# sailordiary/m3f.pytorch

Hardware: AMD Instinct MI355X
Metric: clips/sec (300-frame A+V, fwd+bwd) (higher is better)
Workload: dtype f32 (fp32-accurate products, fp32 accumulate: GEMMs as fp16x3 -- two fp16 terms per scaled operand, three MFMAs, error vs fp64 no larger than an fp32 GEMM's; the forward and backward recurrences at H=512 and H=256 as fp16x3 too (h is bounded; the backward producers split their values under a power-o

## Files before the change

### include/m3t_hip.h

```cpp
#ifndef M3T_HIP_H
#define M3T_HIP_H

#include <stddef.h>
#include <stdint.h>

#ifdef __cplusplus
extern "C" {
#endif

#define M3T_EINVAL 10001
#define M3T_MAX_SCANS 8
#define M3T_ESPIN 10002
#define M3T_SCAN_NO_PERSIST 1
#define M3T_SCAN_WHH 8
#define M3T_SCAN_FP32 4
#define M3T_SCAN_FAULT 16
#define M3T_SCAN_WIDE 32
#define M3T_BF16 2
#define M3T_GEMM_BACKGROUND 1
#define M3T_GEMM_BF16 2
#define M3T_GEMM_HIGH 256
#define M3T_GEMM_F16X3 1024
#define M3T_GEMM_BESIDE_SCAN 512
#define M3T_GEMM_EXCLUSIVE 8
#define M3T_CONV_IMAGES 4096

int m3t_im2col3d(const float* x, int N, int Ci, int T, int H, int W, int kt, int kh, int kw, int st, int sh, int sw,
                 int pt, int ph, int pw, float* out, long long rows_pad, int Kp, unsigned long long* amax_slot, void* stream);

int m3t_conv3d_taps(const float* src, const float* w_taps, float* dst, int N, int C_src, int C_dst, int T, int H, int W,
                    int To, int Ho, int Wo, int kt, int kh, int kw, int base_t, int base_h, int base_w, int sign, int flags,
                    const unsigned long long* amax_src, const unsigned long long* amax_w, float* ws, size_t ws_bytes, float* dst_planes,
                    void* stream);

int m3t_f16x3_split(const float* x, size_t rows, int cols, size_t ld, float* out, size_t ldo, const unsigned long long* slot, void* stream);
int m3t_f16x3_split_perm(const float* w, size_t R, int T, int Cc, size_t sR, size_t sT, size_t sC, float* out, const unsigned long long* slot,
                         void* stream);
int m3t_sgemm_pre(int M, int N, int K, const float* A_img, int lda, const float* B_img, int ldb, float* C, int ldc,
                  const float* bias, int act, int accumulate, const unsigned long long* amax_a, const unsigned long long* amax_b, void* stream);
int m3t_f16x3_image_b(const float* w, int N, int K, size_t ld, float* img, const unsigned long long* slot, void* stream);
int m3t_sgemm_bimg(int M, int N, int K, const float* A, int lda, const float* B_img, float* C, int ldc, const float* bias, int act,
                   int accumulate, float* ws, size_t ws_bytes, const unsigned long long* amax_a, const unsigned long long* amax_b, void* stream);
int m3t_sgemm_ring(int transA, int transB, int M, int N, int K, const float* A, int lda, const float* B, int ldb, float* C, int ldc,
                   const float* bias, int act, int accumulate, int seg_len, int seg_stride, int a_off, int b_off, float* ws, size_t ws_bytes,
                   int splits, const unsigned long long* amax_a, const unsigned long long* amax_b, int variant, void* stream);
int m3t_conv3d_taps_pre(const float* src_img, const float* w_img, float* dst, int N, int C_src, int C_dst, int T, int H, int W,
                        int To, int Ho, int Wo, int kt, int kh, int kw, int base_t, int base_h, int base_w, int sign,
                        const unsigned long long* amax_src, const unsigned long long* amax_w, float* ws, size_t ws_bytes, float* dst_planes,
                    void* stream);

int m3t_planes_to_cl4(const float* x, float* out, int N, int C, long long S, void* stream);
int m3t_conv3d_fwd_taps4(const float* x_img4, const float* w_img, const float* bias, float* y_cl, int N, int Co, int T, int H, int W,
                         int kt, int kh, int kw, int st, int sh, int sw, int pt, int ph, int pw, const unsigned long long* amax_x,
                         const unsigned long long* amax_w, float* ws, size_t ws_bytes, float* y_planes, void* stream);
int m3t_conv3d_fwd_taps(const float* x_img, const float* w_img, const float* bias, float* y_cl, int N, int Ci, int Co, int T, int H, int W,
                        int kt, int kh, int kw, int st, int sh, int sw, int pt, int ph, int pw, const unsigned long long* amax_x,
                        const unsigned long long* amax_w, float* ws, size_t ws_bytes, float* y_planes, void* stream);
int m3t_conv3d_wgrad_taps(const float* x_cl, const float* dy_cl, float* dwt, int N, int Ci, int Co, int T, int H, int W, int kt, int kh, int kw,
                          int st, int sh, int sw, int pt, int ph, int pw, int flags, const unsigned long long* amax_x,
                          const unsigned long long* amax_dy, float* ws, size_t ws_bytes, void* stream);

int m3t_amax_out(unsigned long long* slot);

int m3t_version(void);
int m3t_device_arch(char* arch, int cap);

int m3t_sgemm(int transA, int transB, int M, int N, int K,
              const float* A, int lda, const float* B, int ldb,
              float* C, int ldc, const float* bias, int act, int accumulate,
              int seg_len, int seg_stride, int a_off, int b_off,
              float* ws, size_t ws_bytes, int flags, void* stream);

int m3t_sgemm_scaled(int transA, int transB, int M, int N, int K,
                     const float* A, int lda, const float* B, int ldb,
                     float* C, int ldc, const float* bias, int act, int accumulate,
                     int seg_len, int seg_stride, int a_off, int b_off,
                     float* ws, size_t ws_bytes, int flags,
                     const unsigned long long* amax_a, const unsigned long long* amax_b, void* stream);

int m3t_sgemm_window(int transB, int n_seg, int win_len, int win_stride, int win_off, int N, int K,
                     const float* A, int lda, const float* B, int ldb, float* C, int ldc, const float* bias,
                     int act, int accumulate, int flags, const unsigned long long* amax_a, const unsigned long long* amax_b, void* stream);
#define M3T_WINDOW_BATCH 8
typedef struct {
    const float* A; const float* B; float* C; const float* bias;
    const unsigned long long* amax_a; const unsigned long long* amax_b;
    int accumulate;
} m3t_window_problem;
int m3t_sgemm_window_batch(int n, const m3t_window_problem* problems, int transB, int n_seg, int win_len, int win_stride, int win_off,
                           int N, int K, int lda, int ldb, int ldc, int act, int flags, void* stream);

int m3t_absmax(int n, const float* const* x, const size_t* rows, const int* cols, const size_t* ld,
               unsigned long long* const* slots, void* stream);

int m3t_sgemm_plan(int transA, int M, int N, int K, int seg_len, size_t ws_bytes, int flags, int* kernel, int* splits);

int m3t_colsum(const float* X, int M, int N, int ld, float* out, int accumulate,
               float* ws, size_t ws_bytes, void* stream);

int m3t_transpose(const float* src, int R, int C, int lds, float* dst, int ldd, void* stream);

int m3t_relu_bwd(const float* a, float* dy, size_t n, void* stream);

typedef struct {
    const float* xproj;
    const float* w_hh;
    const float* b_hh;
    float* out;
    float* gates;
    float* h_n;
    int H, reverse, ldx, xoff, ldo, ooff;
} m3t_gru_fwd_desc;

int m3t_gru_scan_fwd(const m3t_gru_fwd_desc* scans, int n_scans, int B, int T,
                     float* ws, size_t ws_bytes, int flags, void* stream);

typedef struct {
    const float* dout;
    const float* out;
    const float* gates;
    const float* w_hh_t;
    const float* dh_n;
    float* dgx;
    float* dgh;
    float* dh;
    float* db_part;
    float* db_ih;
    float* db_hh;
    int H, reverse, ldo, ooff, ldg, goff;
    unsigned long long* amax;
    const float* wfrag;
} m3t_gru_bwd_desc;

size_t m3t_gru_bwd_prepare_floats(int H);
int m3t_gru_bwd_prepare(const float* const* w, int n, int H, int whh_direct, float* const* out, void* stream);

int m3t_gru_scan_workgroups(int n_scans, int H, int B, int T, int flags, int backward);
int m3t_gru_persist_count(void);
int m3t_gru_poll_error(void);
int m3t_gru_error_reset(void);
int m3t_gru_error_defer(int on);
int m3t_gru_inject_error(void* stream);
int m3t_gru_persist_owner(void);
int m3t_gru_scan_arena(void* arena, size_t bytes);
int m3t_gru_scan_arena_reset(void* arena);
int m3t_gru_scan_progress(unsigned* counters, int n_marks, const int* time_bounds, unsigned* need);
int m3t_gru_scan_progress_reset(unsigned* counters);
int m3t_gru_scan_progress_ok(int n_scans, int H, int B, int T, int flags, int backward);
int m3t_stream_wait_progress(const unsigned* counter, unsigned need, void* stream);
int m3t_gru_scan_after(void* event);
int m3t_gru_scan_events(void* start, void* end);
int m3t_gru_persist_profile(unsigned long long* out6);

int m3t_gru_scan_bwd(const m3t_gru_bwd_desc* scans, int n_scans, int B, int T,
                     float* ws, size_t ws_bytes, int flags, void* stream);

int m3t_att_fuse_fwd(const float* s_v, const float* s_a, const float* x_v, const float* x_a,
                     float* f, int rows, int D, void* stream);
int m3t_att_fuse_bwd(const float* df, const float* s_v, const float* s_a,
                     const float* x_v, const float* x_a,
                     float* ds_v, float* ds_a, float* dx_v, float* dx_a,
                     int rows, int D, void* stream);

int m3t_va_loss(const float* y_hat, int rows, int C, int iv, int ia,
                const float* valence, const float* arousal,
                const int64_t* class_expr, const uint8_t* expr_valid, int n_expr,
                float w_v, float w_a, float expr_w, int use_mse,
                float* out_scalars, float* dy, float* ws, size_t ws_bytes, void* stream);
size_t m3t_va_loss_ws_bytes(int rows);

size_t m3t_bn_cl_ws_bytes(size_t M, int C);
int m3t_bn_pool_cl_fwd(const float* x, size_t P, int H, int W, int C, int k, const float* gamma, const float* beta, float* run_mean, float* run_var,
                       float momentum, float eps, int training, float* yp, unsigned char* win, float* save_mean, float* save_invstd, float* ws,
// ... 207 lines not shown
```

### m3f.pytorch_amd/csrc/gemm.hip

```cpp
#include "common.h"
#include <cstdio>
#include <cstdlib>

namespace {

constexpr int BM = 128, BN = 128, BK = 16, LDT = 132;

struct GemmParams {
    const float* A; const float* B; float* C; const float* bias; float* ws;
    int M, N, K, lda, ldb, ldc;
    int act, accumulate, splits, kchunk;
    int seg_len, seg_stride, a_off, b_off;
    int bf16;
    int vecA, vecB;
};

__device__ __forceinline__ int seg_row(int k, int seg_len, int seg_stride, int off) {
    return seg_len > 0 ? (k / seg_len) * seg_stride + (k % seg_len) + off : k;
}

__device__ __forceinline__ void load_kc(const float* __restrict__ src, int ld, int rows, int row0,
                                        int k0, int k_end, int vec, float4 (&r)[2]) {
    const int tid = threadIdx.x;
#pragma unroll
// ... 194 lines not shown
            const float bv = (direct && p.bias) ? p.bias[col] : 0.f;
#pragma unroll
            for (int r = 0; r < 16; ++r) {
                const int row = bm + wm * 64 + i * 32 + (r & 3) + 8 * (r >> 2) + 4 * hi;
                if (!FAST && row >= p.M) continue;
                float v = acc[i][j][r];
                float* q = dst + (size_t)row * ldd + col;
                if (direct) {
                    v += bv;
                    if (p.act == 1) v = m3t_relu(v);
                    if (p.accumulate) v += *q;
                }
                *q = v;
            }
        }
}

__global__ void splitk_reduce_kernel(const float* __restrict__ ws, float* __restrict__ C, const float* __restrict__ bias,
                                     int M, int N, int ldc, int splits, int act, int accumulate) {
    const size_t total = (size_t)M * N;
    for (size_t i = blockIdx.x * (size_t)blockDim.x + threadIdx.x; i < total; i += (size_t)gridDim.x * blockDim.x) {
        const int m = (int)(i / N), n = (int)(i % N);
        float s = 0.f;
        for (int k = 0; k < splits; ++k) s += ws[(size_t)k * total + i];
        if (bias) s += bias[n];
        if (act == 1) s = m3t_relu(s);
        float* q = C + (size_t)m * ldc + n;
        if (accumulate) s += *q;
        *q = s;
    }
}

constexpr int SK_FOLD = 32;
__global__ __launch_bounds__(256) void splitk_fold4_kernel(float* __restrict__ ws, size_t total4, int splits) {
    float4* w4 = reinterpret_cast<float4*>(ws);
    const int k0 = blockIdx.y * SK_FOLD, k1 = min(splits, k0 + SK_FOLD);
    for (size_t i = blockIdx.x * (size_t)blockDim.x + threadIdx.x; i < total4; i += (size_t)gridDim.x * blockDim.x) {
        float4 s = make_float4(0.f, 0.f, 0.f, 0.f);
        int k = k0;
        for (; k + 8 <= k1; k += 8) {
            float4 v[8];
#pragma unroll
            for (int u = 0; u < 8; ++u) v[u] = w4[(size_t)(k + u) * total4 + i];
#pragma unroll
            for (int u = 0; u < 8; ++u) { s.x += v[u].x; s.y += v[u].y; s.z += v[u].z; s.w += v[u].w; }
        }
        for (; k < k1; ++k) {
            const float4 v = w4[(size_t)k * total4 + i];
            s.x += v.x; s.y += v.y; s.z += v.z; s.w += v.w;
        }
        w4[(size_t)k0 * total4 + i] = s;
    }
}

__global__ __launch_bounds__(256) void splitk_reduce4_kernel(const float* __restrict__ ws, float* __restrict__ C,
                                                             const float* __restrict__ bias, int M, int N, int ldc, int splits,
                                                             int act, int accumulate, int kstride) {
    const size_t total4 = (size_t)M * N / 4, slab4 = total4 * (size_t)kstride;
    const float4* w4 = reinterpret_cast<const float4*>(ws);
    const int n4 = N / 4;
    for (size_t i = blockIdx.x * (size_t)blockDim.x + threadIdx.x; i < total4; i += (size_t)gridDim.x * blockDim.x) {
        float4 s = make_float4(0.f, 0.f, 0.f, 0.f);
        int k = 0;
        for (; k + 8 <= splits; k += 8) {
            float4 v[8];
#pragma unroll
            for (int u = 0; u < 8; ++u) v[u] = w4[(size_t)(k + u) * slab4 + i];
#pragma unroll
            for (int u = 0; u < 8; ++u) { s.x += v[u].x; s.y += v[u].y; s.z += v[u].z; s.w += v[u].w; }
        }
        for (; k < splits; ++k) {
            const float4 v = w4[(size_t)k * slab4 + i];
            s.x += v.x; s.y += v.y; s.z += v.z; s.w += v.w;
        }
        const int m = (int)(i / n4), n = (int)(i % n4) * 4;
        if (bias) { s.x += bias[n]; s.y += bias[n + 1]; s.z += bias[n + 2]; s.w += bias[n + 3]; }
        if (act == 1) { s.x = m3t_relu(s.x); s.y = m3t_relu(s.y); s.z = m3t_relu(s.z); s.w = m3t_relu(s.w); }
        float4* q = reinterpret_cast<float4*>(C + (size_t)m * ldc + n);
        if (accumulate) { const float4 c = *q; s.x += c.x; s.y += c.y; s.z += c.z; s.w += c.w; }
        *q = s;
    }
}


constexpr int ABSMAX_REGIONS = 16;
struct AbsmaxArgs { M3TRegion r[ABSMAX_REGIONS]; };
__global__ __launch_bounds__(256) void f16x3_absmax_kernel(AbsmaxArgs a, unsigned epoch) {
    const M3TRegion r = a.r[blockIdx.y];
    const unsigned long long total = r.rows * (unsigned long long)r.c4;
    if ((unsigned long long)blockIdx.x * 256 >= total && blockIdx.x > 0) return;
    unsigned m = 0u;
    const bool dense = (unsigned long long)r.c4 * 4ull == r.ld;
    auto at = [&](unsigned long long i) -> const uint4* {
        if (dense) return reinterpret_cast<const uint4*>(r.p + (size_t)i * 4);
        const unsigned long long row = i / (unsigned)r.c4;
        return reinterpret_cast<const uint4*>(r.p + (size_t)(row * r.ld + (i - row * (unsigned)r.c4) * 4ull));
    };
    auto fin = [](unsigned b) { b &= 0x7fffffffu; return b < 0x7f800000u ? b : 0u; };
    auto fold = [&](const uint4& v) { m = max(max(m, fin(v.x)), max(fin(v.y), max(fin(v.z), fin(v.w)))); };
    const unsigned long long stride = (unsigned long long)gridDim.x * 256;
    unsigned long long i = (unsigned long long)blockIdx.x * 256 + threadIdx.x;
    for (; i + 3 * stride < total; i += 4 * stride) {
        const uint4 v0 = *at(i), v1 = *at(i + stride), v2 = *at(i + 2 * stride), v3 = *at(i + 3 * stride);
        fold(v0); fold(v1); fold(v2); fold(v3);
    }
    for (; i < total; i += stride) fold(*at(i));
#pragma unroll
    for (int o = 32; o > 0; o >>= 1) m = max(m, (unsigned)__shfl_xor((int)m, o, 64));
    __shared__ unsigned red[4];
    if ((threadIdx.x & 63) == 0) red[threadIdx.x >> 6] = m;
    __syncthreads();
    if (threadIdx.x == 0) {
        m = max(max(red[0], red[1]), max(red[2], red[3]));
        const unsigned long long val = ((unsigned long long)epoch << 32) | m;
        if (__hip_atomic_load(r.slot, __ATOMIC_RELAXED, __HIP_MEMORY_SCOPE_AGENT) < val) atomicMax(r.slot, val);
    }
}

static int launch_absmax(const M3TRegion* regs, int n, unsigned epoch, hipStream_t s) {
    AbsmaxArgs a;
    unsigned long long tm = 0;
    for (int i = 0; i < n; ++i) {
        a.r[i] = regs[i];
        const unsigned long long t = regs[i].rows * (unsigned long long)regs[i].c4;
        if (t > tm) tm = t;
    }
    for (int i = n; i < ABSMAX_REGIONS; ++i) a.r[i] = regs[0];
    unsigned long long blocks = (tm + 256ull * 8 - 1) / (256ull * 8);
    static int total = 0;
    if (!total) { const char* e = getenv("M3T_ABSMAX_TOTAL"); total = (e && atoi(e) > 0) ? atoi(e) : 384; }
    const unsigned long long cap = (unsigned long long)max(16, total / max(1, n));
    if (blocks > cap) blocks = cap;
    if (blocks < 1) blocks = 1;
    if (blocks > 1024) blocks = 1024;
    f16x3_absmax_kernel<<<dim3((unsigned)blocks, n), 256, 0, s>>>(a, epoch);
    return (int)hipGetLastError();
}

static void launch_splitk_reduce(const float* ws, float* C, const float* bias, int M, int N, int ldc, int splits, int act,
                                 int accumulate, hipStream_t s) {
    const size_t total = (size_t)M * N;
    if (N % 4 == 0 && ldc % 4 == 0 && ((uintptr_t)C % 16) == 0 && ((uintptr_t)ws % 16) == 0) {
        int blocks = (int)((total / 4 + 255) / 256);
        if (blocks > 4096) blocks = 4096;
        if (splits >= 4 * SK_FOLD && blocks <= 64) {
            const int groups = (splits + SK_FOLD - 1) / SK_FOLD;
            splitk_fold4_kernel<<<dim3(blocks, groups), 256, 0, s>>>(const_cast<float*>(ws), total / 4, splits);
            splitk_reduce4_kernel<<<blocks, 256, 0, s>>>(ws, C, bias, M, N, ldc, groups, act, accumulate, SK_FOLD);
            return;
        }
        splitk_reduce4_kernel<<<blocks, 256, 0, s>>>(ws, C, bias, M, N, ldc, splits, act, accumulate, 1);
        return;
    }
    int blocks = (int)((total + 255) / 256);
    if (blocks > 2048) blocks = 2048;
    splitk_reduce_kernel<<<blocks, 256, 0, s>>>(ws, C, bias, M, N, ldc, splits, act, accumulate);
}

__global__ void colsum_kernel(const float* __restrict__ X, int M, int N, int ld, float* __restrict__ out, int accumulate) {
    __shared__ float red[8][33];
    const int c = blockIdx.x * 32 + (threadIdx.x & 31);
    const int rl = threadIdx.x >> 5;
    float s = 0.f;
    if (c < N)
        for (int m = rl; m < M; m += 8) s += X[(size_t)m * ld + c];
    red[rl][threadIdx.x & 31] = s;
// ... 182 lines not shown
    }
    return on == 1;
}

bool m3t_gemm_tr_enabled() {
    static int on = -1;
    if (on < 0) {
        const char* e = getenv("M3T_GEMM_TR");
        on = (e && e[0] == '0') ? 0 : 1;
    }
    return on == 1;
}

static bool f16x3_on_x6d() { return true; }

static bool x6_enabled() {
    static int on = -1;
    if (on < 0) {
        const char* e = getenv("M3T_GEMM_X6");
        on = (e && e[0] == '0') ? 0 : 1;
    }
    return on == 1;
}

constexpr int GEMM_NO_WIDE = 1 << 20;
struct GemmPlan { int kernel, splits, kchunk, narrow, wide; };

static int narrow_mode() { return 1; }

static bool x6w_enabled() {
    static int on = -1;
    if (on < 0) { const char* e = getenv("M3T_GEMM_X6W"); on = (e && e[0] == '0') ? 0 : 1; }
    return on == 1;
}

static bool tr_wide_wins(int flags) { return (flags & M3T_GEMM_BESIDE_SCAN) != 0; }

static GemmPlan plan_gemm(int transA, int M, int N, int K, int seg_len, bool vec, size_t ws_bytes, int flags) {
    GemmPlan g;
    g.narrow = 0;
    const int bf16 = (flags & M3T_GEMM_BF16) ? 1 : 0;
    const int high = (!bf16 && (flags & M3T_GEMM_HIGH)) ? 1 : 0;
    const int f16x3 = (!bf16 && !high && (flags & M3T_GEMM_F16X3) && m3t_f16x3_enabled()) ? 1 : 0;
    const int tiles = cdiv(M, BM) * cdiv(N, BN);
    const bool n64 = (N % 128 != 0) && (N % 64 == 0) && narrow_mode();
    const bool x6 = x6_enabled() && (M % 128 == 0) && (N % 128 == 0 || n64) && (K % 32 == 0 || seg_len >= 32) && K > 0 && vec &&
                    (seg_len == 0 || seg_len >= 32);
    const double ns_per_k = x6 ? (bf16 ? 14.0 : (high ? 27.0 : (f16x3 ? 22.0 : 36.0))) : 84.0;
    const int kq = x6 ? 32 : BK;
    int splits = 1;
    const size_t cap = ws_bytes / ((size_t)M * N * sizeof(float));
    double best = 1e30;
    auto model = [&](int ntiles, double nsk, int sp) {
        const int rounds = cdiv(ntiles * sp, 256);
        double t = (double)rounds * ((double)K / sp) * nsk * (rounds == 1 ? 1.3 : 1.0);
        if (sp > 1) t += (double)(sp + 2) * M * N * 4.0 / 3000.0 + 3000.0;
        return t;
    };
    if (ws_bytes && K >= 512) {
        for (int sp = 1; sp <= 96 && sp <= K / 96 && (sp == 1 || (size_t)sp <= cap); ++sp) {
            const double t = model(tiles, ns_per_k, sp);
            if (t < best) { best = t; splits = sp; }
        }
    } else best = model(tiles, ns_per_k, 1);
    g.wide = 0;
    if (x6 && !bf16 && !high && N % 256 == 0 && x6w_enabled() && !(flags & (M3T_GEMM_BACKGROUND | GEMM_NO_WIDE))) {
        const int tiles_w = cdiv(M, BM) * (N / 256);
        double best_w = 1e30; int splits_w = 1;
        if (ws_bytes && K >= 512) {
            for (int sp = 1; sp <= 96 && sp <= K / 96 && (sp == 1 || (size_t)sp <= cap); ++sp) {
                const double t = model(tiles_w, 2.0 * 0.8 * ns_per_k, sp);
                if (t < best_w) { best_w = t; splits_w = sp; }
            }
        } else best_w = model(tiles_w, 2.0 * 0.8 * ns_per_k, 1);
        if (best_w < best) { g.wide = 1; splits = splits_w; }
    }
    int kchunk = cdiv(cdiv(K, splits), kq) * kq;
    if (kchunk < kq) kchunk = kq;
    g.kernel = x6 ? 1 : 0; g.kchunk = kchunk; g.splits = K > 0 ? cdiv(K, kchunk) : 1;
    g.narrow = (!g.wide && x6 && narrow_mode() && (n64 || narrow_mode() == 2 || (g.splits == 1 && tiles <= 384))) ? 1 : 0;
    return g;
}

extern "C" int m3t_sgemm_plan(int transA, int M, int N, int K, int seg_len, size_t ws_bytes, int flags, int* kernel, int* splits) {
    if (M <= 0 || N <= 0 || K < 0 || !kernel || !splits) return M3T_EINVAL;
    const GemmPlan g = plan_gemm(transA, M, N, K, seg_len, true, ws_bytes, flags | (transA ? GEMM_NO_WIDE : 0));
    *kernel = g.kernel; *splits = g.splits;
    return 0;
}

extern "C" int m3t_sgemm(int transA, int transB, int M, int N, int K, const float* A, int lda, const float* B, int ldb,
                         float* C, int ldc, const float* bias, int act, int accumulate, int seg_len, int seg_stride,
                         int a_off, int b_off, float* ws, size_t ws_bytes, int flags, void* stream) {
    return m3t_sgemm_scaled(transA, transB, M, N, K, A, lda, B, ldb, C, ldc, bias, act, accumulate, seg_len, seg_stride, a_off, b_off,
                            ws, ws_bytes, flags, nullptr, nullptr, stream);
}

extern "C" int m3t_sgemm_scaled(int transA, int transB, int M, int N, int K, const float* A, int lda, const float* B, int ldb,
                                float* C, int ldc, const float* bias, int act, int accumulate, int seg_len, int seg_stride,
                                int a_off, int b_off, float* ws, size_t ws_bytes, int flags, const unsigned long long* amax_a,
                                const unsigned long long* amax_b, void* stream) {
    if (M <= 0 || N <= 0) return 0;
    if (K < 0 || !A || !B || !C) return M3T_EINVAL;
    if (seg_len > 0 && !(transA == 1 && transB == 0)) return M3T_EINVAL;
    GemmParams p;
    p.A = A; p.B = B; p.C = C; p.bias = bias; p.ws = ws;
    p.M = M; p.N = N; p.K = K; p.lda = lda; p.ldb = ldb; p.ldc = ldc;
    p.act = act; p.accumulate = accumulate;
    p.seg_len = seg_len; p.seg_stride = seg_stride; p.a_off = a_off; p.b_off = b_off;
    p.bf16 = (flags & M3T_GEMM_BF16) ? 1 : 0;
    p.vecA = (lda % 4 == 0) && ((uintptr_t)A % 16 == 0);
    p.vecB = (ldb % 4 == 0) && ((uintptr_t)B % 16 == 0);
    const int tm = cdiv(M, BM), tn = cdiv(N, BN);
    const GemmPlan g = plan_gemm(transA, M, N, K, seg_len, p.vecA && p.vecB, ws ? ws_bytes : 0,
                                 flags | ((transA == 0 && transB == 1) ? 0 : GEMM_NO_WIDE));
    int splits = g.splits, kchunk = g.kchunk;
    {
        static int beside_wgs = -1;
        if (beside_wgs < 0) { const char* e = getenv("M3T_GEMM_BESIDE_WGS"); beside_wgs = e ? atoi(e) : 384; }
        if (beside_wgs > 0 && (flags & M3T_GEMM_BESIDE_SCAN) && g.kernel != 0 && !g.wide && g.splits > 1) {
            const int tiles = cdiv(M, BM) * cdiv(N, g.narrow ? 64 : BN);
            int sp = (beside_wgs + tiles / 2) / tiles;
            if (sp < 1) sp = 1;
            if (sp < g.splits) {
                kchunk = cdiv(cdiv(K, sp), 32) * 32;
                splits = cdiv(K, kchunk);
            }
        }
    }
    p.splits = splits; p.kchunk = kchunk;
    hipStream_t s = (hipStream_t)stream;
    if (g.kernel != 0) {
        int rc;
        const int f16x3 = (!p.bf16 && !(flags & M3T_GEMM_HIGH) && (flags & M3T_GEMM_F16X3) && m3t_f16x3_enabled()) ? 1 : 0;
        const bool wide_tr = f16x3 && !g.wide && !g.narrow && !(transA == 0 && transB == 1) && !(flags & M3T_GEMM_BACKGROUND) && N % 256 == 0 &&
                             K % 32 == 0 && x6w_enabled() && m3t_gemm_tr_enabled() && tr_wide_wins(flags);
        const unsigned long long* use_a = nullptr; const unsigned long long* use_b = nullptr;
        if (f16x3) {
            const size_t kr = seg_len > 0 ? (size_t)(K / seg_len - 1) * seg_stride + seg_len : (size_t)K;
            const float* A0 = seg_len > 0 ? A + (size_t)a_off * lda : A;
            const float* B0 = seg_len > 0 ? B + (size_t)b_off * ldb : B;
            const M3TRegion ra{A0, (unsigned long long)(transA ? kr : (size_t)M), (unsigned long long)lda, (transA ? M : K) / 4, nullptr};
            const M3TRegion rb{B0, (unsigned long long)(transB ? (size_t)N : kr), (unsigned long long)ldb, (transB ? K : N) / 4, nullptr};
            const int rm = m3t_f16x3_measure(ra, amax_a, rb, amax_b, &use_a, &use_b, s);
            if (rm) return rm;
        }
        if (g.wide || wide_tr)
            rc = m3t_sgemm_x6w_launch(transA, transB, M, N, K, A, lda, B, ldb, C, ldc, bias, act, accumulate, seg_len, seg_stride,
                                      a_off, b_off, ws, splits, kchunk, f16x3 ? 3 : 0, use_a, use_b, s);
        else if (!g.narrow && K % 32 == 0 && (!f16x3 || f16x3_on_x6d()) && !(flags & (M3T_GEMM_BACKGROUND | M3T_GEMM_HIGH)) && (x6d_mode() == 1 || (x6d_mode() == 2 && !(flags & M3T_GEMM_BESIDE_SCAN))))
            rc = m3t_sgemm_x6d_launch(transA, transB, M, N, K, A, lda, B, ldb, C, ldc, bias, act, accumulate, seg_len, seg_stride,
                                      a_off, b_off, ws, splits, kchunk, p.bf16 ? 1 : ((flags & M3T_GEMM_HIGH) ? 2 : (f16x3 ? 3 : 0)), use_a, use_b, s);
        else
            rc = m3t_sgemm_x6_launch(transA, transB, M, N, K, A, lda, B, ldb, C, ldc, bias, act, accumulate, seg_len, seg_stride,
                                     a_off, b_off, ws, splits, kchunk, (flags & M3T_GEMM_BACKGROUND) ? (size_t)40 * 1024 : 0,
                                     p.bf16 ? 1 : ((flags & M3T_GEMM_HIGH) ? 2 : (f16x3 ? 3 : 0)), g.narrow, use_a, use_b, s);
        if (rc) return rc;
        if (splits > 1) {
            launch_splitk_reduce(ws, C, bias, M, N, ldc, splits, act, accumulate, s);
            M3T_LAUNCH_CHECK();
        }
        return 0;
    }
    dim3 grid(tn, tm, splits), block(256);
    const bool fast = (M % BM == 0) && (N % BN == 0) && (K % BK == 0) && K > 0 && p.vecA && p.vecB;
    const size_t dyn = (flags & M3T_GEMM_BACKGROUND) ? (size_t)56 * 1024 + 0 : 0;
#define M3T_GEMM_LAUNCH(TA_, TB_)                                                 \
    do {                                                                          \
        if (fast && seg_len >= BK) sgemm_kernel<TA_, TB_, true, true><<<grid, block, dyn, s>>>(p); \
        else if (seg_len > 0) sgemm_kernel<TA_, TB_, false><<<grid, block, dyn, s>>>(p);           \
        else if (fast) sgemm_kernel<TA_, TB_, true><<<grid, block, dyn, s>>>(p);    \
        else sgemm_kernel<TA_, TB_, false><<<grid, block, dyn, s>>>(p);             \
    } while (0)
    if (transA == 0 && transB == 1) M3T_GEMM_LAUNCH(0, 1);
    else if (transA == 0 && transB == 0) M3T_GEMM_LAUNCH(0, 0);
    else if (transA == 1 && transB == 0) M3T_GEMM_LAUNCH(1, 0);
    else M3T_GEMM_LAUNCH(1, 1);
#undef M3T_GEMM_LAUNCH
    M3T_LAUNCH_CHECK();
    if (splits > 1) {
        launch_splitk_reduce(ws, C, bias, M, N, ldc, splits, act, accumulate, s);
        M3T_LAUNCH_CHECK();
    }
    return 0;
}

int m3t_sgemm_x6_window_launch(int n, const m3t_window_problem* pr, int transB, int M, int N, int K, int lda, int ldb, int ldc,
                               int act, int mw_len, int mw_stride, int mw_off, int f16x3, int narrow, hipStream_t s);

extern "C" int m3t_sgemm_window_batch(int n, const m3t_window_problem* pr, int transB, int n_seg, int win_len, int win_stride, int win_off,
                                      int N, int K, int lda, int ldb, int ldc, int act, int flags, void* stream) {
    if (n <= 0 || n_seg <= 0 || win_len <= 0 || N <= 0) return 0;
    if (n > M3T_WINDOW_BATCH || !pr || K <= 0 || win_stride < win_len || win_off < 0 || win_off + win_len > win_stride) return M3T_EINVAL;
    const long long Ml = (long long)n_seg * win_len;
    if (Ml > 0x7fffffffll || (long long)n_seg * win_stride > 0x7fffffffll) return M3T_EINVAL;
    const int M = (int)Ml;
    if (!x6_enabled() || M % 128 != 0 || N % 64 != 0 || K % 32 != 0 || lda % 4 != 0 || ldb % 4 != 0 || (flags & (M3T_GEMM_BF16 | M3T_GEMM_HIGH)))
        return M3T_EINVAL;
    const int f16x3 = ((flags & M3T_GEMM_F16X3) && m3t_f16x3_enabled()) ? 1 : 0;
    hipStream_t s = (hipStream_t)stream;
    m3t_window_problem use[M3T_WINDOW_BATCH];
    for (int i = 0; i < n; ++i) {
        use[i] = pr[i];
        if (!use[i].A || !use[i].B || !use[i].C || (uintptr_t)use[i].A % 16 != 0 || (uintptr_t)use[i].B % 16 != 0) return M3T_EINVAL;
        if (f16x3 && (!use[i].amax_a || !use[i].amax_b)) {
            if (n > 1) return M3T_EINVAL;
            const size_t span = (size_t)(n_seg - 1) * win_stride + win_len;
            const M3TRegion ra{use[i].A + (size_t)win_off * lda, (unsigned long long)span, (unsigned long long)lda, K / 4, nullptr};
            const M3TRegion rb{use[i].B, (unsigned long long)(transB ? (size_t)N : (size_t)K), (unsigned long long)ldb, (transB ? K : N) / 4, nullptr};
            const int rm = m3t_f16x3_measure(ra, use[i].amax_a, rb, use[i].amax_b, &use[i].amax_a, &use[i].amax_b, s);
            if (rm) return rm;
        }
    }
    const int narrow = (N % 128 != 0 || (long long)(M / 128) * (N / 128) * n <= 384) ? 1 : 0;
    return m3t_sgemm_x6_window_launch(n, use, transB ? 1 : 0, M, N, K, lda, ldb, ldc, act, win_len, win_stride, win_off, f16x3, narrow, s);
}

extern "C" int m3t_sgemm_window(int transB, int n_seg, int win_len, int win_stride, int win_off, int N, int K,
                                const float* A, int lda, const float* B, int ldb, float* C, int ldc, const float* bias,
                                int act, int accumulate, int flags, const unsigned long long* amax_a, const unsigned long long* amax_b,
                                void* stream) {
    const m3t_window_problem pr{A, B, C, bias, amax_a, amax_b, accumulate};
    return m3t_sgemm_window_batch(1, &pr, transB, n_seg, win_len, win_stride, win_off, N, K, lda, ldb, ldc, act, flags, stream);
}

int m3t_conv3d_taps_launch(const float* src, const float* w_taps, float* dst, int N, int Cs, int Cd, int T, int H, int W, int To, int Ho, int Wo,
                           int kt, int kh, int kw, int bt_, int bh, int bw, int sg, int f16x3, int pre, const unsigned long long* amax_a,
                           const unsigned long long* amax_b, float* ws, int splits, int kchunk, hipStream_t s, const int* stride3 = nullptr,
                           const float* bias = nullptr, int planes = 0);
extern "C" int m3t_btc_to_bct(const float* src, float* dst, int B, int T, int C, void* stream);
int m3t_conv3d_wgrad_launch(const float* x_cl, const float* dy_cl, float* dwt, int N, int Ci, int Co, int T, int H, int W, int To, int Ho, int Wo,
                            int kt, int kh, int kw, const int* stride3, int pt, int ph, int pw, int f16x3, const unsigned long long* amax_x,
                            const unsigned long long* amax_dy, float* ws, int splits, int kchunk, hipStream_t s, int pre);

int m3t_conv3d_taps4_launch(const float* x_img4, const float* w_img, const float* bias, float* y_cl, int N, int Co, int T, int H, int W, int To,
                            int Ho, int Wo, int kt, int kh, int kw, const int* stride3, int pt, int ph, int pw, const unsigned long long* amax_x,
                            const unsigned long long* amax_w, float* ws, int splits, int kchunk, hipStream_t s, int planes);

static void taps_split(long long rows, int Cd, int K, float* ws, size_t ws_bytes, int& splits, int& kchunk) {
    splits = 1; kchunk = K;
    const long long tiles = ((rows + 127) / 128) * ((Cd + 127) / 128);
    if (!ws || tiles >= 512) return;
    int sp = (int)((640 + tiles - 1) / tiles);
    const size_t cap = ws_bytes / ((size_t)rows * Cd * sizeof(float));
    if ((size_t)sp > cap) sp = (int)cap;
    if (sp > K / 256) sp = K / 256;
    if (sp < 2) return;
    kchunk = cdiv(cdiv(K, sp), 32) * 32;
    splits = cdiv(K, kchunk);
}

namespace {
typedef _Float16 sp_f16x2 __attribute__((ext_vector_type(2)));
typedef float sp_f32x2 __attribute__((ext_vector_type(2)));
__global__ __launch_bounds__(256) void f16x3_split_kernel(const float* __restrict__ x, float* __restrict__ out, size_t rows, int c4, size_t ld,
                                                          size_t ldo, const unsigned long long* __restrict__ slot) {
    float sc, inv;
    m3t_f16_scale((unsigned)*slot, sc, inv);
    const size_t total = rows * (size_t)c4;
    for (size_t i = blockIdx.x * (size_t)blockDim.x + threadIdx.x; i < total; i += (size_t)gridDim.x * blockDim.x) {
        const size_t r = i / c4; const int c = (int)(i - r * c4);
        const float4 v = *reinterpret_cast<const float4*>(x + r * ld + 4 * (size_t)c);
        const sp_f32x2 a = (sp_f32x2){v.x, v.y} * sc, b = (sp_f32x2){v.z, v.w} * sc;
        const sp_f16x2 ha = __builtin_convertvector(a, sp_f16x2), hb = __builtin_convertvector(b, sp_f16x2);
        const sp_f16x2 la = __builtin_convertvector(a - __builtin_convertvector(ha, sp_f32x2), sp_f16x2);
// ... 417 lines not shown
```

### m3f.pytorch_amd/csrc/gemm_x6.hip

```cpp
#include "common.h"
#include <cstdlib>

namespace {

typedef __bf16 bf16x8 __attribute__((ext_vector_type(8)));
typedef __bf16 bf16x4 __attribute__((ext_vector_type(4)));

constexpr int XM = 128, XN = 128, XK = 32;
constexpr int PLANE = XM * 16 + 64;
constexpr int SPLIT_BYTES = 4 * PLANE;
constexpr int OPER_BYTES = 3 * SPLIT_BYTES;
constexpr int TRROW = XM * 2 + 64;
constexpr int TRTERM = XK * TRROW;
static_assert(2 * TRTERM <= OPER_BYTES, "the transposed-read image must fit the operand's LDS");
typedef short s16x4 __attribute__((ext_vector_type(4)));

struct X6Params {
    const float* A; const float* B; float* C; const float* bias; float* ws;
    int M, N, K, lda, ldb, ldc;
    int act, accumulate, splits, kchunk;
    int seg_len, seg_stride, a_off, b_off;
    int cv_T, cv_C, cv_K, cv_dil, cv_lead, cv_anti;
    size_t cv_btap;
    const float* cv_mask; const float* cv_res; float* cv_pre;
// ... 62 lines not shown
__device__ __forceinline__ void kc_store(unsigned char* __restrict__ S, const float4 (&r)[4], float scale = 1.f) {
    const int tid = threadIdx.x & 255;
    const int c = tid & 7, r0 = tid >> 3;
#pragma unroll
    for (int i = 0; i < NR; ++i) {
        unsigned lo[3], hi2[3];
        if (PRE) {
            lo[0] = __float_as_uint(r[i].x); hi2[0] = __float_as_uint(r[i].y); lo[1] = __float_as_uint(r[i].z); hi2[1] = __float_as_uint(r[i].w);
        } else {
            split3_pair<NS>((f32x2){r[i].x, r[i].y}, lo, scale);
            split3_pair<NS>((f32x2){r[i].z, r[i].w}, hi2, scale);
        }
#pragma unroll
        for (int s = 0; s < planes_of(NS); ++s)
            *reinterpret_cast<u32x2*>(S + s * SPLIT_BYTES + (c >> 1) * PLANE + (r0 + 32 * i) * 16 + (c & 1) * 8) = (u32x2){lo[s], hi2[s]};
    }
}
template <int NS, bool PRE = false>
__device__ __forceinline__ void mc_store(unsigned char* __restrict__ S, const float4 (&r)[4], float scale = 1.f) {
    const int tid = threadIdx.x & 255;
    const int wave = tid >> 6, h = (tid >> 5) & 1, row0 = (tid & 31) * 4;
    typedef unsigned u32x4 __attribute__((ext_vector_type(4)));
    unsigned lo[4][3], hi2[4][3];
    if (PRE && NS == 4) {
#pragma unroll
        for (int i = 0; i < 4; ++i) {
            const unsigned sel = (i & 1) ? 0x07060302u : 0x05040100u;
#pragma unroll
            for (int s = 0; s < 2; ++s) {
                const unsigned c0 = __float_as_uint(s == 0 ? (i < 2 ? r[0].x : r[0].y) : (i < 2 ? r[0].z : r[0].w));
                const unsigned c1 = __float_as_uint(s == 0 ? (i < 2 ? r[1].x : r[1].y) : (i < 2 ? r[1].z : r[1].w));
                const unsigned c2 = __float_as_uint(s == 0 ? (i < 2 ? r[2].x : r[2].y) : (i < 2 ? r[2].z : r[2].w));
                const unsigned c3 = __float_as_uint(s == 0 ? (i < 2 ? r[3].x : r[3].y) : (i < 2 ? r[3].z : r[3].w));
                lo[i][s] = __builtin_amdgcn_perm(c1, c0, sel);
                hi2[i][s] = __builtin_amdgcn_perm(c3, c2, sel);
            }
        }
    } else
#pragma unroll
    for (int i = 0; i < 4; ++i) {
        const float v0 = i == 0 ? r[0].x : i == 1 ? r[0].y : i == 2 ? r[0].z : r[0].w;
        const float v1 = i == 0 ? r[1].x : i == 1 ? r[1].y : i == 2 ? r[1].z : r[1].w;
        const float v2 = i == 0 ? r[2].x : i == 1 ? r[2].y : i == 2 ? r[2].z : r[2].w;
        const float v3 = i == 0 ? r[3].x : i == 1 ? r[3].y : i == 2 ? r[3].z : r[3].w;
        split3_pair<NS>((f32x2){v0, v1}, lo[i], scale);
        split3_pair<NS>((f32x2){v2, v3}, hi2[i], scale);
    }
    unsigned char* q = S + wave * PLANE + (row0 + 2 * h) * 16;
#pragma unroll
    for (int s = 0; s < planes_of(NS); ++s) {
        const u32x2 e0 = __builtin_amdgcn_permlane32_swap(lo[0][s], lo[2][s], false, false);
        const u32x2 e1 = __builtin_amdgcn_permlane32_swap(hi2[0][s], hi2[2][s], false, false);
        const u32x2 f0 = __builtin_amdgcn_permlane32_swap(lo[1][s], lo[3][s], false, false);
        const u32x2 f1 = __builtin_amdgcn_permlane32_swap(hi2[1][s], hi2[3][s], false, false);
        *reinterpret_cast<u32x4*>(q + s * SPLIT_BYTES) = (u32x4){e0.x, e1.x, e0.y, e1.y};
        *reinterpret_cast<u32x4*>(q + s * SPLIT_BYTES + 16) = (u32x4){f0.x, f1.x, f0.y, f1.y};
    }
}

template <int NS, bool PRE = false>
__device__ __forceinline__ void mc_store_tr(unsigned char* __restrict__ S, const float4 (&r)[4], float scale = 1.f) {
    const int tid = threadIdx.x & 255;
    unsigned char* q = S + 4 * (tid >> 5) * TRROW + (tid & 31) * 8;
#pragma unroll
    for (int e = 0; e < 4; ++e) {
        unsigned a[3], b[3];
        if (PRE) {
            a[0] = __float_as_uint(r[e].x); b[0] = __float_as_uint(r[e].y); a[1] = __float_as_uint(r[e].z); b[1] = __float_as_uint(r[e].w);
        } else {
            split3_pair<NS>((f32x2){r[e].x, r[e].y}, a, scale);
            split3_pair<NS>((f32x2){r[e].z, r[e].w}, b, scale);
        }
#pragma unroll
        for (int s = 0; s < planes_of(NS); ++s) *reinterpret_cast<u32x2*>(q + s * TRTERM + e * TRROW) = (u32x2){a[s], b[s]};
    }
}
__device__ __forceinline__ bf16x8 tr_frag(const unsigned char* at) {
    typedef __attribute__((address_space(3))) s16x4 lds_s16x4;
    const s16x4 lo = __builtin_amdgcn_ds_read_tr16_b64_v4i16((lds_s16x4*)(at));
    const s16x4 hi = __builtin_amdgcn_ds_read_tr16_b64_v4i16((lds_s16x4*)(at + 4 * TRROW));
    return __builtin_bit_cast(bf16x8, __builtin_shufflevector(lo, hi, 0, 1, 2, 3, 4, 5, 6, 7));
}

template <int TA, int TB, bool SEG, int NS, bool CONV = false, int XNT = 128, bool MW = false, int C3 = 0, int PRE = 0, bool TR = false>
__global__ __launch_bounds__(256, 3) void sgemm_x6_kernel(X6Params p, X6Batch bt) {
    static_assert(!TR || NS == 4, "the transposed-read image is sized for two terms");
    constexpr bool TRA = TR && TA == 1, TRB = TR && TB == 0;
    if (MW) {
        const int z = blockIdx.z;
        p.A = bt.A[z]; p.B = bt.B[z]; p.C = bt.C[z]; p.bias = bt.bias[z];
        p.amax_a = bt.amax_a[z]; p.amax_b = bt.amax_b[z]; p.accumulate = bt.accumulate[z];
    }
    constexpr int NJ = XNT / 64;
    constexpr int BR = XNT / 32;
    __shared__ __attribute__((aligned(16))) unsigned char lds[2 * OPER_BYTES];
    unsigned char* As = lds;
    unsigned char* Bs = lds + OPER_BYTES;
    const int tid = threadIdx.x, lane = tid & 63, wave = tid >> 6;
    const int wm = wave >> 1, wn = wave & 1;
    const int l31 = lane & 31, hi = lane >> 5;

    const int tn_ = gridDim.x, nt_ = gridDim.x * gridDim.y;
    const int lin = blockIdx.y * tn_ + blockIdx.x;
    const int xq = nt_ >> 3, xr = nt_ & 7, xcd = lin & 7, slot = lin >> 3;
    const int til = xcd * xq + min(xcd, xr) + slot;
    const int bm = (til / tn_) * XM, bn = (til % tn_) * XNT;
    const bool bcol = XNT == 128 || (tid & 31) < 16;
    const int k_begin = MW ? 0 : blockIdx.z * p.kchunk;
    const int k_end = min(p.K, k_begin + p.kchunk);
    const int ntiles = (C3 == 2 || SEG) ? (k_end - k_begin + XK - 1) / XK : (k_end - k_begin) / XK;
    __shared__ int rowmap[MW ? XM : 1];
    if (MW) {
        if (tid < XM) {
            const int m = bm + tid, q = m / p.mw_len;
            rowmap[tid] = q * p.mw_stride + (m - q * p.mw_len) + p.mw_off;
        }
        __syncthreads();
    }

    f32x16 acc[2][NJ];
#pragma unroll
    for (int i = 0; i < 2; ++i)
#pragma unroll
        for (int j = 0; j < NJ; ++j)
#pragma unroll
            for (int r = 0; r < 16; ++r) acc[i][j][r] = 0.f;

    float sc_a = 1.f, sc_b = 1.f, sc_ia = 1.f, sc_ib = 1.f;
    if (NS == 4) {
        m3t_f16_scale((unsigned)*p.amax_a, sc_a, sc_ia);
        m3t_f16_scale((unsigned)*p.amax_b, sc_b, sc_ib);
    }

    const float* pa; const float* pb;
    size_t a_step, b_step, a_krow = 0, b_krow = 0;
    const float* paw[MW ? 4 : 1];
    if (TA == 0) { pa = p.A + (size_t)(bm + (tid >> 3)) * p.lda + k_begin + (tid & 7) * 4; a_step = XK; }
    else { pa = p.A + (size_t)(k_begin + (tid >> 5) * 4) * p.lda + bm + (tid & 31) * 4; a_step = (size_t)XK * p.lda; a_krow = p.lda; }
    if (MW) {
#pragma unroll
        for (int i = 0; i < 4; ++i) paw[i] = p.A + (size_t)rowmap[(tid >> 3) + 32 * i] * p.lda + k_begin + (tid & 7) * 4;
    }
    if (TB == 1) { pb = p.B + (size_t)(bn + (tid >> 3)) * p.ldb + k_begin + (tid & 7) * 4; b_step = XK; }
    else { pb = p.B + (size_t)(k_begin + (tid >> 5) * 4) * p.ldb + bn + (tid & 31) * 4; b_step = (size_t)XK * p.ldb; b_krow = p.ldb; }
    int sq = 0, sr = 0;
    if (SEG) {
        const int k = k_begin + (tid >> 5) * 4;
        sq = k / p.seg_len; sr = k % p.seg_len;
    }

    constexpr bool C3ROWS = C3 == 1 || C3 == 3;
    int c3_tt[C3ROWS ? 4 : 1], c3_hh[C3ROWS ? 4 : 1], c3_ww[C3ROWS ? 4 : 1], c3_nb[C3ROWS ? 4 : 1];
    if (C3ROWS) {
#pragma unroll
        for (int i = 0; i < 4; ++i) {
            int m = bm + (tid >> 3) + 32 * i;
            const bool past = m >= p.M;
            const int w_ = m % p.c3_W; m /= p.c3_W;
            const int h_ = m % p.c3_H; m /= p.c3_H;
            const int t_ = m % p.c3_T; m /= p.c3_T;
            c3_tt[i] = past ? -(1 << 28) : t_ * p.c3_st + p.c3_bt; c3_hh[i] = h_ * p.c3_sh + p.c3_bh; c3_ww[i] = w_ * p.c3_sw + p.c3_bw; c3_nb[i] = past ? 0 : m * p.c3_To;
        }
    }
    int g_w = 0, g_h = 0, g_t = 0, g_n = 0, adv_w = 0, adv_h = 0, adv_t = 0, adv_n = 0, g_dt = 0, g_dh = 0, g_dw = 0, g_c = 0;
    int g_k = 0;
    bool g_ok = false;
    if (SEG) g_k = k_begin + (tid >> 5) * 4;
    if (C3 == 2) {
        g_k = k_begin + (tid >> 5) * 4;
        const int m0 = bm + (tid & 31) * 4;
        const int j = m0 / p.c3_C;
        g_c = m0 - j * p.c3_C;
        g_ok = j < p.c3_kt * p.c3_kh * p.c3_kw;
        const int khw = p.c3_kh * p.c3_kw;
        const int jt = j / khw, jr = j - jt * khw, jh = jr / p.c3_kw, jw = jr - jh * p.c3_kw;
        g_dt = p.c3_bt + jt; g_dh = p.c3_bh + jh; g_dw = p.c3_bw + jw;
        int k = k_begin + (tid >> 5) * 4;
        g_w = k % p.c3_W; k /= p.c3_W; g_h = k % p.c3_H; k /= p.c3_H; g_t = k % p.c3_T; g_n = k / p.c3_T;
        int a = XK;
        adv_w = a % p.c3_W; a /= p.c3_W; adv_h = a % p.c3_H; a /= p.c3_H; adv_t = a % p.c3_T; adv_n = a / p.c3_T;
    }
    int cv_t[4] = {0, 0, 0, 0}, cv_k = k_begin;
    if (CONV) {
#pragma unroll
        for (int i = 0; i < 4; ++i) cv_t[i] = (bm + (tid >> 3) + 32 * i) % p.cv_T;
    }
    float4 ra[4], rb[4];
    auto gload = [&]() {
        if (C3 == 2) {
            int w_ = g_w, h_ = g_h, t_ = g_t, n_ = g_n;
#pragma unroll
// ... 81 lines not shown
#pragma unroll
                for (int i = 0; i < 4; ++i) { ra[i] = *reinterpret_cast<const float4*>(paw[i]); paw[i] += XK; }
            } else if (TA == 0) kc_load(pa, p.lda, ra);
            else {
#pragma unroll
                for (int e = 0; e < 4; ++e) ra[e] = *reinterpret_cast<const float4*>(pa + e * a_krow);
            }
            if (TB == 1) kc_load<BR>(pb, p.ldb, rb);
            else {
#pragma unroll
                for (int e = 0; e < 4; ++e) rb[e] = bcol ? *reinterpret_cast<const float4*>(pb + e * b_krow) : make_float4(0.f, 0.f, 0.f, 0.f);
            }
            pa += a_step; pb += b_step;
        }
    };
    auto sstore = [&]() {
        if (TA == 0) kc_store<NS, 4, (PRE & 1) != 0>(As, ra, sc_a);
        else if (TRA) mc_store_tr<NS, (PRE & 1) != 0>(As, ra, sc_a);
        else mc_store<NS, (PRE & 1) != 0>(As, ra, sc_a);
        if (TB == 1) kc_store<NS, BR, (PRE & 2) != 0>(Bs, rb, sc_b);
        else if (TRB) mc_store_tr<NS, (PRE & 2) != 0>(Bs, rb, sc_b);
        else mc_store<NS, (PRE & 2) != 0>(Bs, rb, sc_b);
    };

    const int tro = (8 * hi + ((lane >> 2) & 3)) * TRROW + (16 * ((lane >> 4) & 1) + 4 * (lane & 3)) * 2;
    if (ntiles > 0) { gload(); sstore(); }
    __syncthreads();
    for (int t = 0; t < ntiles; ++t) {
        if (t + 1 < ntiles) gload();
        __builtin_amdgcn_sched_barrier(0);
#pragma unroll
        for (int kh = 0; kh < 2; ++kh) {
            constexpr int NP = planes_of(NS);
            bf16x8 fa[NP][2], fb[NP][NJ];
#pragma unroll
            for (int s = 0; s < NP; ++s)
#pragma unroll
                for (int i = 0; i < 2; ++i) {
                    if (TRA) fa[s][i] = tr_frag(As + tro + s * TRTERM + kh * 16 * TRROW + (wm * 64 + i * 32) * 2);
                    else fa[s][i] = *reinterpret_cast<const bf16x8*>(As + s * SPLIT_BYTES + (kh * 2 + hi) * PLANE + (wm * 64 + i * 32 + l31) * 16);
                    if (i < NJ) {
                        if (TRB) fb[s][i] = tr_frag(Bs + tro + s * TRTERM + kh * 16 * TRROW + (wn * 32 * NJ + i * 32) * 2);
                        else fb[s][i] = *reinterpret_cast<const bf16x8*>(Bs + s * SPLIT_BYTES + (kh * 2 + hi) * PLANE + (wn * 32 * NJ + i * 32 + l31) * 16);
                    }
                }
            __builtin_amdgcn_sched_barrier(0);
#pragma unroll
            for (int i = 0; i < 2; ++i)
#pragma unroll
                for (int j = 0; j < NJ; ++j) {
                    f32x16 c = acc[i][j];
                    if (NS == 4) {
                        c = __builtin_amdgcn_mfma_f32_32x32x16_f16(__builtin_bit_cast(f16x8, fa[1][i]), __builtin_bit_cast(f16x8, fb[0][j]), c, 0, 0, 0);
                        c = __builtin_amdgcn_mfma_f32_32x32x16_f16(__builtin_bit_cast(f16x8, fa[0][i]), __builtin_bit_cast(f16x8, fb[1][j]), c, 0, 0, 0);
                        c = __builtin_amdgcn_mfma_f32_32x32x16_f16(__builtin_bit_cast(f16x8, fa[0][i]), __builtin_bit_cast(f16x8, fb[0][j]), c, 0, 0, 0);
                        acc[i][j] = c;
                        continue;
                    }
                    if (NS == 2) {
                        c = __builtin_amdgcn_mfma_f32_32x32x16_bf16(fa[1][i], fb[1][j], c, 0, 0, 0);
                        c = __builtin_amdgcn_mfma_f32_32x32x16_bf16(fa[1][i], fb[0][j], c, 0, 0, 0);
                        c = __builtin_amdgcn_mfma_f32_32x32x16_bf16(fa[0][i], fb[1][j], c, 0, 0, 0);
                    }
                    if (NS == 3) {
                        c = __builtin_amdgcn_mfma_f32_32x32x16_bf16(fa[NS - 1][i], fb[0][j], c, 0, 0, 0);
                        c = __builtin_amdgcn_mfma_f32_32x32x16_bf16(fa[NS / 2][i], fb[NS / 2][j], c, 0, 0, 0);
                        c = __builtin_amdgcn_mfma_f32_32x32x16_bf16(fa[0][i], fb[NS - 1][j], c, 0, 0, 0);
                        c = __builtin_amdgcn_mfma_f32_32x32x16_bf16(fa[NS / 2][i], fb[0][j], c, 0, 0, 0);
                        c = __builtin_amdgcn_mfma_f32_32x32x16_bf16(fa[0][i], fb[NS / 2][j], c, 0, 0, 0);
                    }
                    c = __builtin_amdgcn_mfma_f32_32x32x16_bf16(fa[0][i], fb[0][j], c, 0, 0, 0);
                    acc[i][j] = c;
                }
        }
        __builtin_amdgcn_sched_barrier(0);
        __syncthreads();
        if (t + 1 < ntiles) {
            sstore();
            __syncthreads();
        }
    }

    const bool direct = p.splits == 1;
    float* dst = direct ? p.C : p.ws + (size_t)blockIdx.z * p.M * p.N;
    const int ldd = direct ? p.ldc : p.N;
    if constexpr (C3 == 1 || C3 == 3) {
        if (direct && p.tr_S > 0) {
            const int S = p.tr_S;
#pragma unroll
            for (int i = 0; i < 2; ++i)
#pragma unroll
                for (int j = 0; j < NJ; ++j) {
                    const int col = bn + wn * 32 * NJ + j * 32 + l31;
                    const float bv = p.bias ? p.bias[col] : 0.f;
#pragma unroll
                    for (int q4 = 0; q4 < 4; ++q4) {
                        const int m0 = bm + wm * 64 + i * 32 + 8 * q4 + 4 * hi;
                        if (m0 >= p.M) continue;
                        int n = m0 / S, sp = m0 - n * S;
                        float4 v;
                        v.x = acc[i][j][4 * q4 + 0] * sc_ia * sc_ib + bv; v.y = acc[i][j][4 * q4 + 1] * sc_ia * sc_ib + bv;
                        v.z = acc[i][j][4 * q4 + 2] * sc_ia * sc_ib + bv; v.w = acc[i][j][4 * q4 + 3] * sc_ia * sc_ib + bv;
                        if ((S & 3) == 0) *reinterpret_cast<float4*>(p.C + ((size_t)n * p.N + col) * S + sp) = v;
                        else {
                            const float ve[4] = {v.x, v.y, v.z, v.w};
#pragma unroll
                            for (int e = 0; e < 4; ++e) {
                                if (m0 + e >= p.M) break;
                                p.C[((size_t)n * p.N + col) * S + sp] = ve[e];
                                if (++sp == S) { sp = 0; ++n; }
                            }
                        }
                    }
                }
            return;
        }
    }
    float vmax = 0.f;
#pragma unroll
    for (int i = 0; i < 2; ++i)
#pragma unroll
        for (int j = 0; j < NJ; ++j) {
            const int col = bn + wn * 32 * NJ + j * 32 + l31;
            const float bv = (direct && p.bias) ? p.bias[col] : 0.f;
            float dm[4] = {1.f, 1.f, 1.f, 1.f};
#pragma unroll
            for (int r = 0; r < 16; ++r) {
                const int row = bm + wm * 64 + i * 32 + (r & 3) + 8 * (r >> 2) + 4 * hi;
                if (C3ROWS && row >= p.M) continue;
                if (CONV && p.cv_drop.on && (r & 3) == 0) m3t_drop_mask4(p.cv_drop, (uint32_t)row >> 2, (uint32_t)col, dm);
                float v = acc[i][j][r];
                if (NS == 4) v = v * sc_ia * sc_ib;
                float* q = dst + (size_t)(MW ? rowmap[row - bm] : row) * ldd + col;
                if (CONV) {
                    const size_t o = (size_t)row * ldd + col;
                    v += bv;
                    if (p.cv_pre) p.cv_pre[o] = v;
                    const float mk = p.cv_drop.on ? dm[r & 3] : (p.cv_mask ? p.cv_mask[o] : 1.f);
                    if (p.act == 1) v = m3t_relu(v) * mk;
                    else if (p.act == 2) v = m3t_relu(m3t_relu(v) * mk + p.cv_res[o]);
                    else if (p.cv_res) v += p.cv_res[o];
                    vmax = fmaxf(vmax, m3t_fin_abs(v));
                } else if (direct) {
                    v += bv;
                    if (p.act == 1) v = m3t_relu(v);
                    if (p.accumulate) v += *q;
                }
                *q = v;
            }
        }
    if (CONV && p.cv_amax) {
        __shared__ float red4[4];
        m3t_block_raise_slot(p.cv_amax, vmax, red4);
    }
}

const X6Batch g_no_batch = {};

}

int m3t_sgemm_x6_launch(int transA, int transB, int M, int N, int K, const float* A, int lda, const float* B, int ldb,
                        float* C, int ldc, const float* bias, int act, int accumulate, int seg_len, int seg_stride,
                        int a_off, int b_off, float* ws, int splits, int kchunk, size_t dyn_lds, int bf16_operands, int narrow,
                        const unsigned long long* amax_a, const unsigned long long* amax_b, hipStream_t s) {
    X6Params p;
    p.amax_a = amax_a; p.amax_b = amax_b;
    p.A = A; p.B = B; p.C = C; p.bias = bias; p.ws = ws;
    p.M = M; p.N = N; p.K = K; p.lda = lda; p.ldb = ldb; p.ldc = ldc;
    p.act = act; p.accumulate = accumulate; p.splits = splits; p.kchunk = kchunk;
    p.seg_len = seg_len; p.seg_stride = seg_stride; p.a_off = a_off; p.b_off = b_off;
    p.cv_T = p.cv_C = p.cv_K = p.cv_dil = p.cv_lead = p.cv_anti = 0; p.cv_btap = 0; p.cv_mask = p.cv_res = nullptr; p.cv_pre = nullptr;
    p.cv_drop = m3t_make_drop(0.f, 0ull);
    p.cv_amax = nullptr;
    p.mw_len = p.mw_stride = p.mw_off = 0;
    p.c3_T = p.c3_H = p.c3_W = p.c3_To = p.c3_Ho = p.c3_Wo = p.c3_kt = p.c3_kh = p.c3_kw = p.c3_bt = p.c3_bh = p.c3_bw = p.c3_sg = p.c3_C = 0; p.c3_st = p.c3_sh = p.c3_sw = 1; p.tr_S = 0;
    dim3 grid(N / (narrow ? 64 : XN), M / XM, splits), block(256);
#define M3T_X6_DISPATCH(NS_, XNT_, TR_)                                                                                                                 \
    do {                                                                                                                                               \
        if (seg_len > 0) sgemm_x6_kernel<1, 0, true, NS_, false, XNT_, false, 0, 0, TR_><<<grid, block, dyn_lds, s>>>(p, g_no_batch);                  \
        else if (transA == 0 && transB == 1) sgemm_x6_kernel<0, 1, false, NS_, false, XNT_><<<grid, block, dyn_lds, s>>>(p, g_no_batch);               \
        else if (transA == 0 && transB == 0) sgemm_x6_kernel<0, 0, false, NS_, false, XNT_, false, 0, 0, TR_><<<grid, block, dyn_lds, s>>>(p, g_no_batch); \
        else if (transA == 1 && transB == 0) sgemm_x6_kernel<1, 0, false, NS_, false, XNT_, false, 0, 0, TR_><<<grid, block, dyn_lds, s>>>(p, g_no_batch); \
        else sgemm_x6_kernel<1, 1, false, NS_, false, XNT_, false, 0, 0, TR_><<<grid, block, dyn_lds, s>>>(p, g_no_batch);                             \
    } while (0)
    if (bf16_operands == 3 && (!amax_a || !amax_b)) return M3T_EINVAL;
    const bool tr = m3t_gemm_tr_enabled();
    if (bf16_operands == 1) { if (narrow) M3T_X6_DISPATCH(1, 64, false); else M3T_X6_DISPATCH(1, 128, false); }
    else if (bf16_operands == 2) { if (narrow) M3T_X6_DISPATCH(2, 64, false); else M3T_X6_DISPATCH(2, 128, false); }
    else if (bf16_operands == 3 && tr) { if (narrow) M3T_X6_DISPATCH(4, 64, true); else M3T_X6_DISPATCH(4, 128, true); }
    else if (bf16_operands == 3) { if (narrow) M3T_X6_DISPATCH(4, 64, false); else M3T_X6_DISPATCH(4, 128, false); }
    else { if (narrow) M3T_X6_DISPATCH(3, 64, false); else M3T_X6_DISPATCH(3, 128, false); }
#undef M3T_X6_DISPATCH
    hipError_t e = hipGetLastError();
    return (int)e;
}

int m3t_sgemm_x6_window_launch(int n, const m3t_window_problem* pr, int transB, int M, int N, int K, int lda, int ldb, int ldc,
                               int act, int mw_len, int mw_stride, int mw_off, int f16x3, int narrow, hipStream_t s) {
    X6Params p;
    X6Batch bt = {};
    for (int i = 0; i < n; ++i) {
        if (f16x3 && (!pr[i].amax_a || !pr[i].amax_b)) return M3T_EINVAL;
        bt.A[i] = pr[i].A; bt.B[i] = pr[i].B; bt.C[i] = pr[i].C; bt.bias[i] = pr[i].bias;
        bt.amax_a[i] = pr[i].amax_a; bt.amax_b[i] = pr[i].amax_b; bt.accumulate[i] = pr[i].accumulate;
    }
    p.amax_a = p.amax_b = nullptr;
    p.A = p.B = nullptr; p.C = nullptr; p.bias = nullptr; p.ws = nullptr;
    p.M = M; p.N = N; p.K = K; p.lda = lda; p.ldb = ldb; p.ldc = ldc;
    p.act = act; p.accumulate = 0; p.splits = 1; p.kchunk = K;
    p.seg_len = p.seg_stride = p.a_off = p.b_off = 0;
    p.cv_T = p.cv_C = p.cv_K = p.cv_dil = p.cv_lead = p.cv_anti = 0; p.cv_btap = 0; p.cv_mask = p.cv_res = nullptr; p.cv_pre = nullptr;
    p.cv_drop = m3t_make_drop(0.f, 0ull);
    p.cv_amax = nullptr;
    p.mw_len = mw_len; p.mw_stride = mw_stride; p.mw_off = mw_off;
    dim3 grid(N / (narrow ? 64 : XN), M / XM, n), block(256);
#define M3T_X6W_GO(NS_, XNT_, TR_)                                                                                  \
    do {                                                                                                            \
        if (transB) sgemm_x6_kernel<0, 1, false, NS_, false, XNT_, true><<<grid, block, 0, s>>>(p, bt);             \
        else sgemm_x6_kernel<0, 0, false, NS_, false, XNT_, true, 0, 0, TR_><<<grid, block, 0, s>>>(p, bt);         \
    } while (0)
    if (f16x3 && m3t_gemm_tr_enabled()) { if (narrow) M3T_X6W_GO(4, 64, true); else M3T_X6W_GO(4, 128, true); }
    else if (f16x3) { if (narrow) M3T_X6W_GO(4, 64, false); else M3T_X6W_GO(4, 128, false); }
    else { if (narrow) M3T_X6W_GO(3, 64, false); else M3T_X6W_GO(3, 128, false); }
#undef M3T_X6W_GO
    return (int)hipGetLastError();
}


int m3t_sgemm_x6_pre_launch(int M, int N, int K, const float* A, int lda, const float* B, int ldb, float* C, int ldc, const float* bias,
                            int act, int accumulate, int narrow, const unsigned long long* amax_a, const unsigned long long* amax_b, hipStream_t s) {
    if (!amax_a || !amax_b) return M3T_EINVAL;
    X6Params p;
    p.amax_a = amax_a; p.amax_b = amax_b; p.cv_amax = nullptr;
    p.A = A; p.B = B; p.C = C; p.bias = bias; p.ws = nullptr;
    p.M = M; p.N = N; p.K = K; p.lda = lda; p.ldb = ldb; p.ldc = ldc;
    p.act = act; p.accumulate = accumulate; p.splits = 1; p.kchunk = K;
    p.seg_len = p.seg_stride = p.a_off = p.b_off = 0;
    p.cv_T = p.cv_C = p.cv_K = p.cv_dil = p.cv_lead = p.cv_anti = 0; p.cv_btap = 0; p.cv_mask = p.cv_res = nullptr; p.cv_pre = nullptr;
    p.cv_drop = m3t_make_drop(0.f, 0ull);
    p.mw_len = p.mw_stride = p.mw_off = 0;
    p.c3_T = p.c3_H = p.c3_W = p.c3_To = p.c3_Ho = p.c3_Wo = p.c3_kt = p.c3_kh = p.c3_kw = p.c3_bt = p.c3_bh = p.c3_bw = p.c3_sg = p.c3_C = 0; p.c3_st = p.c3_sh = p.c3_sw = 1; p.tr_S = 0;
    dim3 grid(N / (narrow ? 64 : XN), M / XM, 1), block(256);
    if (narrow) sgemm_x6_kernel<0, 1, false, 4, false, 64, false, false, 3><<<grid, block, 0, s>>>(p, g_no_batch);
    else sgemm_x6_kernel<0, 1, false, 4, false, 128, false, false, 3><<<grid, block, 0, s>>>(p, g_no_batch);
    return (int)hipGetLastError();
}

int m3t_conv3d_taps_launch(const float* src, const float* w_taps, float* dst, int N, int Cs, int Cd, int T, int H, int W, int To, int Ho, int Wo,
                           int kt, int kh, int kw, int bt_, int bh, int bw, int sg, int f16x3, int pre, const unsigned long long* amax_a,
                           const unsigned long long* amax_b, float* ws, int splits, int kchunk, hipStream_t s, const int* stride3,
                           const float* bias, int planes) {
    X6Params p;
    if (pre && !f16x3) return M3T_EINVAL;
    if (f16x3 && (!amax_a || !amax_b)) return M3T_EINVAL;
    p.amax_a = amax_a; p.amax_b = amax_b; p.cv_amax = nullptr;
    p.A = src; p.B = w_taps; p.C = dst; p.bias = bias; p.ws = ws;
    p.M = N * T * H * W; p.N = Cd; p.K = kt * kh * kw * Cs; p.lda = Cs; p.ldb = pre ? kt * kh * kw * Cs : Cd; p.ldc = Cd;
    p.act = 0; p.accumulate = 0; p.splits = splits; p.kchunk = kchunk;
    p.seg_len = p.seg_stride = p.a_off = p.b_off = 0;
    p.cv_T = p.cv_C = p.cv_K = p.cv_dil = p.cv_lead = p.cv_anti = 0; p.cv_btap = 0; p.cv_mask = p.cv_res = nullptr; p.cv_pre = nullptr;
    p.cv_drop = m3t_make_drop(0.f, 0ull);
    p.mw_len = p.mw_stride = p.mw_off = 0;
    p.c3_T = T; p.c3_H = H; p.c3_W = W; p.c3_To = To; p.c3_Ho = Ho; p.c3_Wo = Wo; p.c3_kt = kt; p.c3_kh = kh; p.c3_kw = kw;
    p.c3_bt = bt_; p.c3_bh = bh; p.c3_bw = bw; p.c3_sg = sg; p.c3_C = Cs;
    p.c3_st = stride3 ? stride3[0] : 1; p.c3_sh = stride3 ? stride3[1] : 1; p.c3_sw = stride3 ? stride3[2] : 1;
    p.tr_S = (planes && splits == 1) ? T * H * W : 0;
    const int tm = (p.M + XM - 1) / XM;
    const bool narrow = (Cd % 128 != 0) || (Cd / XN) * tm * splits <= 384;
    dim3 grid(Cd / (narrow ? 64 : XN), tm, splits), block(256);
#define M3T_C3_GO(NS_, TR_)                                                                                                  \
    do {                                                                                                                     \
        if (narrow) sgemm_x6_kernel<0, 0, false, NS_, false, 64, false, 1, 0, TR_><<<grid, block, 0, s>>>(p, g_no_batch);    \
        else sgemm_x6_kernel<0, 0, false, NS_, false, 128, false, 1, 0, TR_><<<grid, block, 0, s>>>(p, g_no_batch);          \
    } while (0)
    if (pre) {
        if (narrow) sgemm_x6_kernel<0, 1, false, 4, false, 64, false, 1, 3><<<grid, block, 0, s>>>(p, g_no_batch);
        else sgemm_x6_kernel<0, 1, false, 4, false, 128, false, 1, 3><<<grid, block, 0, s>>>(p, g_no_batch);
// ... 106 lines not shown
```

### m3f.pytorch_amd/csrc/gemm_x6d.hip

```cpp
#include "common.h"
#include <cstdlib>
#include <type_traits>

namespace {

typedef __bf16 bf16x8 __attribute__((ext_vector_type(8)));
typedef __bf16 bf16x4 __attribute__((ext_vector_type(4)));
typedef __bf16 bf16x2 __attribute__((ext_vector_type(2)));
typedef float f32x2 __attribute__((ext_vector_type(2)));
typedef unsigned u32x2 __attribute__((ext_vector_type(2)));
typedef unsigned u32x4 __attribute__((ext_vector_type(4)));
typedef float f32x4 __attribute__((ext_vector_type(4)));

constexpr int BM = 128, BN = 128, BKS = 16, NTH = 256;
constexpr int PLANEB = BM * 16 + 128;
constexpr int SPLITB = 2 * PLANEB;
constexpr int OPERB = 3 * SPLITB;
constexpr int STAGEB = 2 * OPERB;
constexpr int TRROW = BM * 2 + 64;
constexpr int TRTERM = BKS * TRROW;
static_assert(2 * TRTERM <= OPERB, "the transposed-read image must fit the operand's LDS");
typedef short s16x4 __attribute__((ext_vector_type(4)));
typedef short s16x8 __attribute__((ext_vector_type(8)));

// ... 13 lines not shown
typedef _Float16 f16x2 __attribute__((ext_vector_type(2)));
typedef _Float16 f16x8 __attribute__((ext_vector_type(8)));
constexpr int planes_of(int NS) { return NS == 4 ? 2 : NS; }
template <int NS>
__device__ __forceinline__ void split3_pair(f32x2 v, unsigned (&o)[3], float scale = 1.f) {
    if (NS == 4) {
        const f32x2 vs = v * scale;
        const f16x2 h = __builtin_convertvector(vs, f16x2);
        o[0] = __builtin_bit_cast(unsigned, h);
        const f32x2 r1 = vs - __builtin_convertvector(h, f32x2);
        const f16x2 l = __builtin_convertvector(r1, f16x2);
        o[1] = __builtin_bit_cast(unsigned, l);
        return;
    }
    const bf16x2 h = __builtin_convertvector(v, bf16x2);
    o[0] = __builtin_bit_cast(unsigned, h);
    if (NS == 1) return;
    f32x2 hf;
    hf.x = __uint_as_float(o[0] << 16); hf.y = __uint_as_float(o[0] & 0xffff0000u);
    const f32x2 r1 = v - hf;
    const bf16x2 m = __builtin_convertvector(r1, bf16x2);
    o[1] = __builtin_bit_cast(unsigned, m);
    if (NS == 2) return;
    f32x2 mf;
    mf.x = __uint_as_float(o[1] << 16); mf.y = __uint_as_float(o[1] & 0xffff0000u);
    const f32x2 r2 = r1 - mf;
    const bf16x2 l = __builtin_convertvector(r2, bf16x2);
    o[2] = __builtin_bit_cast(unsigned, l);
}

template <int NS>
__device__ __forceinline__ void kc_store_c(unsigned char* __restrict__ S, const f32x4 (&r)[2], float scale) {
    const int tid = threadIdx.x;
    unsigned char* q = S + ((tid >> 1) & 1) * PLANEB + (tid >> 2) * 16 + (tid & 1) * 8;
#pragma unroll
    for (int i = 0; i < 2; ++i) {
        unsigned lo[3], hi2[3];
        split3_pair<NS>((f32x2){r[i].x, r[i].y}, lo, scale);
        split3_pair<NS>((f32x2){r[i].z, r[i].w}, hi2, scale);
#pragma unroll
        for (int s = 0; s < planes_of(NS); ++s) *reinterpret_cast<u32x2*>(q + s * SPLITB + i * 1024) = (u32x2){lo[s], hi2[s]};
    }
}
template <int NS>
__device__ __forceinline__ void mc_store_c(unsigned char* __restrict__ S, const f32x4 (&r)[2], float scale) {
    const int tid = threadIdx.x, lane = tid & 63, w = tid >> 6;
    unsigned o[4][3];
    split3_pair<NS>((f32x2){r[0].x, r[1].x}, o[0], scale);
    split3_pair<NS>((f32x2){r[0].y, r[1].y}, o[1], scale);
    split3_pair<NS>((f32x2){r[0].z, r[1].z}, o[2], scale);
    split3_pair<NS>((f32x2){r[0].w, r[1].w}, o[3], scale);
    unsigned char* q = S + (w >> 1) * PLANEB + ((w & 1) * 64 + (lane & 15) * 4 + (lane >> 4)) * 16;
#pragma unroll
    for (int s = 0; s < planes_of(NS); ++s) {
        const u32x2 p01 = __builtin_amdgcn_permlane16_swap(o[0][s], o[1][s], false, false);
        const u32x2 p23 = __builtin_amdgcn_permlane16_swap(o[2][s], o[3][s], false, false);
        const u32x2 c02 = __builtin_amdgcn_permlane32_swap(p01.x, p23.x, false, false);
        const u32x2 c13 = __builtin_amdgcn_permlane32_swap(p01.y, p23.y, false, false);
        *reinterpret_cast<u32x4*>(q + s * SPLITB) = (u32x4){c02.x, c13.x, c02.y, c13.y};
    }
}

template <int NS>
__device__ __forceinline__ void mc_store_tr(unsigned char* __restrict__ S, const f32x4 (&r)[2], float scale) {
    const int tid = threadIdx.x, lane = tid & 63, w = tid >> 6;
    unsigned char* q = S + (8 * (w >> 1) + 2 * (lane >> 4)) * TRROW + ((w & 1) * 64 + (lane & 15) * 4) * 2;
#pragma unroll
    for (int e = 0; e < 2; ++e) {
        unsigned a[3], b[3];
        split3_pair<NS>((f32x2){r[e].x, r[e].y}, a, scale);
        split3_pair<NS>((f32x2){r[e].z, r[e].w}, b, scale);
#pragma unroll
        for (int s = 0; s < planes_of(NS); ++s) *reinterpret_cast<u32x2*>(q + s * TRTERM + e * TRROW) = (u32x2){a[s], b[s]};
    }
}
__device__ __forceinline__ bf16x8 tr_frag(const unsigned char* at) {
    typedef __attribute__((address_space(3))) s16x4 lds_s16x4;
    const s16x4 lo = __builtin_amdgcn_ds_read_tr16_b64_v4i16((lds_s16x4*)(at));
    const s16x4 hi = __builtin_amdgcn_ds_read_tr16_b64_v4i16((lds_s16x4*)(at + 4 * TRROW));
    return __builtin_bit_cast(bf16x8, __builtin_shufflevector(lo, hi, 0, 1, 2, 3, 4, 5, 6, 7));
}

template <int TA, int TB, bool SEG, int NS, bool CONV = false, bool TR = false>
__global__ __launch_bounds__(NTH, 3) void sgemm_x6d_kernel(X6DParams p) {
    static_assert(!TR || NS == 4, "the transposed-read image is sized for two terms");
    constexpr bool TRA = TR && TA == 1, TRB = TR && TB == 0;
    extern __shared__ __attribute__((aligned(16))) unsigned char ldsb[];
    const int tid = threadIdx.x, lane = tid & 63, wave = tid >> 6;
    const int wm = wave >> 1, wn = wave & 1;
    const int l31 = lane & 31, hi = lane >> 5;

    const int tn_ = gridDim.x, nt_ = gridDim.x * gridDim.y;
    const int lin = blockIdx.y * tn_ + blockIdx.x;
    const int xq = nt_ >> 3, xr = nt_ & 7, xcd = lin & 7, slot = lin >> 3;
    const int til = xcd * xq + min(xcd, xr) + slot;
    const int bm = (til / tn_) * BM, bn = (til % tn_) * BN;
    const int k_begin = blockIdx.z * p.kchunk;
    const int k_end = min(p.K, k_begin + p.kchunk);
    const int nst = (k_end - k_begin) / BKS;

    f32x16 acc[2][2];
#pragma unroll
    for (int i = 0; i < 2; ++i)
#pragma unroll
        for (int j = 0; j < 2; ++j)
#pragma unroll
            for (int r = 0; r < 16; ++r) acc[i][j][r] = 0.f;
    float sc_a = 1.f, sc_b = 1.f, sc_ia = 1.f, sc_ib = 1.f;
    if (NS == 4) {
        m3t_f16_scale((unsigned)*p.amax_a, sc_a, sc_ia);
        m3t_f16_scale((unsigned)*p.amax_b, sc_b, sc_ib);
    }

    const float* pa[2]; const float* pb[2];
    size_t a_step, b_step;
    const int mck = 8 * (wave >> 1) + 2 * (lane >> 4);
    const int mcr = (wave & 1) * 64 + (lane & 15) * 4;
    if (TA == 0) {
#pragma unroll
        for (int i = 0; i < 2; ++i) pa[i] = p.A + (size_t)min(bm + (tid >> 2) + 64 * i, p.M - 1) * p.lda + k_begin + (tid & 3) * 4;
        a_step = BKS;
    } else {
        const int c0 = min(bm + mcr, p.M - 4);
#pragma unroll
        for (int e = 0; e < 2; ++e) pa[e] = p.A + (size_t)(k_begin + mck + e) * p.lda + c0;
        a_step = (size_t)BKS * p.lda;
    }
    if (TB == 1) {
#pragma unroll
        for (int i = 0; i < 2; ++i) pb[i] = p.B + (size_t)min(bn + (tid >> 2) + 64 * i, p.N - 1) * p.ldb + k_begin + (tid & 3) * 4;
        b_step = BKS;
    } else {
        const int c0 = min(bn + mcr, p.N - 4);
#pragma unroll
        for (int e = 0; e < 2; ++e) pb[e] = p.B + (size_t)(k_begin + mck + e) * p.ldb + c0;
        b_step = (size_t)BKS * p.ldb;
    }
    int sq[2] = {0, 0}, sr[2] = {0, 0};
    if (SEG) {
#pragma unroll
        for (int e = 0; e < 2; ++e) {
            const int k = k_begin + mck + e;
            sq[e] = k / p.seg_len; sr[e] = k % p.seg_len;
        }
        const int ca = min(bm + mcr, p.M - 4), cb = min(bn + mcr, p.N - 4);
        pa[0] = p.A + (size_t)p.a_off * p.lda + ca;
        pb[0] = p.B + (size_t)p.b_off * p.ldb + cb;
    }

    int cv_t[2] = {0, 0};
    if (CONV) {
#pragma unroll
        for (int i = 0; i < 2; ++i) cv_t[i] = (bm + (tid >> 2) + 64 * i) % p.cv_T;
    }
    f32x4 ra0[2], rb0[2], ra1[2], rb1[2];
    int loaded = 0;
    auto gload = [&](f32x4 (&ra)[2], f32x4 (&rb)[2]) {
        const bool adv = loaded + 1 < nst;
        if (CONV) {
            const int k0 = k_begin + BKS * min(loaded, nst - 1);
            const int j = k0 / p.cv_C, kc = k0 - j * p.cv_C;
            const int sft = (p.cv_K - 1 - j) * p.cv_dil;
            const int off = p.cv_anti ? sft - p.cv_lead : p.cv_lead - sft;
            const float* qa = p.A + ((ptrdiff_t)(bm + (tid >> 2)) + off) * (ptrdiff_t)p.lda + kc + (tid & 3) * 4;
#pragma unroll
            for (int i = 0; i < 2; ++i) {
                const bool ok = (unsigned)(cv_t[i] + off) < (unsigned)p.cv_T;
                ra[i] = ok ? *reinterpret_cast<const f32x4*>(qa + (ptrdiff_t)i * 64 * p.lda) : (f32x4){0.f, 0.f, 0.f, 0.f};
            }
            if (TB == 1) {
                const float* qb = p.B + (size_t)j * p.cv_btap + (size_t)(bn + (tid >> 2)) * p.ldb + kc + (tid & 3) * 4;
#pragma unroll
                for (int i = 0; i < 2; ++i) rb[i] = *reinterpret_cast<const f32x4*>(qb + (size_t)i * 64 * p.ldb);
            } else {
#pragma unroll
                for (int e = 0; e < 2; ++e) {
                    rb[e] = *reinterpret_cast<const f32x4*>(pb[e]);
                    pb[e] += adv ? b_step : 0;
                }
            }
        } else if (SEG) {
#pragma unroll
            for (int e = 0; e < 2; ++e) {
                const size_t row = (size_t)sq[e] * p.seg_stride + sr[e];
                ra[e] = *reinterpret_cast<const f32x4*>(pa[0] + row * p.lda);
                rb[e] = *reinterpret_cast<const f32x4*>(pb[0] + row * p.ldb);
                int r = sr[e] + (adv ? BKS : 0), q = sq[e];
                if (r >= p.seg_len) { r -= p.seg_len; ++q; }
                sr[e] = r; sq[e] = q;
            }
        } else {
#pragma unroll
            for (int e = 0; e < 2; ++e) {
                ra[e] = *reinterpret_cast<const f32x4*>(pa[e]);
                rb[e] = *reinterpret_cast<const f32x4*>(pb[e]);
                pa[e] += adv ? a_step : 0;
                pb[e] += adv ? b_step : 0;
            }
        }
        ++loaded;
    };
    auto sstore = [&](unsigned char* st, const f32x4 (&ra)[2], const f32x4 (&rb)[2]) {
        if (TA == 0) kc_store_c<NS>(st, ra, sc_a); else if (TRA) mc_store_tr<NS>(st, ra, sc_a); else mc_store_c<NS>(st, ra, sc_a);
        if (TB == 1) kc_store_c<NS>(st + OPERB, rb, sc_b); else if (TRB) mc_store_tr<NS>(st + OPERB, rb, sc_b); else mc_store_c<NS>(st + OPERB, rb, sc_b);
    };

    constexpr int NSB = NS == 4 ? 2 : NS;
    constexpr int PA[6] = {NSB - 1, NSB / 2, NSB == 2 ? 1 : 0, NSB == 2 ? 1 : NSB / 2, 0, 0};
    constexpr int PB[6] = {0, NSB / 2, NSB == 2 ? 1 : NSB - 1, 0, NSB == 2 ? 1 : NSB / 2, 0};
    const int tro = (8 * hi + ((lane >> 2) & 3)) * TRROW + (16 * ((lane >> 4) & 1) + 4 * (lane & 3)) * 2;
    const int fro_a = TRA ? tro + wm * 128 : hi * PLANEB + (wm * 64 + l31) * 16;
    const int fro_b = OPERB + (TRB ? tro + wn * 128 : hi * PLANEB + (wn * 64 + l31) * 16);
    auto stage = [&](const unsigned char* cur, unsigned char* nxt, const f32x4 (&ua)[2], const f32x4 (&ub)[2]) {
        constexpr int NP = planes_of(NS);
        bf16x8 fa[NP][2], fb[NP][2];
#pragma unroll
        for (int s = 0; s < NP; ++s)
#pragma unroll
            for (int i = 0; i < 2; ++i) {
                if (TRA) fa[s][i] = tr_frag(cur + fro_a + s * TRTERM + i * 64);
                else fa[s][i] = *reinterpret_cast<const bf16x8*>(cur + fro_a + s * SPLITB + i * 512);
                if (TRB) fb[s][i] = tr_frag(cur + fro_b + s * TRTERM + i * 64);
                else fb[s][i] = *reinterpret_cast<const bf16x8*>(cur + fro_b + s * SPLITB + i * 512);
            }
        sstore(nxt, ua, ub);
#pragma unroll
        for (int i = 0; i < 2; ++i)
#pragma unroll
            for (int j = 0; j < 2; ++j) {
                f32x16 c = acc[i][j];
                if (NS == 4) {
                    c = __builtin_amdgcn_mfma_f32_32x32x16_f16(__builtin_bit_cast(f16x8, fa[1][i]), __builtin_bit_cast(f16x8, fb[0][j]), c, 0, 0, 0);
                    c = __builtin_amdgcn_mfma_f32_32x32x16_f16(__builtin_bit_cast(f16x8, fa[0][i]), __builtin_bit_cast(f16x8, fb[1][j]), c, 0, 0, 0);
                    c = __builtin_amdgcn_mfma_f32_32x32x16_f16(__builtin_bit_cast(f16x8, fa[0][i]), __builtin_bit_cast(f16x8, fb[0][j]), c, 0, 0, 0);
                } else {
#pragma unroll
                    for (int q = (NS == 3 ? 0 : (NS == 2 ? 2 : 5)); q < 6; ++q)
                        c = __builtin_amdgcn_mfma_f32_32x32x16_bf16(fa[PA[q]][i], fb[PB[q]][j], c, 0, 0, 0);
                }
                acc[i][j] = c;
            }
    };

    unsigned char* buf0 = ldsb;
    unsigned char* buf1 = ldsb + STAGEB;
    if (nst > 0) {
        gload(ra0, rb0);
        sstore(buf0, ra0, rb0);
        gload(ra1, rb1);
    }
    asm volatile("s_waitcnt lgkmcnt(0)\n\ts_barrier" ::: "memory");
    for (int t = 0; t < nst; t += 2) {
        gload(ra0, rb0);
        stage(buf0, buf1, ra1, rb1);
        asm volatile("s_waitcnt lgkmcnt(0)\n\ts_barrier" ::: "memory");
        gload(ra1, rb1);
        stage(buf1, buf0, ra0, rb0);
        asm volatile("s_waitcnt lgkmcnt(0)\n\ts_barrier" ::: "memory");
    }

    const bool direct = p.splits == 1;
    float* dst = direct ? p.C : p.ws + (size_t)blockIdx.z * p.M * p.N;
    const int ldd = direct ? p.ldc : p.N;
#pragma unroll
    for (int i = 0; i < 2; ++i)
#pragma unroll
        for (int j = 0; j < 2; ++j) {
            const int col = bn + wn * 64 + j * 32 + l31;
            const float bv = (direct && p.bias) ? p.bias[col] : 0.f;
            float dm[4] = {1.f, 1.f, 1.f, 1.f};
#pragma unroll
            for (int r = 0; r < 16; ++r) {
                const int row = bm + wm * 64 + i * 32 + (r & 3) + 8 * (r >> 2) + 4 * hi;
                if (CONV && p.cv_drop.on && (r & 3) == 0) m3t_drop_mask4(p.cv_drop, (uint32_t)row >> 2, (uint32_t)col, dm);
                float v = acc[i][j][r];
                if (NS == 4) v = v * sc_ia * sc_ib;
                float* q = dst + (size_t)row * ldd + col;
                if (CONV) {
                    const size_t o = (size_t)row * ldd + col;
                    v += bv;
                    if (p.cv_pre) p.cv_pre[o] = v;
                    const float mk = p.cv_drop.on ? dm[r & 3] : (p.cv_mask ? p.cv_mask[o] : 1.f);
                    if (p.act == 1) v = m3t_relu(v) * mk;
                    else if (p.act == 2) v = m3t_relu(m3t_relu(v) * mk + p.cv_res[o]);
                    else if (p.cv_res) v += p.cv_res[o];
                } else if (direct) {
                    v += bv;
                    if (p.act == 1) v = m3t_relu(v);
                    if (p.accumulate) v += *q;
                }
                *q = v;
            }
        }
}

}

int m3t_sgemm_x6d_launch(int transA, int transB, int M, int N, int K, const float* A, int lda, const float* B, int ldb,
                         float* C, int ldc, const float* bias, int act, int accumulate, int seg_len, int seg_stride,
                         int a_off, int b_off, float* ws, int splits, int kchunk, int bf16_operands,
                         const unsigned long long* amax_a, const unsigned long long* amax_b, hipStream_t s) {
    X6DParams p;
    p.amax_a = amax_a; p.amax_b = amax_b;
    if (bf16_operands == 3 && (!amax_a || !amax_b)) return M3T_EINVAL;
    p.A = A; p.B = B; p.C = C; p.bias = bias; p.ws = ws;
    p.M = M; p.N = N; p.K = K; p.lda = lda; p.ldb = ldb; p.ldc = ldc;
    p.act = act; p.accumulate = accumulate; p.splits = splits; p.kchunk = kchunk;
    p.seg_len = seg_len; p.seg_stride = seg_stride; p.a_off = a_off; p.b_off = b_off;
    p.cv_T = p.cv_C = p.cv_K = p.cv_dil = p.cv_lead = p.cv_anti = 0; p.cv_btap = 0; p.cv_mask = p.cv_res = nullptr; p.cv_pre = nullptr;
    p.cv_drop = m3t_make_drop(0.f, 0ull);
    dim3 grid(N / BN, M / BM, splits), block(NTH);
    const size_t lds = 2 * (size_t)STAGEB;
    const bool tr = m3t_gemm_tr_enabled();
#define M3T_X6D_GO(TA_, TB_, SEG_, NS_, TR_)                                                                          \
    do {                                                                                                               \
        static bool attr_set = false;                                                                                  \
        if (!attr_set) {                                                                                               \
            hipError_t ea = hipFuncSetAttribute((const void*)sgemm_x6d_kernel<TA_, TB_, SEG_, NS_, false, TR_>,        \
                                                hipFuncAttributeMaxDynamicSharedMemorySize, (int)lds);                \
            if (ea != hipSuccess) return (int)ea;                                                                      \
            attr_set = true;                                                                                           \
        }                                                                                                              \
        sgemm_x6d_kernel<TA_, TB_, SEG_, NS_, false, TR_><<<grid, block, lds, s>>>(p);                                 \
    } while (0)
#define M3T_X6D_DISPATCH(NS_, TR_)                                                                                   \
    do {                                                                                                               \
        if (seg_len > 0) M3T_X6D_GO(1, 0, true, NS_, TR_);                                                             \
        else if (transA == 0 && transB == 1) M3T_X6D_GO(0, 1, false, NS_, false);                                      \
        else if (transA == 0 && transB == 0) M3T_X6D_GO(0, 0, false, NS_, TR_);                                        \
        else if (transA == 1 && transB == 0) M3T_X6D_GO(1, 0, false, NS_, TR_);                                        \
        else M3T_X6D_GO(1, 1, false, NS_, TR_);                                                                        \
    } while (0)
    if (bf16_operands == 1) M3T_X6D_DISPATCH(1, false);
    else if (bf16_operands == 2) M3T_X6D_DISPATCH(2, false);
    else if (bf16_operands == 3) { if (tr) M3T_X6D_DISPATCH(4, true); else M3T_X6D_DISPATCH(4, false); }
    else M3T_X6D_DISPATCH(3, false);
#undef M3T_X6D_DISPATCH
#undef M3T_X6D_GO
    return (int)hipGetLastError();
}


int m3t_conv_x6d_launch(const float* x, const float* w_t, const float* bias, const float* res, const float* mask, float* y,
                        float* pre, int B, int T, int Ci, int Co, int K, int dil, int lead, int act, int anti, int bf16_operands,
                        M3TDrop drop, hipStream_t s) {
    X6DParams p;
    p.amax_a = p.amax_b = nullptr;
    p.A = x; p.B = w_t; p.C = y; p.bias = bias; p.ws = nullptr;
    p.M = B * T; p.N = Co; p.K = K * Ci; p.lda = Ci; p.ldb = anti ? Co : Ci; p.ldc = Co;
    p.act = act; p.accumulate = 0; p.splits = 1; p.kchunk = K * Ci;
    p.seg_len = p.seg_stride = p.a_off = p.b_off = 0;
    p.cv_T = T; p.cv_C = Ci; p.cv_K = K; p.cv_dil = dil; p.cv_lead = lead; p.cv_anti = anti;
    p.cv_btap = (size_t)Co * Ci; p.cv_mask = mask; p.cv_res = res; p.cv_pre = pre; p.cv_drop = drop;
    dim3 grid(Co / BN, p.M / BM, 1), block(NTH);
    const size_t lds = 2 * (size_t)STAGEB;
#define M3T_CONVD_GO(TB_, NS_)                                                                                            \
    do {                                                                                                                   \
        static bool attr_set = false;                                                                                      \
        if (!attr_set) {                                                                                                   \
            hipError_t ea = hipFuncSetAttribute((const void*)sgemm_x6d_kernel<0, TB_, false, NS_, true>,                   \
                                                hipFuncAttributeMaxDynamicSharedMemorySize, (int)lds);                    \
            if (ea != hipSuccess) return (int)ea;                                                                          \
            attr_set = true;                                                                                               \
        }                                                                                                                  \
        sgemm_x6d_kernel<0, TB_, false, NS_, true><<<grid, block, lds, s>>>(p);                                            \
    } while (0)
    if (anti) {
        if (bf16_operands == 1) M3T_CONVD_GO(0, 1); else if (bf16_operands == 2) M3T_CONVD_GO(0, 2); else M3T_CONVD_GO(0, 3);
    } else {
        if (bf16_operands == 1) M3T_CONVD_GO(1, 1); else if (bf16_operands == 2) M3T_CONVD_GO(1, 2); else M3T_CONVD_GO(1, 3);
    }
#undef M3T_CONVD_GO
    return (int)hipGetLastError();
}
```

### m3f.pytorch_amd/csrc/gemm_x6w.hip

```cpp
#include "common.h"
#include <atomic>
#include <cstdlib>

namespace {

typedef __bf16 bf16x8 __attribute__((ext_vector_type(8)));
typedef __bf16 bf16x2 __attribute__((ext_vector_type(2)));
typedef float f32x2 __attribute__((ext_vector_type(2)));
typedef unsigned u32x2 __attribute__((ext_vector_type(2)));
typedef unsigned u32x4 __attribute__((ext_vector_type(4)));
typedef float f32x4 __attribute__((ext_vector_type(4)));
typedef _Float16 f16x2 __attribute__((ext_vector_type(2)));
typedef _Float16 f16x8 __attribute__((ext_vector_type(8)));

constexpr int WM = 128, WN = 256, WKS = 16, WTH = 256;
constexpr int PLA = WM * 16 + 128;
constexpr int PLB = WN * 16 + 128;
constexpr int planes_of(int NS) { return NS == 4 ? 2 : NS; }
constexpr int opera(int NS) { return planes_of(NS) * 2 * PLA; }
constexpr int operb(int NS) { return planes_of(NS) * 2 * PLB; }
constexpr int stageb(int NS) { return opera(NS) + operb(NS); }
constexpr int TRROWA = WM * 2 + 64, TRROWB = WN * 2 + 64;
constexpr int opera_of(int NS, bool tr) { return tr ? 2 * WKS * TRROWA : opera(NS); }
constexpr int operb_of(int NS, bool tr) { return tr ? 2 * WKS * TRROWB : operb(NS); }
// ... 9 lines not shown
    const unsigned long long* amax_b;
};

template <int NS>
__device__ __forceinline__ void split3_pair(f32x2 v, unsigned (&o)[3], float scale = 1.f) {
    if (NS == 4) {
        const f32x2 vs = v * scale;
        const f16x2 h = __builtin_convertvector(vs, f16x2);
        o[0] = __builtin_bit_cast(unsigned, h);
        const f32x2 r1 = vs - __builtin_convertvector(h, f32x2);
        const f16x2 l = __builtin_convertvector(r1, f16x2);
        o[1] = __builtin_bit_cast(unsigned, l);
        return;
    }
    const bf16x2 h = __builtin_convertvector(v, bf16x2);
    o[0] = __builtin_bit_cast(unsigned, h);
    f32x2 hf;
    hf.x = __uint_as_float(o[0] << 16); hf.y = __uint_as_float(o[0] & 0xffff0000u);
    const f32x2 r1 = v - hf;
    const bf16x2 m = __builtin_convertvector(r1, bf16x2);
    o[1] = __builtin_bit_cast(unsigned, m);
    f32x2 mf;
    mf.x = __uint_as_float(o[1] << 16); mf.y = __uint_as_float(o[1] & 0xffff0000u);
    const f32x2 r2 = r1 - mf;
    const bf16x2 l = __builtin_convertvector(r2, bf16x2);
    o[2] = __builtin_bit_cast(unsigned, l);
}

template <int NS, int NR, int PL>
__device__ __forceinline__ void kc_store_w(unsigned char* __restrict__ S, const f32x4 (&r)[NR], float scale) {
    const int tid = threadIdx.x;
    unsigned char* q = S + ((tid >> 1) & 1) * PL + (tid >> 2) * 16 + (tid & 1) * 8;
#pragma unroll
    for (int i = 0; i < NR; ++i) {
        unsigned lo[3], hi2[3];
        split3_pair<NS>((f32x2){r[i].x, r[i].y}, lo, scale);
        split3_pair<NS>((f32x2){r[i].z, r[i].w}, hi2, scale);
#pragma unroll
        for (int s = 0; s < planes_of(NS); ++s) *reinterpret_cast<u32x2*>(q + s * 2 * PL + i * 1024) = (u32x2){lo[s], hi2[s]};
    }
}
template <int NS, int PL>
__device__ __forceinline__ void mc_store_w(unsigned char* __restrict__ S, const f32x4& r0, const f32x4& r1, float scale, int half) {
    const int tid = threadIdx.x, lane = tid & 63, w = tid >> 6;
    unsigned o[4][3];
    split3_pair<NS>((f32x2){r0.x, r1.x}, o[0], scale);
    split3_pair<NS>((f32x2){r0.y, r1.y}, o[1], scale);
    split3_pair<NS>((f32x2){r0.z, r1.z}, o[2], scale);
    split3_pair<NS>((f32x2){r0.w, r1.w}, o[3], scale);
    unsigned char* q = S + (w >> 1) * PL + (half * 128 + (w & 1) * 64 + (lane & 15) * 4 + (lane >> 4)) * 16;
#pragma unroll
    for (int s = 0; s < planes_of(NS); ++s) {
        const u32x2 p01 = __builtin_amdgcn_permlane16_swap(o[0][s], o[1][s], false, false);
        const u32x2 p23 = __builtin_amdgcn_permlane16_swap(o[2][s], o[3][s], false, false);
        const u32x2 c02 = __builtin_amdgcn_permlane32_swap(p01.x, p23.x, false, false);
        const u32x2 c13 = __builtin_amdgcn_permlane32_swap(p01.y, p23.y, false, false);
        *reinterpret_cast<u32x4*>(q + s * 2 * PL) = (u32x4){c02.x, c13.x, c02.y, c13.y};
    }
}

template <int NS, int ROW>
__device__ __forceinline__ void mc_store_wtr(unsigned char* __restrict__ S, const f32x4& r0, const f32x4& r1, float scale, int half) {
    const int tid = threadIdx.x, lane = tid & 63, w = tid >> 6;
    unsigned char* q = S + (8 * (w >> 1) + 2 * (lane >> 4)) * ROW + (half * 128 + (w & 1) * 64 + (lane & 15) * 4) * 2;
#pragma unroll
    for (int e = 0; e < 2; ++e) {
        const f32x4& r = e ? r1 : r0;
        unsigned a[3], b[3];
        split3_pair<NS>((f32x2){r.x, r.y}, a, scale);
        split3_pair<NS>((f32x2){r.z, r.w}, b, scale);
#pragma unroll
        for (int s = 0; s < planes_of(NS); ++s) *reinterpret_cast<u32x2*>(q + s * WKS * ROW + e * ROW) = (u32x2){a[s], b[s]};
    }
}
template <int ROW>
__device__ __forceinline__ bf16x8 tr_frag(const unsigned char* at) {
    typedef __attribute__((address_space(3))) s16x4 lds_s16x4;
    const s16x4 lo = __builtin_amdgcn_ds_read_tr16_b64_v4i16((lds_s16x4*)(at));
    const s16x4 hi = __builtin_amdgcn_ds_read_tr16_b64_v4i16((lds_s16x4*)(at + 4 * ROW));
    return __builtin_bit_cast(bf16x8, __builtin_shufflevector(lo, hi, 0, 1, 2, 3, 4, 5, 6, 7));
}

template <int TA, int TB, bool SEG, int NS, int BD = 0, bool TR = false>
__global__ __launch_bounds__(WTH, 2) void sgemm_x6w_kernel(X6WParams p) {
    static_assert(!TR || (NS == 4 && !BD), "the transposed-read image is sized for two terms");
    constexpr bool TRA = TR && TA == 1, TRB = TR && TB == 0;
    extern __shared__ __attribute__((aligned(16))) unsigned char ldsb[];
    constexpr int NP = planes_of(NS);
    constexpr int OPA = opera_of(NS, TRA), STG = stageb_of(NS, TA, TB, TR);
    const int tid = threadIdx.x, lane = tid & 63, wave = tid >> 6;
    const int wm = wave >> 1, wn = wave & 1;
    const int l31 = lane & 31, hi = lane >> 5;

    const int tn_ = gridDim.x, nt_ = gridDim.x * gridDim.y;
    const int lin = blockIdx.y * tn_ + blockIdx.x;
    const int xq = nt_ >> 3, xr = nt_ & 7, xcd = lin & 7, slot = lin >> 3;
    const int til = xcd * xq + min(xcd, xr) + slot;
    const int bm = (til / tn_) * WM, bn = (til % tn_) * WN;
    const int k_begin = blockIdx.z * p.kchunk;
    const int k_end = min(p.K, k_begin + p.kchunk);
    const int nst = (k_end - k_begin) / WKS;

    f32x16 acc[2][4];
#pragma unroll
    for (int i = 0; i < 2; ++i)
#pragma unroll
        for (int j = 0; j < 4; ++j)
#pragma unroll
            for (int r = 0; r < 16; ++r) acc[i][j][r] = 0.f;
    float sc_a = 1.f, sc_b = 1.f, sc_ia = 1.f, sc_ib = 1.f;
    if (NS == 4) {
        m3t_f16_scale((unsigned)*p.amax_a, sc_a, sc_ia);
        m3t_f16_scale((unsigned)*p.amax_b, sc_b, sc_ib);
    }

    const float* pa[2]; const float* pb[4];
    size_t a_step, b_step;
    const int mck = 8 * (wave >> 1) + 2 * (lane >> 4);
    const int mcr = (wave & 1) * 64 + (lane & 15) * 4;
    if (TA == 0) {
#pragma unroll
        for (int i = 0; i < 2; ++i) pa[i] = p.A + (size_t)(bm + (tid >> 2) + 64 * i) * p.lda + k_begin + (tid & 3) * 4;
        a_step = WKS;
    } else {
#pragma unroll
        for (int e = 0; e < 2; ++e) pa[e] = p.A + (size_t)(k_begin + mck + e) * p.lda + bm + mcr;
        a_step = (size_t)WKS * p.lda;
    }
    const int wv = __builtin_amdgcn_readfirstlane(wave);
    const unsigned char* bd_src = nullptr;
    if (BD) {
        bd_src = reinterpret_cast<const unsigned char*>(p.B) + ((size_t)(bn / 64 + wv) * (p.K / 8) + k_begin / 8) * 2048 + lane * 16;
        b_step = 0;
    } else if (TB == 1) {
#pragma unroll
        for (int i = 0; i < 4; ++i) pb[i] = p.B + (size_t)(bn + (tid >> 2) + 64 * i) * p.ldb + k_begin + (tid & 3) * 4;
        b_step = WKS;
    } else {
#pragma unroll
        for (int h = 0; h < 2; ++h)
#pragma unroll
            for (int e = 0; e < 2; ++e) pb[2 * h + e] = p.B + (size_t)(k_begin + mck + e) * p.ldb + bn + 128 * h + mcr;
        b_step = (size_t)WKS * p.ldb;
    }
    int srow = 0, sr = 0;
    if (SEG) {
        const int k = k_begin + mck;
        srow = (k / p.seg_len) * p.seg_stride + k % p.seg_len; sr = k % p.seg_len;
        pa[0] = p.A + (size_t)p.a_off * p.lda + bm + mcr;
        pb[0] = p.B + (size_t)p.b_off * p.ldb + bn + mcr;
    }
    f32x4 ra0[2], rb0[4], ra1[2], rb1[4];
    int loaded = 0;
    auto gload = [&](f32x4 (&ra)[2], f32x4 (&rb)[4]) {
        const bool adv = loaded + 1 < nst;
        if (SEG) {
#pragma unroll
            for (int e = 0; e < 2; ++e) {
                const size_t row = (size_t)(srow + e + ((e && sr + 1 >= p.seg_len) ? p.seg_stride - p.seg_len : 0));
                ra[e] = *reinterpret_cast<const f32x4*>(pa[0] + row * p.lda);
                rb[e] = *reinterpret_cast<const f32x4*>(pb[0] + row * p.ldb);
                rb[2 + e] = *reinterpret_cast<const f32x4*>(pb[0] + row * p.ldb + 128);
            }
            if (adv) {
                sr += WKS; srow += WKS;
                if (sr >= p.seg_len) { sr -= p.seg_len; srow += p.seg_stride - p.seg_len; }
            }
        } else {
#pragma unroll
            for (int e = 0; e < 2; ++e) {
                ra[e] = *reinterpret_cast<const f32x4*>(pa[e]);
                pa[e] += adv ? a_step : 0;
            }
            if (!BD) {
#pragma unroll
                for (int e = 0; e < 4; ++e) {
                    rb[e] = *reinterpret_cast<const f32x4*>(pb[e]);
                    pb[e] += adv ? b_step : 0;
                }
            }
        }
        ++loaded;
// ... 26 lines not shown
    const int trk = 8 * hi + ((lane >> 2) & 3), trc = (16 * ((lane >> 4) & 1) + 4 * (lane & 3)) * 2;
    const int fro_a = TRA ? trk * TRROWA + trc + wm * 128 : hi * PLA + (wm * 64 + l31) * 16;
    const int fro_b = OPA + (TRB ? trk * TRROWB + trc + wn * 256 : hi * PLB + (wn * 128 + l31) * 16);
    auto stage = [&](const unsigned char* cur, unsigned char* nxt, const f32x4 (&ua)[2], const f32x4 (&ub)[4]) {
        bf16x8 fa[NP][2], fb[NP][4];
#pragma unroll
        for (int s = 0; s < NP; ++s) {
#pragma unroll
            for (int i = 0; i < 2; ++i) {
                if (TRA) fa[s][i] = tr_frag<TRROWA>(cur + fro_a + s * WKS * TRROWA + i * 64);
                else fa[s][i] = *reinterpret_cast<const bf16x8*>(cur + fro_a + s * 2 * PLA + i * 512);
            }
#pragma unroll
            for (int j = 0; j < 4; ++j) {
                if (TRB) fb[s][j] = tr_frag<TRROWB>(cur + fro_b + s * WKS * TRROWB + j * 64);
                else fb[s][j] = *reinterpret_cast<const bf16x8*>(cur + fro_b + s * 2 * PLB + j * 512);
            }
        }
        sstore(nxt, ua, ub);
#pragma unroll
        for (int i = 0; i < 2; ++i)
#pragma unroll
            for (int j = 0; j < 4; ++j) {
                f32x16 c = acc[i][j];
                if (NS == 4) {
                    c = __builtin_amdgcn_mfma_f32_32x32x16_f16(__builtin_bit_cast(f16x8, fa[1][i]), __builtin_bit_cast(f16x8, fb[0][j]), c, 0, 0, 0);
                    c = __builtin_amdgcn_mfma_f32_32x32x16_f16(__builtin_bit_cast(f16x8, fa[0][i]), __builtin_bit_cast(f16x8, fb[1][j]), c, 0, 0, 0);
                    c = __builtin_amdgcn_mfma_f32_32x32x16_f16(__builtin_bit_cast(f16x8, fa[0][i]), __builtin_bit_cast(f16x8, fb[0][j]), c, 0, 0, 0);
                } else {
#pragma unroll
                    for (int q = 0; q < 6; ++q)
                        c = __builtin_amdgcn_mfma_f32_32x32x16_bf16(fa[PA[q] < NP ? PA[q] : 0][i], fb[PB[q] < NP ? PB[q] : 0][j], c, 0, 0, 0);
                }
                acc[i][j] = c;
            }
    };

    unsigned char* buf0 = ldsb;
    unsigned char* buf1 = ldsb + STG;
    if (BD) {
        if (nst > 0) {
            bdma(buf0);
            gload(ra0, rb0);
            sstore(buf0, ra0, rb0);
            __builtin_amdgcn_sched_barrier(0);
            bdma(buf1);
            __builtin_amdgcn_sched_barrier(0);
            gload(ra1, rb1);
        }
        asm volatile("s_waitcnt vmcnt(2) lgkmcnt(0)\n\ts_barrier" ::: "memory");
        for (int t = 0; t < nst; t += 2) {
            __builtin_amdgcn_sched_barrier(0);
            gload(ra0, rb0);
            stage(buf0, buf1, ra1, rb1);
            asm volatile("s_waitcnt vmcnt(2) lgkmcnt(0)\n\ts_barrier" ::: "memory");
            __builtin_amdgcn_sched_barrier(0);
            bdma(buf0);
            __builtin_amdgcn_sched_barrier(0);
            gload(ra1, rb1);
            stage(buf1, buf0, ra0, rb0);
            asm volatile("s_waitcnt vmcnt(2) lgkmcnt(0)\n\ts_barrier" ::: "memory");
            __builtin_amdgcn_sched_barrier(0);
            bdma(buf1);
            __builtin_amdgcn_sched_barrier(0);
        }
    } else {
    if (nst > 0) {
        gload(ra0, rb0);
        sstore(buf0, ra0, rb0);
        gload(ra1, rb1);
    }
    asm volatile("s_waitcnt lgkmcnt(0)\n\ts_barrier" ::: "memory");
    for (int t = 0; t < nst; t += 2) {
        gload(ra0, rb0);
        stage(buf0, buf1, ra1, rb1);
        asm volatile("s_waitcnt lgkmcnt(0)\n\ts_barrier" ::: "memory");
        gload(ra1, rb1);
        stage(buf1, buf0, ra0, rb0);
        asm volatile("s_waitcnt lgkmcnt(0)\n\ts_barrier" ::: "memory");
    }
    }

    const bool direct = p.splits == 1;
    float* dst = direct ? p.C : p.ws + (size_t)blockIdx.z * p.M * p.N;
    const int ldd = direct ? p.ldc : p.N;
#pragma unroll
    for (int i = 0; i < 2; ++i)
#pragma unroll
        for (int j = 0; j < 4; ++j) {
            const int col = bn + wn * 128 + j * 32 + l31;
            const float bv = (direct && p.bias) ? p.bias[col] : 0.f;
#pragma unroll
            for (int r = 0; r < 16; ++r) {
                const int row = bm + wm * 64 + i * 32 + (r & 3) + 8 * (r >> 2) + 4 * hi;
                float v = acc[i][j][r];
                if (NS == 4) v = v * sc_ia * sc_ib;
                float* q = dst + (size_t)row * ldd + col;
                if (direct) {
                    v += bv;
                    if (p.act == 1) v = m3t_relu(v);
                    if (p.accumulate) v += *q;
                }
                *q = v;
            }
        }
}

}

int m3t_sgemm_x6w_launch(int transA, int transB, int M, int N, int K, const float* A, int lda, const float* B, int ldb,
                         float* C, int ldc, const float* bias, int act, int accumulate, int seg_len, int seg_stride,
                         int a_off, int b_off, float* ws, int splits, int kchunk, int bf16_operands,
                         const unsigned long long* amax_a, const unsigned long long* amax_b, hipStream_t s) {
    if (bf16_operands != 0 && bf16_operands != 3) return M3T_EINVAL;
    if (bf16_operands == 3 && (!amax_a || !amax_b)) return M3T_EINVAL;
    X6WParams p;
    p.amax_a = amax_a; p.amax_b = amax_b;
    p.A = A; p.B = B; p.C = C; p.bias = bias; p.ws = ws;
    p.M = M; p.N = N; p.K = K; p.lda = lda; p.ldb = ldb; p.ldc = ldc;
    p.act = act; p.accumulate = accumulate; p.splits = splits; p.kchunk = kchunk;
    p.seg_len = seg_len; p.seg_stride = seg_stride; p.a_off = a_off; p.b_off = b_off;
    dim3 grid(N / WN, M / WM, splits), block(WTH);
    int dev = 0;
    if (hipGetDevice(&dev) != hipSuccess || dev < 0 || dev >= 32) return M3T_EINVAL;
#define M3T_X6W_GO(TA_, TB_, SEG_, NS_, TR_)                                                                          \
    do {                                                                                                               \
        const size_t lds = 2 * (size_t)stageb_of(NS_, TA_, TB_, TR_);                                                  \
        static std::atomic<unsigned> attr_set{0};                      \
        if (!(attr_set.load(std::memory_order_relaxed) & (1u << dev))) {                                               \
            hipError_t ea = hipFuncSetAttribute((const void*)sgemm_x6w_kernel<TA_, TB_, SEG_, NS_, 0, TR_>,            \
                                                hipFuncAttributeMaxDynamicSharedMemorySize, (int)lds);                \
            if (ea != hipSuccess) return (int)ea;                                                                      \
            attr_set.fetch_or(1u << dev, std::memory_order_relaxed);                                                   \
        }                                                                                                              \
        sgemm_x6w_kernel<TA_, TB_, SEG_, NS_, 0, TR_><<<grid, block, lds, s>>>(p);                                     \
    } while (0)
#define M3T_X6W_DISPATCH(NS_, TR_)                                                                                   \
    do {                                                                                                               \
        if (seg_len > 0) M3T_X6W_GO(1, 0, true, NS_, TR_);                                                             \
        else if (transA == 0 && transB == 1) M3T_X6W_GO(0, 1, false, NS_, false);                                      \
        else if (transA == 0 && transB == 0) M3T_X6W_GO(0, 0, false, NS_, TR_);                                        \
        else if (transA == 1 && transB == 0) M3T_X6W_GO(1, 0, false, NS_, TR_);                                        \
        else M3T_X6W_GO(1, 1, false, NS_, TR_);                                                                        \
    } while (0)
    if (bf16_operands == 3 && m3t_gemm_tr_enabled()) M3T_X6W_DISPATCH(4, true);
    else if (bf16_operands == 3) M3T_X6W_DISPATCH(4, false);
    else M3T_X6W_DISPATCH(3, false);
#undef M3T_X6W_DISPATCH
#undef M3T_X6W_GO
    return (int)hipGetLastError();
}

int m3t_sgemm_x6w_bimg_launch(int M, int N, int K, const float* A, int lda, const float* B_img, float* C, int ldc, const float* bias, int act,
                              int accumulate, float* ws, int splits, int kchunk, const unsigned long long* amax_a,
                              const unsigned long long* amax_b, hipStream_t s) {
    if (!amax_a || !amax_b) return M3T_EINVAL;
    X6WParams p;
    p.amax_a = amax_a; p.amax_b = amax_b;
    p.A = A; p.B = B_img; p.C = C; p.bias = bias; p.ws = ws;
    p.M = M; p.N = N; p.K = K; p.lda = lda; p.ldb = 0; p.ldc = ldc;
    p.act = act; p.accumulate = accumulate; p.splits = splits; p.kchunk = kchunk;
    p.seg_len = p.seg_stride = p.a_off = p.b_off = 0;
    dim3 grid(N / WN, M / WM, splits), block(WTH);
    const size_t lds = 2 * (size_t)stageb(4);
    int dev = 0;
    if (hipGetDevice(&dev) != hipSuccess || dev < 0 || dev >= 32) return M3T_EINVAL;
    static std::atomic<unsigned> attr_set{0};
    if (!(attr_set.load(std::memory_order_relaxed) & (1u << dev))) {
        hipError_t ea = hipFuncSetAttribute((const void*)sgemm_x6w_kernel<0, 1, false, 4, 1>, hipFuncAttributeMaxDynamicSharedMemorySize, (int)lds);
        if (ea != hipSuccess) return (int)ea;
        attr_set.fetch_or(1u << dev, std::memory_order_relaxed);
    }
    sgemm_x6w_kernel<0, 1, false, 4, 1><<<grid, block, lds, s>>>(p);
    return (int)hipGetLastError();
}
```

### m3f.pytorch_amd/m3t/_lib.py

```python
import ctypes as C
import os

_HERE = os.path.dirname(os.path.abspath(__file__))
LIB_PATH = os.environ.get("M3T_LIB_PATH") or os.path.join(os.path.dirname(_HERE), "lib", "libm3t_hip.so")
CSRC_DIR = os.path.join(os.path.dirname(_HERE), "csrc")

M3T_EINVAL = 10001
M3T_ESPIN = 10002
M3T_SCAN_NO_PERSIST = 1
M3T_BF16 = 2
M3T_GEMM_BESIDE_SCAN = 512
M3T_GEMM_F16X3 = 1024
M3T_GEMM_HIGH = 256
M3T_GEMM_EXCLUSIVE = 8
M3T_CONV_IMAGES = 4096
M3T_SCAN_FP32 = 4
M3T_SCAN_WHH = 8
M3T_SCAN_FAULT = 16
M3T_SCAN_WIDE = 32
M3T_MAX_SCANS = 8

_f = C.c_void_p
_i = C.c_int
_z = C.c_size_t
_s = C.c_void_p


class GruFwdDesc(C.Structure):
    _fields_ = [("xproj", _f), ("w_hh", _f), ("b_hh", _f), ("out", _f), ("gates", _f), ("h_n", _f),
                ("H", _i), ("reverse", _i), ("ldx", _i), ("xoff", _i), ("ldo", _i), ("ooff", _i)]


class GruBwdDesc(C.Structure):
    _fields_ = [("dout", _f), ("out", _f), ("gates", _f), ("w_hh_t", _f), ("dh_n", _f),
                ("dgx", _f), ("dgh", _f), ("dh", _f), ("db_part", _f), ("db_ih", _f), ("db_hh", _f),
                ("H", _i), ("reverse", _i), ("ldo", _i), ("ooff", _i), ("ldg", _i), ("goff", _i), ("amax", _f), ("wfrag", _f)]


class WindowProblem(C.Structure):
    _fields_ = [("A", _f), ("B", _f), ("C", _f), ("bias", _f), ("amax_a", _f), ("amax_b", _f), ("accumulate", _i)]


class AttDecArgs(C.Structure):
    _fields_ = [(n, _f) for n in ("enc", "P", "h0", "w_a", "v", "w_ih", "w_hh", "b_ih", "b_hh", "w_o", "b_o", "y0", "trg", "tf",
                                  "out", "h_last", "G", "alpha", "a_save", "x", "gates", "hs", "dout", "dh_last", "dgi", "dgh",
                                  "dc", "da", "dy", "dP", "dv_acc", "dh", "dy0", "w_iht", "wt", "dyin", "dhz")] + \
        [(n, _i) for n in ("B", "T", "L", "H", "save")]


M3T_WINDOW_BATCH = 8

SIGNATURES = {
    "m3t_version": [],
    "m3t_device_arch": [C.c_char_p, _i],
    "m3t_sgemm": [_i, _i, _i, _i, _i, _f, _i, _f, _i, _f, _i, _f, _i, _i, _i, _i, _i, _i, _f, _z, _i, _s],
    "m3t_sgemm_scaled": [_i, _i, _i, _i, _i, _f, _i, _f, _i, _f, _i, _f, _i, _i, _i, _i, _i, _i, _f, _z, _i, _f, _f, _s],
    "m3t_sgemm_window": [_i, _i, _i, _i, _i, _i, _i, _f, _i, _f, _i, _f, _i, _f, _i, _i, _i, _f, _f, _s],
    "m3t_sgemm_window_batch": [_i, C.POINTER(WindowProblem), _i, _i, _i, _i, _i, _i, _i, _i, _i, _i, _i, _i, _s],
    "m3t_absmax": [_i, C.POINTER(C.c_void_p), C.POINTER(C.c_size_t), C.POINTER(C.c_int), C.POINTER(C.c_size_t), C.POINTER(C.c_void_p), _s],
    "m3t_sgemm_plan": [_i, _i, _i, _i, _i, _z, _i, C.POINTER(C.c_int), C.POINTER(C.c_int)],
    "m3t_im2col3d": [_f] + [_i] * 14 + [_f, C.c_longlong, _i, C.c_void_p, _s],
    "m3t_conv3d_taps": [_f, _f, _f] + [_i] * 17 + [_f, _f, _f, _z, _f, _s],
    "m3t_sgemm_pre": [_i, _i, _i, _f, _i, _f, _i, _f, _i, _f, _i, _i, _f, _f, _s],
    "m3t_f16x3_split": [_f, _z, _i, _z, _f, _z, _f, _s],
    "m3t_f16x3_split_perm": [_f, _z, _i, _i, _z, _z, _z, _f, _f, _s],
    "m3t_f16x3_image_b": [_f, _i, _i, _z, _f, _f, _s],
    "m3t_sgemm_bimg": [_i, _i, _i, _f, _i, _f, _f, _i, _f, _i, _i, _f, _z, _f, _f, _s],
    "m3t_sgemm_ring": [_i, _i, _i, _i, _i, _f, _i, _f, _i, _f, _i, _f, _i, _i, _i, _i, _i, _i, _f, _z, _i, _f, _f, _i, _s],
    "m3t_conv3d_taps_pre": [_f, _f, _f] + [_i] * 16 + [_f, _f, _f, _z, _f, _s],
    "m3t_conv3d_fwd_taps": [_f, _f, _f, _f] + [_i] * 15 + [_f, _f, _f, _z, _f, _s],
    "m3t_conv3d_fwd_taps4": [_f, _f, _f, _f] + [_i] * 14 + [_f, _f, _f, _z, _f, _s],
    "m3t_planes_to_cl4": [_f, _f, _i, _i, C.c_longlong, _s],
    "m3t_conv3d_wgrad_taps": [_f, _f, _f] + [_i] * 16 + [_f, _f, _f, _z, _s],
    "m3t_amax_out": [C.c_void_p],
    "m3t_colsum": [_f, _i, _i, _i, _f, _i, _f, _z, _s],
    "m3t_transpose": [_f, _i, _i, _i, _f, _i, _s],
    "m3t_relu_bwd": [_f, _f, _z, _s],
    "m3t_gru_scan_fwd": [C.POINTER(GruFwdDesc), _i, _i, _i, _f, _z, _i, _s],
    "m3t_gru_scan_bwd": [C.POINTER(GruBwdDesc), _i, _i, _i, _f, _z, _i, _s],
    "m3t_gru_bwd_prepare_floats": [_i],
    "m3t_gru_bwd_prepare": [C.POINTER(C.c_void_p), _i, _i, _i, C.POINTER(C.c_void_p), _s],
    "m3t_gru_persist_count": [],
    "m3t_gru_scan_workgroups": [_i, _i, _i, _i, _i, _i],
    "m3t_gru_poll_error": [],
    "m3t_gru_error_reset": [],
    "m3t_gru_error_defer": [_i],
    "m3t_gru_inject_error": [_s],
    "m3t_gru_persist_owner": [],
    "m3t_gru_scan_arena": [C.c_void_p, _z],
    "m3t_gru_scan_arena_reset": [C.c_void_p],
    "m3t_gru_scan_after": [C.c_void_p],
    "m3t_gru_scan_progress": [C.c_void_p, _i, C.POINTER(C.c_int), C.POINTER(C.c_uint)],
    "m3t_gru_scan_progress_reset": [C.c_void_p],
    "m3t_gru_scan_progress_ok": [_i, _i, _i, _i, _i, _i],
    "m3t_stream_wait_progress": [C.c_void_p, C.c_uint, _s],
    "m3t_gru_scan_events": [C.c_void_p, C.c_void_p],
    "m3t_gru_persist_profile": [C.c_void_p],
    "m3t_att_fuse_fwd": [_f, _f, _f, _f, _f, _i, _i, _s],
    "m3t_att_fuse_bwd": [_f, _f, _f, _f, _f, _f, _f, _f, _f, _i, _i, _s],
    "m3t_bn_cl_ws_bytes": [_z, _i],
    "m3t_bn_cl_fwd": [_f, _z, _i, _f, _f, _f, _f, C.c_float, C.c_float, _i, _i, _f, _f, _f, _f, _z, _s],
    "m3t_bn_cl_bwd": [_f, _f, _f, _f, _f, _f, _z, _i, _i, _i, _f, _f, _f, _f, _f, _z, _s],
    "m3t_bn_pool_cl_fwd": [_f, _z, _i, _i, _i, _i, _f, _f, _f, _f, C.c_float, C.c_float, _i, _f, C.c_void_p, _f, _f, _f, _z, _s],
    "m3t_bn_pool_cl_bwd": [_f, _f, _f, C.c_void_p, _f, _f, _f, _z, _i, _i, _i, _i, _i, _f, _f, _f, _f, _f, _z, _s],
    "m3t_pool_cl_fwd": [_f, _z, _i, _i, _i, _i, _i, _i, _i, _i, _i, _f, C.c_void_p, _s],
    "m3t_pool_cl_bwd": [_f, C.c_void_p, _z, _i, _i, _i, _i, _i, _i, _i, _i, _i, _f, _s],
    "m3t_va_loss": [_f, _i, _i, _i, _i, _f, _f, _f, _f, _i, C.c_float, C.c_float, C.c_float, _i, _f, _f, _f, _z, _s],
    "m3t_va_loss_ws_bytes": [_i],
    "m3t_weight_norm_fwd": [_f, _f, _f, _f, _i, _i, _i, _s],
    "m3t_weight_norm_bwd": [_f, _f, _f, _f, _f, _f, _i, _i, _i, _s],
    "m3t_causal_conv_fwd": [_f, _f, _f, _f, _f, _f, _f, _i, _i, _i, _i, _i, _i, _i, _i, _s],
    "m3t_causal_conv_wgrad": [_f, _f, _f, _i, _i, _i, _i, _i, _i, _f, _z, _s],
    "m3t_conv1d_fwd": [_f, _f, _f, _f, _f, _f, _f, _i, _i, _i, _i, _i, _i, _i, _i, _i, C.c_float, C.c_ulonglong, _i, _s],
    "m3t_conv1d_fwd_scaled": [_f, _f, _f, _f, _f, _f, _f, _i, _i, _i, _i, _i, _i, _i, _i, _i, C.c_float, C.c_ulonglong, _i, _f, _f, _s],
    "m3t_conv1d_wgrad": [_f, _f, _f, _i, _i, _i, _i, _i, _i, _i, _f, _z, _i, _s],
    "m3t_conv1d_wgrad_scaled": [_f, _f, _f, _i, _i, _i, _i, _i, _i, _i, _f, _z, _i, _f, _f, _s],
    "m3t_pool_planes_fwd": [_f, C.c_longlong, _i, _i, _i, _i, _i, _i, _i, _i, _f, C.c_void_p, _s],
    "m3t_pool_planes_bwd": [_f, C.c_void_p, C.c_longlong, _i, _i, _i, _i, _i, _i, _i, _i, _f, _s],
    "m3t_bn_planes_ws_bytes": [_i, _i, _i],
    "m3t_bn_planes_fwd": [_f, _i, _i, _i, _f, _f, _f, _f, C.c_float, C.c_float, _i, _i, _f, _f, _f, _f, _z, _s],
    "m3t_bn_planes_bwd": [_f, _f, _f, _f, _f, _f, _i, _i, _i, _i, _i, _f, _f, _f, _f, _z, _s],
    "m3t_bn_rows_ws_bytes": [_i, _i],
    "m3t_bn_rows_fwd": [_f, _i, _i, _f, _f, _f, _f, C.c_float, C.c_float, _i, _i, _f, _f, _f, _f, _z, _s],
    "m3t_bn_rows_bwd": [_f, _f, _f, _f, _f, _f, _i, _i, _i, _i, _f, _f, _f, _f, _z, _s],
    "m3t_bct_to_btc": [_f, _f, _i, _i, _i, _s],
    "m3t_bct_to_btc_sums": [_f, _f, _i, _i, _i, _f, _s],
    "m3t_bct_to_btc_img": [_f, _f, _i, _i, _i, C.c_void_p, _f, _s],
    "m3t_btc_to_bct": [_f, _f, _i, _i, _i, _s],
    "m3t_mask_pos": [_f, _f, _f, _f, _z, _s],
    "m3t_add_relu": [_f, _f, _f, _z, _s],
    "m3t_mask_pos_drop": [_f, _f, _f, _i, _i, C.c_float, C.c_ulonglong, _s],
    "m3t_cbam_channel_fwd": [_f, _f, _f, _f, _f, _f, _f, _f, _f, _f, _i, _i, _i, _i, _s],
    "m3t_cbam_channel_bwd": [_f, _f, _f, _f, _f, _f, _f, _f, _f, _f, _f, _f, _f, _i, _i, _i, _i, _f, _z, _s],
    "m3t_cbam_spatial_fwd": [_f, _f, _f, _f, _f, _f, _f, _f, _f, _f, _i, _i, _i, _i, _i, C.c_float, C.c_float, _f, _z, _s],
    "m3t_cbam_spatial_bwd": [_f, _f, _f, _f, _f, _f, _f, _f, _f, _f, _f, _f, _i, _i, _i, _i, _i, _f, _z, _s],
    "m3t_cbam_fused_ok": [_i, _i, _i, _i],
    "m3t_cbam_fused_ws_bytes": [_i, _i, _i, _i, _i],
    "m3t_cbam_fwd": [_f] * 20 + [_i] * 6 + [C.c_float, C.c_float, _f, _z, _s],
    "m3t_cbam_bwd": [_f] * 23 + [_i] * 6 + [_f, _z, _s],
    "m3t_smooth_tracks": [_f, _f, _i, _i, _i, _f, _s],
    "m3t_ccc_masked": [_f, _f, _f, C.c_longlong, _i, _f, _s],
# ... 92 lines not shown
```

### m3f.pytorch_amd/m3t/ops.py

```python
import ctypes as C
import os
import sys

import torch

from . import _lib
from ._lib import GruFwdDesc, GruBwdDesc, M3T_MAX_SCANS, M3THipError

_WS = {}
_WS_MIN = 64 << 20

PROFILE = []

import weakref

_GRAD_SINKS = {}


def register_grad_sink(param, view, owner=None):
    _GRAD_SINKS[id(param)] = [weakref.ref(param), view, False, id(owner) if owner is not None else None]


def clear_grad_sinks(owner=None):
    if owner is None:
# ... 182 lines not shown

def wgrad_joined(device):
    _WGRAD_PENDING[(device.type, device.index)] = False


def wgrad_stream(device, i=0):
    key = (device.type, device.index)
    sts = _WGRAD.get(key)
    if sts is None:
        sts = [torch.cuda.Stream(device=device) for _ in range(_N_WGRAD)]
        _WGRAD[key] = sts
        for i_, st_ in enumerate(sts):
            _ROLE_OF_HANDLE[(st_.device.index, st_.cuda_stream)] = "wgrad%d" % i_
            _wait_slot_fill(st_, key)
    return sts[i % min(2, len(sts))]


def wgrad_streams(device):
    wgrad_stream(device)
    return _WGRAD[(device.type, device.index)]


def live_streams(device):
    key = (device.type, device.index)
    return ([_SIDE[key]] if key in _SIDE else []) + list(_WGRAD.get(key) or [])


_ROLE_OF_HANDLE = {}


def _ws_tag(device):
    if _RAW_STREAM is not None and device.index is not None:
        return _ROLE_OF_HANDLE.get((device.index, _RAW_STREAM(device.index)), "main")
    cur = cur_stream(device)
    st = _SIDE.get((device.type, device.index))
    if st is not None and cur == st:
        return "side"
    for i, st in enumerate(_WGRAD.get((device.type, device.index)) or []):
        if cur == st:
            return "wgrad%d" % i
    return "main"


def workspace(device, nbytes=_WS_MIN, tag=None):
    key = (device.type, device.index, tag or _ws_tag(device))
    ws = _WS.get(key)
    if ws is None or ws.numel() * 4 < nbytes:
        ws = torch.empty(max(nbytes, _WS_MIN) // 4, dtype=torch.float32, device=device)
        _WS[key] = ws
    return ws


_PREC = [_lib.M3T_GEMM_F16X3]


class precision:

    def __init__(self, mode):
        if mode not in ("fp32", "x6", "high", "bf16"):
            raise ValueError("precision mode must be 'fp32', 'x6', 'high' or 'bf16'")
        self.flag = {"fp32": _lib.M3T_GEMM_F16X3, "x6": 0, "high": _lib.M3T_GEMM_HIGH, "bf16": _lib.M3T_BF16}[mode]

    def __enter__(self):
        self.prev = _PREC[0]
        _PREC[0] = self.flag
        return self

    def __exit__(self, *exc):
        _PREC[0] = self.prev
        return False


def sgemm(transA, transB, M, N, K, A, a_off, lda, B, b_off, ldb, Cm, c_off, ldc, bias=None, act=0,
          accumulate=False, seg=(0, 0, 0, 0), use_ws=True, prec=None, exclusive=False, amax=(None, None)):
    ws = workspace(Cm.device) if use_ws else None
    flags = (_PREC[0] if prec is None else prec) | (_lib.M3T_GEMM_EXCLUSIVE if exclusive else 0)
    if _FENCED[0]:
        flags |= _lib.M3T_GEMM_BESIDE_SCAN
    with _Timed("sgemm_kernel", 1, 2.0 * M * N * K) if PROFILE_GEMM[0] else _NULL:
        rc = lib().m3t_sgemm_scaled(transA, transB, M, N, K, _p(A, a_off), lda, _p(B, b_off), ldb, _p(Cm, c_off), ldc,
                                    _p(bias), act, int(accumulate), seg[0], seg[1], seg[2], seg[3],
                                    _p(ws), (ws.numel() * 4) if ws is not None else 0, flags, amax[0], amax[1], _stream())
    _lib.check(rc, "m3t_sgemm")


_AMAX_ONE = {}


def amax_one(device):
    key = (device.type, device.index)
    t = _AMAX_ONE.get(key)
    if t is None:
        t = _AMAX_ONE[key] = torch.full((1,), 0x3F800000, dtype=torch.int64, device=device)
    return t.data_ptr()


_SLOT_POOL = {}
_SLOT_CHUNK = 8192


def amax_slots(n, device):
    key = (device.type, device.index)
    st = _SLOT_POOL.get(key)
    if st is None or st[1] + n > st[0].numel():
        st = _SLOT_POOL[key] = [torch.zeros(max(_SLOT_CHUNK, n), dtype=torch.int64, device=device), 0]
        if device.type == "cuda":
            ev = torch.cuda.Event()
            ev.record(cur_stream(device))
            others = ([_SIDE.get(key)] if _SIDE.get(key) is not None else []) + list(_WGRAD.get(key) or [])
            for other in others:
                other.wait_event(ev)
            st.append(ev)
            st.append({cur_stream(device).cuda_stream} | {o.cuda_stream for o in others})
    if len(st) > 3 and device.type == "cuda":
        h = _RAW_STREAM(device.index if device.index is not None else _CUR_DEV()) if _RAW_STREAM is not None else None
        if h is not None and h not in st[3]:
            cur_stream(device).wait_event(st[2])
            st[3].add(h)
    v = st[0][st[1]:st[1] + n]
    st[1] += n
    return v


_W_AMAX = {}
_W_AMAX_ON = os.environ.get("M3T_WEIGHT_AMAX", "1") != "0"
_W_GEN = [0]


def weights_changed():
    _W_GEN[0] += 1


invalidate_weight_amax = weights_changed


def measure_weight_amax(params, owner=None):
    if not _W_AMAX_ON:
        return
    ws = [p for p in params if p.dim() >= 2 and p.is_cuda and p.dtype == torch.float32 and p.is_contiguous()
          and (p.numel() // p.shape[0]) % 4 == 0 and p.data_ptr() % 16 == 0]
    if not ws:
        return
    slots = amax_slots(len(ws), ws[0].device)
    if measure_amax([(p.detach().view(p.shape[0], -1), slots.data_ptr() + 8 * i) for i, p in enumerate(ws)]):
        for i, p in enumerate(ws):
            _W_AMAX[id(p)] = (weakref.ref(p), slots.data_ptr() + 8 * i, id(owner), slots, p._version, p.data_ptr(), _W_GEN[0])


def drop_weight_amax(owner=None):
    for k in [k for k, e in _W_AMAX.items() if owner is None or e[2] == id(owner)]:
        del _W_AMAX[k]


def weight_amax(w, keep=None):
    e = _W_AMAX.get(id(w))
    if e is None or e[0]() is not w:
        return _frozen_weight_amax(w, keep)
    if e[4] != w._version or e[5] != w.data_ptr() or e[6] != _W_GEN[0]:
        del _W_AMAX[id(w)]
        return None
    if keep is not None and not any(k is e[3] for k in keep):
        keep.append(e[3])
    return e[1]


_W_AMAX_FROZEN = {}
# ... 535 lines not shown


_CONCURRENT_ENABLED = os.environ.get("M3T_SCAN_CONCURRENT", "1") != "0"
_CUS = {}


def _pair_fits(dev, n_heavy, H_heavy, n_light, H_light, B, T, prec):
    if not _CONCURRENT_ENABLED:
        return False
    key = (dev.type, dev.index)
    cus = _CUS.get(key)
    if cus is None:
        cus = _CUS[key] = torch.cuda.get_device_properties(dev).multi_processor_count
    base = _scan_flags(dev) | prec
    if base & _lib.M3T_SCAN_NO_PERSIST:
        return False
    for bwd in (0, 1):
        a = lib().m3t_gru_scan_workgroups(n_heavy, H_heavy, B, T, base | _lib.M3T_SCAN_WIDE, bwd)
        b = lib().m3t_gru_scan_workgroups(n_light, H_light, B, T, base | _lib.M3T_SCAN_WIDE, bwd)
        if a <= 0 or b <= 0 or a + b > cus or (a + 7) // 8 + (b + 7) // 8 > cus // 8:
            return False
    return True


class _MultiBiGRU(torch.autograd.Function):

    @staticmethod
    def forward(ctx, n_stacks, L, cat_lo, cat_hi, unit_mask, *tensors):
        per = 1 + 8 * L
        assert len(tensors) == n_stacks * per
        xs, params = [], []
        for s in range(n_stacks):
            xs.append(_req(tensors[s * per].contiguous(), "x"))
            params.append([_req(t, "gru parameter") for t in tensors[s * per + 1:(s + 1) * per]])
        B, T = xs[0].shape[0], xs[0].shape[1]
        dev = xs[0].device
        for x in xs:
            if x.shape[0] != B or x.shape[1] != T:
                raise M3THipError("grouped GRU stacks must share batch and length")
        Hs = [params[s][1].shape[1] for s in range(n_stacks)]
        new = lambda *shape: torch.empty(*shape, dtype=torch.float32, device=dev)
        h_ns = [new(2 * L, B, Hs[s]) for s in range(n_stacks)]
        outs = [[new(B, T, 2 * Hs[s]) for s in range(n_stacks)] for _ in range(L)]
        cat_buf = None
        if cat_hi - cat_lo >= 2:
            cat_buf = new(B, T, sum(2 * Hs[s] for s in range(cat_lo, cat_hi)))
            off = 0
            for s in range(cat_lo, cat_hi):
                outs[L - 1][s] = cat_buf[..., off:off + 2 * Hs[s]]
                off += 2 * Hs[s]
        gates = [[new(2, B, T, 4 * Hs[s]) for s in range(n_stacks)] for _ in range(L)]
        xprojs = [[new(B, T, 6 * Hs[s]) for s in range(n_stacks)] for _ in range(L)]
        main = cur_stream()
        prec = _PREC[0]
        groups = _stream_groups(Hs, B)
        fslots = None
        if (prec & _lib.M3T_GEMM_F16X3) and all(h % 4 == 0 for h in Hs):
            fslots = amax_slots(n_stacks * (1 + 2 * L), dev)
            items = [(xs[s], fslots.data_ptr() + 8 * s) for s in range(n_stacks) if not (unit_mask >> s) & 1]
            wslot = {}
            ctx.w_keep = []
            for l in range(L):
                for s in range(n_stacks):
                    for d in (0, 1):
                        a = weight_amax(params[s][(2 * l + d) * 4], ctx.w_keep)
                        if a is None:
                            a = fslots.data_ptr() + 8 * (n_stacks + (l * n_stacks + s) * 2 + d)
                            items.append((params[s][(2 * l + d) * 4], a))
                        wslot[(l, s, d)] = a
            if not measure_amax(items):
                fslots = None
        one = amax_one(dev)

        def fslot_x(l, s):
            return None if fslots is None else (fslots.data_ptr() + 8 * s if (l == 0 and not (unit_mask >> s) & 1) else one)

        def fslot_w(l, s, d):
            return None if fslots is None else wslot[(l, s, d)]

        alone = not _interleaved(groups) and all(kind == "main" for kind, _ in groups)

        def level_fwd(l, idxs, scan, after=None, wide=False, progress=None):
            descs = []
            for s in idxs:
                H = Hs[s]
                inp = xs[s] if l == 0 else outs[l - 1][s]
                I = inp.shape[-1]
                for d in (0, 1):
                    w_ih, w_hh, b_ih, b_hh = params[s][(2 * l + d) * 4:(2 * l + d) * 4 + 4]
                    if not scan:
                        sgemm(0, 1, B * T, 3 * H, I, inp, 0, I, w_ih, 0, I, xprojs[l][s], d * 3 * H, 6 * H, bias=b_ih, prec=prec,
                              exclusive=alone, amax=(fslot_x(l, s), fslot_w(l, s, d)))
                    else:
                        descs.append(GruFwdDesc(_vp(xprojs[l][s]), _vp(w_hh), _vp(b_hh), _vp(outs[l][s]),
                                                _vp(gates[l][s], d * B * T * 4 * H), _vp(h_ns[s], (2 * l + d) * B * H),
                                                H, d, 6 * H, d * 3 * H, outs[l][s].stride(1), d * H))
            if scan:
                return _scan_fwd(descs, B, T, prec | (_lib.M3T_SCAN_WIDE if (wide or FORCE_WIDE_FWD[0]) else 0), after,
                                 None if progress is None else (_progress_counters(dev), progress))

        def chunk_plan(idxs, wide):
            if L < 2 or fslots is None or len({Hs[i] for i in idxs}) != 1 or 2 * len(idxs) > M3T_MAX_SCANS:
                return None
            H = Hs[idxs[0]]
            if H % 64 != 0:
                return None
            fl = _scan_flags(dev) | prec | (_lib.M3T_SCAN_WIDE if (wide or FORCE_WIDE_FWD[0]) else 0)
            if not lib().m3t_gru_scan_progress_ok(2 * len(idxs), H, B, T, fl, 0):
                return None
            return _chunk_bounds(B, T)

        def proj_pieces(l, idxs, tb, need, scan_stream):
            wg = wgrad_stream(dev, 0)
            ctr = _progress_counters(dev)
            ev_end = torch.cuda.Event()
            ev_end.record(scan_stream)
            lo, hi = [0] + tb, tb + [T]
            with on_stream(wg):
                ended = False
                for dirn, k, w, second in _arrivals(tb, T):
                    if k is None:
                        if not ended:
                            wg.wait_event(ev_end)
                            ended = True
                    else:
                        _wait_progress(ctr, dirn, need[dirn * len(tb) + k])
                    H = Hs[idxs[0]]
                    lda = outs[l - 1][idxs[0]].stride(1)
                    probs = []
                    for si in idxs:
                        src = outs[l - 1][si]
                        assert src.stride(1) == lda
                        for d in (0, 1):
                            w_ih, _, b_ih, _ = params[si][(2 * l + d) * 4:(2 * l + d) * 4 + 4]
                            probs.append((src, dirn * H, w_ih, dirn * H, xprojs[l][si], d * 3 * H, None if second else b_ih, second,
                                          one, fslot_w(l, si, d)))
                    sgemm_window_batch(probs, 1, B, hi[w] - lo[w], T, lo[w], 3 * H, H, lda, 2 * H, 6 * H, prec=prec)
                ev = torch.cuda.Event()
                ev.record(wg)
            scan_stream.wait_event(ev)

        concurrent = (_interleaved(groups) and len({Hs[i] for i in groups[0][1]}) == 1 and len({Hs[i] for i in groups[1][1]}) == 1
                      and _pair_fits(dev, 2 * len(groups[0][1]), Hs[groups[0][1][0]], 2 * len(groups[1][1]), Hs[groups[1][1][0]], B, T, prec))
        if concurrent:
            heavy, light = groups[0][1], groups[1][1]
            side = side_stream(dev)
            side.wait_stream(main)
            _FENCED[0] = True
            try:
                tb = chunk_plan(heavy, True)
                if tb is not None:
                    wgrad_stream(dev, 0).wait_stream(main)
                for l in range(L):
                    if l == 0 or tb is None:
                        level_fwd(l, heavy, False)
                    ev_al = None
                    if ALIGN_LIGHT[0] and l > 0:
                        ev_al = torch.cuda.Event()
                        ev_al.record(main)
                    with on_stream(side):
                        level_fwd(l, light, False)
                        level_fwd(l, light, True, ev_al, True)
                    need = level_fwd(l, heavy, True, None, True, tb if l + 1 < L else None)
                    if tb is not None and l + 1 < L:
                        proj_pieces(l + 1, heavy, tb, need, main)
            finally:
# ... 211 lines not shown
                            wg.wait_event(ev_end)
                            ended = True
                    else:
                        _wait_progress(ctr, dirn, need[dirn * n + k])
                    d = 1 - dirn
                    j = w if dirn == 0 else n - w
                    by_shape = {}
                    for si in idxs:
                        if need_dx[l][si]:
                            I = layer_io(l, si)[0].shape[-1]
                            by_shape.setdefault(I, []).append((dgx[l][si], d * 3 * Hs[si], params[si][(2 * l + d) * 4], 0, dinp[l][si], 0, None,
                                                               second, bslot(l, si, d, j), fslot_w(l, si, d)))
                    for I, probs in by_shape.items():
                        H = Hs[idxs[0]]
                        sgemm_window_batch(probs, 0, B, hi[w] - lo[w], T, lo[w], I, 3 * H, 6 * H, I, I, prec=prec)
                ev = torch.cuda.Event()
                ev.record(wg)
            scan_stream.wait_event(ev)
            for si in idxs:
                if need_dx[l][si]:
                    cur[si] = dinp[l][si]

        def start_marks(idxs):
            if not SCAN_FIRST[0] or bslots is None or len({Hs[i] for i in idxs}) != 1 or 2 * len(idxs) > M3T_MAX_SCANS or T < 64 or not direct_whh:
                return None
            fl = _scan_flags(dev) | prec | _lib.M3T_SCAN_WHH | _lib.M3T_SCAN_WIDE
            if not lib().m3t_gru_scan_progress_ok(2 * len(idxs), Hs[idxs[0]], B, T, fl, 1):
                return None
            return [8, T - 8]

        held = {}

        def release_held(key, started):
            fn = held.pop(key, None)
            if fn is None:
                return
            if started is not None:
                ctr_, need_ = started
                with on_stream(wgs[0]):
                    _wait_progress(ctr_, 0, need_[0])
                    _wait_progress(ctr_, 1, need_[2])
            fn()

        def level_scan(l, idxs, after=None, wide=False, progress=None):
            descs = []
            for s in idxs:
                H = Hs[s]
                inp, out, gts = layer_io(l, s)
                for d in (0, 1):
                    w_hh = params[s][(2 * l + d) * 4 + 1]
                    if not direct_whh:
                        _lib.check(lib().m3t_transpose(_p(w_hh), 3 * H, H, H, _p(wht[l][s][d]), 3 * H, _stream()),
                                   "m3t_transpose")
                    base = s * per + 1 + (2 * l + d) * 4
                    descs.append(GruBwdDesc(_vp(cur[s]), _vp(out), _vp(gts, d * B * T * 4 * H),
                                            _vp(w_hh if direct_whh else wht[l][s][d]),
                                            _vp(dhns[s], (2 * l + d) * B * H) if dhns[s] is not None else None,
                                            _vp(dgx[l][s]), _vp(dgh[l][s], d * B * T * 3 * H), _vp(dh[l][s], d * B * H),
                                            _vp(dbp[l][s], d * B * 4 * H), _vp(out_grads[base + 2]), _vp(out_grads[base + 3]),
                                            H, d, out.stride(1), d * H, 6 * H, d * 3 * H, bslot(l, s, d),
                                            _vp(wfq[(l, s, d)]) if (l, s, d) in wfq else None))
            chain = _ws_tag(dev)
            sm = None
            if progress is None and chain in held:
                sm = start_marks(idxs)
            need = _scan_bwd(descs, B, T, prec | (_lib.M3T_SCAN_WHH if direct_whh else 0) | _lib.M3T_SCAN_WIDE, after,
                             None if (progress is None and sm is None) else (_progress_counters(dev), progress if progress is not None else sm))
            if progress is not None:
                pending[(l, tuple(idxs))] = (progress, need)
            release_held(chain, (_progress_counters(dev), need) if sm is not None else None)
            if RANGE_PROBE[0] is not None:
                for s in idxs:
                    for d in (0, 1):
                        _probe_range("dgx l%d s%d d%d H%d" % (l, s, d, Hs[s]), dgx[l][s].view(B * T, 6 * Hs[s])[:, d * 3 * Hs[s]:(d + 1) * 3 * Hs[s]])
                        _probe_range("dgh l%d s%d d%d H%d" % (l, s, d, Hs[s]), dgh[l][s][d].view(B * T, 3 * Hs[s]))

        pending = {}

        def level_dx(l, idxs):
            pg = pending.pop((l, tuple(idxs)), None)
            if pg is not None:
                dx_pieces(l, idxs, pg[0], pg[1], cur_stream())
                return
            for s in idxs:
                H = Hs[s]
                inp, out, gts = layer_io(l, s)
                I = inp.shape[-1]
                if need_dx[l][s]:
                    for d in (0, 1):
                        sgemm(0, 0, B * T, I, 3 * H, dgx[l][s], d * 3 * H, 6 * H, params[s][(2 * l + d) * 4], 0, I,
                              dinp[l][s], 0, I, accumulate=(d == 1), prec=prec, amax=(bslot(l, s, d), fslot_w(l, s, d)))
                    cur[s] = dinp[l][s]

        wgs = wgrad_streams(dev)
        rr = [0]

        def _level_dw(l, idxs, pool):
            for s in idxs:
                H = Hs[s]
                inp, out, gts = layer_io(l, s)
                I = inp.shape[-1]
                for d in (0, 1):
                    base = s * per + 1 + (2 * l + d) * 4
                    dw_ih, dw_hh = out_grads[base:base + 2]
                    goff = d * B * T * 3 * H
                    with (on_stream(pool[rr[0] % len(pool)]) if pool is not None else _NULL):
                        if T > 1:
                            a_off, b_off = (1, 0) if d == 0 else (0, 1)
                            sgemm(1, 0, 3 * H, H, B * (T - 1), dgh[l][s], goff, 3 * H, out, d * H, out.stride(1), dw_hh, 0, H,
                                  seg=(T - 1, T, a_off, b_off), prec=prec, amax=(bslot(l, s, d), one if bslots is not None else None))
                        else:
                            dw_hh.zero_()
                    rr[0] += 1
                    with (on_stream(pool[rr[0] % len(pool)]) if pool is not None else _NULL):
                        sgemm(1, 0, 3 * H, I, B * T, dgx[l][s], d * 3 * H, 6 * H, inp, 0, I, dw_ih, 0, I, prec=prec,
                              amax=(bslot(l, s, d), fslot_x(l, s)))
                    rr[0] += 1

        def level_dw(l, idxs, spread=False, wg_i=0):
            if spread:
                _level_dw(l, idxs, [cur_stream(), wgs[1]])
            else:
                with on_stream(wgs[wg_i]):
                    _level_dw(l, idxs, None)

        light_idxs = groups[1][1] if (LIGHT_DW_STREAM1[0] and ctx.concurrent and _interleaved(groups)) else None

        for w_ in wgs:
            w_.wait_stream(main)

        def level_gemms(l, idxs, last=False):
            level_dx(l, idxs)
            ev = torch.cuda.Event()
            ev.record(cur_stream())
            wg_i = 1 if (light_idxs is not None and list(idxs) == list(light_idxs)) else 0
            for w_ in (wgs if last else [wgs[wg_i]]):
                w_.wait_event(ev)
            if last or not SCAN_FIRST[0]:
                level_dw(l, idxs, spread=last, wg_i=wg_i)
            else:
                held[_ws_tag(dev)] = lambda: level_dw(l, idxs, spread=False, wg_i=wg_i)

        if ctx.concurrent and _interleaved(groups):
            heavy, light = groups[0][1], groups[1][1]
            side = side_stream(dev)
            side.wait_stream(main)
            _FENCED[0] = True
            try:
                for l in range(L - 1, -1, -1):
                    ev_al = None
                    if ALIGN_LIGHT[0] and _ALIGN_BWD and l < L - 1:
                        ev_al = torch.cuda.Event()
                        ev_al.record(main)
                    level_scan(l, heavy, None, True, chunk_plan(l, heavy))
                    with on_stream(side):
                        level_scan(l, light, ev_al)
                    level_gemms(l, heavy, last=(l == 0))
                    with on_stream(side):
                        level_gemms(l, light, last=(l == 0))
            finally:
                _FENCED[0] = False
            main.wait_stream(side)
        elif _interleaved(groups):
            heavy, light = groups[0][1], groups[1][1]
            side = side_stream(dev)
            side.wait_stream(main)
            ev_light = None
            _FENCED[0] = True
            try:
                if L == 2:
                    level_scan(1, heavy, None)
                    ev_h1 = torch.cuda.Event()
                    ev_h1.record(main)
                    level_gemms(1, heavy)
                    with on_stream(side):
                        level_scan(1, light, ev_h1)
                        ev_l1 = torch.cuda.Event()
                        ev_l1.record(side)
                        level_gemms(1, light)
                    level_scan(0, heavy, ev_l1)
# ... 2044 lines not shown
```

Before: 2830.

## Batch same-shape GRU projection and dgrad GEMMs into single grouped launches

Adds a batched scaled-GEMM entry point that runs up to eight same-shape f16x3 GEMMs in one launch, with the batch index folded into grid z alongside split-K, plus a batched split-K reduction. The forward input projections and the backward dx GEMMs across streams and directions are grouped by shape and routed through it; dw batching exists but is off by default. The aim is to cut launch count and fill the GPU better with small GEMMs. In exchange the splits are chosen per problem while several problems share one workspace, which can force smaller pieces, and the forward level now returns before the old path.

```diff
diff --git a/include/m3t_hip.h b/include/m3t_hip.h
--- a/include/m3t_hip.h
+++ b/include/m3t_hip.h
@@ -89,6 +89,11 @@
 } m3t_window_problem;
 int m3t_sgemm_window_batch(int n, const m3t_window_problem* problems, int transB, int n_seg, int win_len, int win_stride, int win_off,
                            int N, int K, int lda, int ldb, int ldc, int act, int flags, void* stream);
+
+int m3t_sgemm_scaled_batch(int n, const m3t_window_problem* problems, int transA, int transB, int M, int N, int K, int lda, int ldb, int ldc,
+                           int act, int seg_len, int seg_stride, int a_off, int b_off, float* ws, size_t ws_bytes, int flags, void* stream);
+int m3t_sgemm_batch_plan(int n, int transA, int transB, int M, int N, int K, int seg_len, size_t ws_bytes, int flags, int* batched,
+                         int* splits, int* pieces);
 
 int m3t_absmax(int n, const float* const* x, const size_t* rows, const int* cols, const size_t* ld,
                unsigned long long* const* slots, void* stream);
diff --git a/m3f.pytorch_amd/csrc/gemm.hip b/m3f.pytorch_amd/csrc/gemm.hip
--- a/m3f.pytorch_amd/csrc/gemm.hip
+++ b/m3f.pytorch_amd/csrc/gemm.hip
@@ -300,6 +300,39 @@
     }
 }
 
+struct ReduceBatch { float* C[M3T_WINDOW_BATCH]; const float* bias[M3T_WINDOW_BATCH]; int accumulate[M3T_WINDOW_BATCH]; };
+__global__ __launch_bounds__(256) void splitk_reduce4_batch_kernel(const float* __restrict__ ws, ReduceBatch rb, int M, int N, int ldc, int splits,
+                                                                   int act) {
+    const size_t total4 = (size_t)M * N / 4;
+    const int z = blockIdx.y;
+    const float4* w4 = reinterpret_cast<const float4*>(ws) + (size_t)z * splits * total4;
+    float* __restrict__ C = rb.C[z];
+    const float* __restrict__ bias = rb.bias[z];
+    const int accumulate = rb.accumulate[z];
+    const int n4 = N / 4;
+    for (size_t i = blockIdx.x * (size_t)blockDim.x + threadIdx.x; i < total4; i += (size_t)gridDim.x * blockDim.x) {
+        float4 s = make_float4(0.f, 0.f, 0.f, 0.f);
+        int k = 0;
+        for (; k + 8 <= splits; k += 8) {
+            float4 v[8];
+#pragma unroll
+            for (int u = 0; u < 8; ++u) v[u] = w4[(size_t)(k + u) * total4 + i];
+#pragma unroll
+            for (int u = 0; u < 8; ++u) { s.x += v[u].x; s.y += v[u].y; s.z += v[u].z; s.w += v[u].w; }
+        }
+        for (; k < splits; ++k) {
+            const float4 v = w4[(size_t)k * total4 + i];
+            s.x += v.x; s.y += v.y; s.z += v.z; s.w += v.w;
+        }
+        const int m = (int)(i / n4), n = (int)(i % n4) * 4;
+        if (bias) { s.x += bias[n]; s.y += bias[n + 1]; s.z += bias[n + 2]; s.w += bias[n + 3]; }
+        if (act == 1) { s.x = m3t_relu(s.x); s.y = m3t_relu(s.y); s.z = m3t_relu(s.z); s.w = m3t_relu(s.w); }
+        float4* q = reinterpret_cast<float4*>(C + (size_t)m * ldc + n);
+        if (accumulate) { const float4 c = *q; s.x += c.x; s.y += c.y; s.z += c.z; s.w += c.w; }
+        *q = s;
+    }
+}
+
 
 constexpr int ABSMAX_REGIONS = 16;
 struct AbsmaxArgs { M3TRegion r[ABSMAX_REGIONS]; };
@@ -648,6 +681,38 @@
     return g;
 }
 
+enum { GEMM_ON_FP32 = 0, GEMM_ON_X6W = 1, GEMM_ON_X6D = 2, GEMM_ON_X6 = 3 };
+struct GemmRoute { GemmPlan g; int splits, kchunk, f16x3, which; };
+static GemmRoute route_gemm(int transA, int transB, int M, int N, int K, int seg_len, bool vec, size_t ws_bytes, int flags) {
+    GemmRoute r;
+    const GemmPlan g = plan_gemm(transA, M, N, K, seg_len, vec, ws_bytes, flags | ((transA == 0 && transB == 1) ? 0 : GEMM_NO_WIDE));
+    int splits = g.splits, kchunk = g.kchunk;
+    {
+        static int beside_wgs = -1;
+        if (beside_wgs < 0) { const char* e = getenv("M3T_GEMM_BESIDE_WGS"); beside_wgs = e ? atoi(e) : 384; }
+        if (beside_wgs > 0 && (flags & M3T_GEMM_BESIDE_SCAN) && g.kernel != 0 && !g.wide && g.splits > 1) {
+            const int tiles = cdiv(M, BM) * cdiv(N, g.narrow ? 64 : BN);
+            int sp = (beside_wgs + tiles / 2) / tiles;
+            if (sp < 1) sp = 1;
+            if (sp < g.splits) {
+                kchunk = cdiv(cdiv(K, sp), 32) * 32;
+                splits = cdiv(K, kchunk);
+            }
+        }
+    }
+    const int bf16 = (flags & M3T_GEMM_BF16) ? 1 : 0;
+    const int f16x3 = (!bf16 && !(flags & M3T_GEMM_HIGH) && (flags & M3T_GEMM_F16X3) && m3t_f16x3_enabled()) ? 1 : 0;
+    const bool wide_tr = f16x3 && !g.wide && !g.narrow && !(transA == 0 && transB == 1) && !(flags & M3T_GEMM_BACKGROUND) && N % 256 == 0 &&
+                         K % 32 == 0 && x6w_enabled() && m3t_gemm_tr_enabled() && tr_wide_wins(flags);
+    r.g = g; r.splits = splits; r.kchunk = kchunk; r.f16x3 = f16x3;
+    if (g.kernel == 0) r.which = GEMM_ON_FP32;
+    else if (g.wide || wide_tr) r.which = GEMM_ON_X6W;
+    else if (!g.narrow && K % 32 == 0 && (!f16x3 || f16x3_on_x6d()) && !(flags & (M3T_GEMM_BACKGROUND | M3T_GEMM_HIGH)) && (x6d_mode() == 1 || (x6d_mode() == 2 && !(flags & M3T_GEMM_BESIDE_SCAN))))
+        r.which = GEMM_ON_X6D;
+    else r.which = GEMM_ON_X6;
+    return r;
+}
+
 extern "C" int m3t_sgemm_plan(int transA, int M, int N, int K, int seg_len, size_t ws_bytes, int flags, int* kernel, int* splits) {
     if (M <= 0 || N <= 0 || K < 0 || !kernel || !splits) return M3T_EINVAL;
     const GemmPlan g = plan_gemm(transA, M, N, K, seg_len, true, ws_bytes, flags | (transA ? GEMM_NO_WIDE : 0));
@@ -678,29 +743,14 @@
     p.vecA = (lda % 4 == 0) && ((uintptr_t)A % 16 == 0);
     p.vecB = (ldb % 4 == 0) && ((uintptr_t)B % 16 == 0);
     const int tm = cdiv(M, BM), tn = cdiv(N, BN);
-    const GemmPlan g = plan_gemm(transA, M, N, K, seg_len, p.vecA && p.vecB, ws ? ws_bytes : 0,
-                                 flags | ((transA == 0 && transB == 1) ? 0 : GEMM_NO_WIDE));
-    int splits = g.splits, kchunk = g.kchunk;
-    {
-        static int beside_wgs = -1;
-        if (beside_wgs < 0) { const char* e = getenv("M3T_GEMM_BESIDE_WGS"); beside_wgs = e ? atoi(e) : 384; }
-        if (beside_wgs > 0 && (flags & M3T_GEMM_BESIDE_SCAN) && g.kernel != 0 && !g.wide && g.splits > 1) {
-            const int tiles = cdiv(M, BM) * cdiv(N, g.narrow ? 64 : BN);
-            int sp = (beside_wgs + tiles / 2) / tiles;
-            if (sp < 1) sp = 1;
-            if (sp < g.splits) {
-                kchunk = cdiv(cdiv(K, sp), 32) * 32;
-                splits = cdiv(K, kchunk);
-            }
-        }
-    }
+    const GemmRoute rt = route_gemm(transA, transB, M, N, K, seg_len, p.vecA && p.vecB, ws ? ws_bytes : 0, flags);
+    const GemmPlan g = rt.g;
+    const int splits = rt.splits, kchunk = rt.kchunk;
     p.splits = splits; p.kchunk = kchunk;
     hipStream_t s = (hipStream_t)stream;
     if (g.kernel != 0) {
         int rc;
-        const int f16x3 = (!p.bf16 && !(flags & M3T_GEMM_HIGH) && (flags & M3T_GEMM_F16X3) && m3t_f16x3_enabled()) ? 1 : 0;
-        const bool wide_tr = f16x3 && !g.wide && !g.narrow && !(transA == 0 && transB == 1) && !(flags & M3T_GEMM_BACKGROUND) && N % 256 == 0 &&
-                             K % 32 == 0 && x6w_enabled() && m3t_gemm_tr_enabled() && tr_wide_wins(flags);
+        const int f16x3 = rt.f16x3;
         const unsigned long long* use_a = nullptr; const unsigned long long* use_b = nullptr;
         if (f16x3) {
             const size_t kr = seg_len > 0 ? (size_t)(K / seg_len - 1) * seg_stride + seg_len : (size_t)K;
@@ -711,10 +761,10 @@
             const int rm = m3t_f16x3_measure(ra, amax_a, rb, amax_b, &use_a, &use_b, s);
             if (rm) return rm;
         }
-        if (g.wide || wide_tr)
+        if (rt.which == GEMM_ON_X6W)
             rc = m3t_sgemm_x6w_launch(transA, transB, M, N, K, A, lda, B, ldb, C, ldc, bias, act, accumulate, seg_len, seg_stride,
                                       a_off, b_off, ws, splits, kchunk, f16x3 ? 3 : 0, use_a, use_b, s);
-        else if (!g.narrow && K % 32 == 0 && (!f16x3 || f16x3_on_x6d()) && !(flags & (M3T_GEMM_BACKGROUND | M3T_GEMM_HIGH)) && (x6d_mode() == 1 || (x6d_mode() == 2 && !(flags & M3T_GEMM_BESIDE_SCAN))))
+        else if (rt.which == GEMM_ON_X6D)
             rc = m3t_sgemm_x6d_launch(transA, transB, M, N, K, A, lda, B, ldb, C, ldc, bias, act, accumulate, seg_len, seg_stride,
                                       a_off, b_off, ws, splits, kchunk, p.bf16 ? 1 : ((flags & M3T_GEMM_HIGH) ? 2 : (f16x3 ? 3 : 0)), use_a, use_b, s);
         else
@@ -747,6 +797,90 @@
     if (splits > 1) {
         launch_splitk_reduce(ws, C, bias, M, N, ldc, splits, act, accumulate, s);
         M3T_LAUNCH_CHECK();
+    }
+    return 0;
+}
+
+int m3t_sgemm_x6w_batch_launch(int n, const m3t_window_problem* pr, int transA, int transB, int M, int N, int K, int lda, int ldb, int ldc,
+                               int act, int seg_len, int seg_stride, int a_off, int b_off, float* ws, int splits, int kchunk, hipStream_t s);
+int m3t_sgemm_x6d_batch_launch(int n, const m3t_window_problem* pr, int transA, int transB, int M, int N, int K, int lda, int ldb, int ldc,
+                               int act, int seg_len, int seg_stride, int a_off, int b_off, float* ws, int splits, int kchunk, hipStream_t s);
+int m3t_sgemm_x6_batch_launch(int n, const m3t_window_problem* pr, int transA, int transB, int M, int N, int K, int lda, int ldb, int ldc,
+                              int act, int seg_len, int seg_stride, int a_off, int b_off, float* ws, int splits, int kchunk, int narrow,
+                              hipStream_t s);
+
+static void plan_batch(int n, int transA, int transB, int M, int N, int K, int seg_len, int ldc, bool aligned, bool c_vec, size_t ws_bytes, int flags,
+                       GemmRoute& rt, int& batched, int& per) {
+    rt = route_gemm(transA, transB, M, N, K, seg_len, aligned, ws_bytes, flags);
+    batched = 0; per = 1;
+    if (!aligned || rt.which == GEMM_ON_FP32 || !rt.f16x3 || (flags & M3T_GEMM_BACKGROUND)) return;
+    if (rt.splits > 1) {
+        const size_t total = (size_t)M * N;
+        int blocks = (int)((total / 4 + 255) / 256);
+        if (blocks > 4096) blocks = 4096;
+        if (!(N % 4 == 0 && ldc % 4 == 0 && c_vec) || (rt.splits >= 4 * SK_FOLD && blocks <= 64)) return;
+        const size_t fit = ws_bytes / ((size_t)rt.splits * total * sizeof(float));
+        if (fit < 1) return;
+        per = fit < (size_t)n ? (int)fit : n;
+    } else per = n;
+    batched = 1;
+}
+
+extern "C" int m3t_sgemm_batch_plan(int n, int transA, int transB, int M, int N, int K, int seg_len, size_t ws_bytes, int flags, int* batched,
+                                    int* splits, int* pieces) {
+    if (n < 1 || n > M3T_WINDOW_BATCH || M <= 0 || N <= 0 || K < 0 || !batched || !splits || !pieces) return M3T_EINVAL;
+    GemmRoute rt; int b, per;
+    plan_batch(n, transA, transB, M, N, K, seg_len, N, true, true, ws_bytes, flags, rt, b, per);
+    *batched = b; *splits = rt.splits; *pieces = b ? cdiv(n, per) : n;
+    return 0;
+}
+
+extern "C" int m3t_sgemm_scaled_batch(int n, const m3t_window_problem* pr, int transA, int transB, int M, int N, int K, int lda, int ldb, int ldc,
+                                      int act, int seg_len, int seg_stride, int a_off, int b_off, float* ws, size_t ws_bytes, int flags,
+                                      void* stream) {
+    if (n <= 0 || M <= 0 || N <= 0) return 0;
+    if (n > M3T_WINDOW_BATCH || !pr || K < 0) return M3T_EINVAL;
+    if (seg_len > 0 && !(transA == 1 && transB == 0)) return M3T_EINVAL;
+    bool aligned = (lda % 4 == 0) && (ldb % 4 == 0), c_vec = true;
+    for (int i = 0; i < n; ++i) {
+        if (!pr[i].A || !pr[i].B || !pr[i].C) return M3T_EINVAL;
+        aligned = aligned && (uintptr_t)pr[i].A % 16 == 0 && (uintptr_t)pr[i].B % 16 == 0 && pr[i].amax_a && pr[i].amax_b;
+        c_vec = c_vec && (uintptr_t)pr[i].C % 16 == 0;
+    }
+    if (!ws) ws_bytes = 0;
+    c_vec = c_vec && (uintptr_t)ws % 16 == 0;
+    GemmRoute rt; int batched, per;
+    plan_batch(n, transA, transB, M, N, K, seg_len, ldc, aligned, c_vec, ws_bytes, flags, rt, batched, per);
+    if (!batched) {
+        for (int i = 0; i < n; ++i) {
+            const int rc = m3t_sgemm_scaled(transA, transB, M, N, K, pr[i].A, lda, pr[i].B, ldb, pr[i].C, ldc, pr[i].bias, act, pr[i].accumulate,
+                                            seg_len, seg_stride, a_off, b_off, ws, ws_bytes, flags, pr[i].amax_a, pr[i].amax_b, stream);
+            if (rc) return rc;
+        }
+        return 0;
+    }
+    hipStream_t s = (hipStream_t)stream;
+    for (int i = 0; i < n; i += per) {
+        const int cnt = n - i < per ? n - i : per;
+        int rc;
+        if (rt.which == GEMM_ON_X6W)
+            rc = m3t_sgemm_x6w_batch_launch(cnt, pr + i, transA, transB, M, N, K, lda, ldb, ldc, act, seg_len, seg_stride, a_off, b_off, ws,
+                                            rt.splits, rt.kchunk, s);
+        else if (rt.which == GEMM_ON_X6D)
+            rc = m3t_sgemm_x6d_batch_launch(cnt, pr + i, transA, transB, M, N, K, lda, ldb, ldc, act, seg_len, seg_stride, a_off, b_off, ws,
+                                            rt.splits, rt.kchunk, s);
+        else
+            rc = m3t_sgemm_x6_batch_launch(cnt, pr + i, transA, transB, M, N, K, lda, ldb, ldc, act, seg_len, seg_stride, a_off, b_off, ws,
+                                           rt.splits, rt.kchunk, rt.g.narrow, s);
+        if (rc) return rc;
+        if (rt.splits > 1) {
+            ReduceBatch rb = {};
+            for (int j = 0; j < cnt; ++j) { rb.C[j] = pr[i + j].C; rb.bias[j] = pr[i + j].bias; rb.accumulate[j] = pr[i + j].accumulate; }
+            int blocks = (int)(((size_t)M * N / 4 + 255) / 256);
+            if (blocks > 4096) blocks = 4096;
+            splitk_reduce4_batch_kernel<<<dim3(blocks, cnt), 256, 0, s>>>(ws, rb, M, N, ldc, rt.splits, act);
+            M3T_LAUNCH_CHECK();
+        }
     }
     return 0;
 }
diff --git a/m3f.pytorch_amd/csrc/gemm_x6.hip b/m3f.pytorch_amd/csrc/gemm_x6.hip
--- a/m3f.pytorch_amd/csrc/gemm_x6.hip
+++ b/m3f.pytorch_amd/csrc/gemm_x6.hip
@@ -168,14 +168,17 @@
     return __builtin_bit_cast(bf16x8, __builtin_shufflevector(lo, hi, 0, 1, 2, 3, 4, 5, 6, 7));
 }
 
-template <int TA, int TB, bool SEG, int NS, bool CONV = false, int XNT = 128, bool MW = false, int C3 = 0, int PRE = 0, bool TR = false>
+template <int TA, int TB, bool SEG, int NS, bool CONV = false, int XNT = 128, bool MW = false, int C3 = 0, int PRE = 0, bool TR = false, bool BT = false>
 __global__ __launch_bounds__(256, 3) void sgemm_x6_kernel(X6Params p, X6Batch bt) {
     static_assert(!TR || NS == 4, "the transposed-read image is sized for two terms");
+    static_assert(!BT || !MW, "a window batch has no split-K slabs");
     constexpr bool TRA = TR && TA == 1, TRB = TR && TB == 0;
-    if (MW) {
-        const int z = blockIdx.z;
+    int zk = blockIdx.z;
+    if (MW || BT) {
+        const int z = BT ? blockIdx.z / p.splits : blockIdx.z;
         p.A = bt.A[z]; p.B = bt.B[z]; p.C = bt.C[z]; p.bias = bt.bias[z];
         p.amax_a = bt.amax_a[z]; p.amax_b = bt.amax_b[z]; p.accumulate = bt.accumulate[z];
+        if (BT) { zk = blockIdx.z - z * p.splits; p.ws += (size_t)z * p.splits * p.M * p.N; }
     }
     constexpr int NJ = XNT / 64;
     constexpr int BR = XNT / 32;
@@ -192,7 +195,7 @@
     const int til = xcd * xq + min(xcd, xr) + slot;
     const int bm = (til / tn_) * XM, bn = (til % tn_) * XNT;
     const bool bcol = XNT == 128 || (tid & 31) < 16;
-    const int k_begin = MW ? 0 : blockIdx.z * p.kchunk;
+    const int k_begin = MW ? 0 : zk * p.kchunk;
     const int k_end = min(p.K, k_begin + p.kchunk);
     const int ntiles = (C3 == 2 || SEG) ? (k_end - k_begin + XK - 1) / XK : (k_end - k_begin) / XK;
     __shared__ int rowmap[MW ? XM : 1];
@@ -440,7 +443,7 @@
     }
 
     const bool direct = p.splits == 1;
-    float* dst = direct ? p.C : p.ws + (size_t)blockIdx.z * p.M * p.N;
+    float* dst = direct ? p.C : p.ws + (size_t)zk * p.M * p.N;
     const int ldd = direct ? p.ldc : p.N;
     if constexpr (C3 == 1 || C3 == 3) {
         if (direct && p.tr_S > 0) {
@@ -551,6 +554,42 @@
 #undef M3T_X6_DISPATCH
     hipError_t e = hipGetLastError();
     return (int)e;
+}
+
+int m3t_sgemm_x6_batch_launch(int n, const m3t_window_problem* pr, int transA, int transB, int M, int N, int K, int lda, int ldb, int ldc,
+                              int act, int seg_len, int seg_stride, int a_off, int b_off, float* ws, int splits, int kchunk, int narrow,
+                              hipStream_t s) {
+    if (n < 1 || n > M3T_WINDOW_BATCH || splits < 1) return M3T_EINVAL;
+    X6Params p;
+    X6Batch bt = {};
+    for (int i = 0; i < n; ++i) {
+        if (!pr[i].amax_a || !pr[i].amax_b) return M3T_EINVAL;
+        bt.A[i] = pr[i].A; bt.B[i] = pr[i].B; bt.C[i] = pr[i].C; bt.bias[i] = pr[i].bias;
+        bt.amax_a[i] = pr[i].amax_a; bt.amax_b[i] = pr[i].amax_b; bt.accumulate[i] = pr[i].accumulate;
+    }
+    p.amax_a = p.amax_b = nullptr;
+    p.A = p.B = nullptr; p.C = nullptr; p.bias = nullptr; p.ws = ws;
+    p.M = M; p.N = N; p.K = K; p.lda = lda; p.ldb = ldb; p.ldc = ldc;
+    p.act = act; p.accumulate = 0; p.splits = splits; p.kchunk = kchunk;
+    p.seg_len = seg_len; p.seg_stride = seg_stride; p.a_off = a_off; p.b_off = b_off;
+    p.cv_T = p.cv_C = p.cv_K = p.cv_dil = p.cv_lead = p.cv_anti = 0; p.cv_btap = 0; p.cv_mask = p.cv_res = nullptr; p.cv_pre = nullptr;
+    p.cv_drop = m3t_make_drop(0.f, 0ull);
+    p.cv_amax = nullptr;
+    p.mw_len = p.mw_stride = p.mw_off = 0;
+    p.c3_T = p.c3_H = p.c3_W = p.c3_To = p.c3_Ho = p.c3_Wo = p.c3_kt = p.c3_kh = p.c3_kw = p.c3_bt = p.c3_bh = p.c3_bw = p.c3_sg = p.c3_C = 0; p.c3_st = p.c3_sh = p.c3_sw = 1; p.tr_S = 0;
+    dim3 grid(N / (narrow ? 64 : XN), M / XM, n * splits), block(256);
+#define M3T_X6B_DISPATCH(XNT_, TR_)                                                                                                           \
+    do {                                                                                                                                      \
+        if (seg_len > 0) sgemm_x6_kernel<1, 0, true, 4, false, XNT_, false, 0, 0, TR_, true><<<grid, block, 0, s>>>(p, bt);                    \
+        else if (transA == 0 && transB == 1) sgemm_x6_kernel<0, 1, false, 4, false, XNT_, false, 0, 0, false, true><<<grid, block, 0, s>>>(p, bt); \
+        else if (transA == 0 && transB == 0) sgemm_x6_kernel<0, 0, false, 4, false, XNT_, false, 0, 0, TR_, true><<<grid, block, 0, s>>>(p, bt);   \
+        else if (transA == 1 && transB == 0) sgemm_x6_kernel<1, 0, false, 4, false, XNT_, false, 0, 0, TR_, true><<<grid, block, 0, s>>>(p, bt);   \
+        else sgemm_x6_kernel<1, 1, false, 4, false, XNT_, false, 0, 0, TR_, true><<<grid, block, 0, s>>>(p, bt);                               \
+    } while (0)
+    if (m3t_gemm_tr_enabled()) { if (narrow) M3T_X6B_DISPATCH(64, true); else M3T_X6B_DISPATCH(128, true); }
+    else { if (narrow) M3T_X6B_DISPATCH(64, false); else M3T_X6B_DISPATCH(128, false); }
+#undef M3T_X6B_DISPATCH
+    return (int)hipGetLastError();
 }
 
 int m3t_sgemm_x6_window_launch(int n, const m3t_window_problem* pr, int transB, int M, int N, int K, int lda, int ldb, int ldc,
diff --git a/m3f.pytorch_amd/csrc/gemm_x6d.hip b/m3f.pytorch_amd/csrc/gemm_x6d.hip
--- a/m3f.pytorch_amd/csrc/gemm_x6d.hip
+++ b/m3f.pytorch_amd/csrc/gemm_x6d.hip
@@ -119,7 +119,7 @@
 }
 
 template <int TA, int TB, bool SEG, int NS, bool CONV = false, bool TR = false>
-__global__ __launch_bounds__(NTH, 3) void sgemm_x6d_kernel(X6DParams p) {
+__device__ __forceinline__ void x6d_body(const X6DParams& p, const int zk) {
     static_assert(!TR || NS == 4, "the transposed-read image is sized for two terms");
     constexpr bool TRA = TR && TA == 1, TRB = TR && TB == 0;
     extern __shared__ __attribute__((aligned(16))) unsigned char ldsb[];
@@ -132,7 +132,7 @@
     const int xq = nt_ >> 3, xr = nt_ & 7, xcd = lin & 7, slot = lin >> 3;
     const int til = xcd * xq + min(xcd, xr) + slot;
     const int bm = (til / tn_) * BM, bn = (til % tn_) * BN;
-    const int k_begin = blockIdx.z * p.kchunk;
+    const int k_begin = zk * p.kchunk;
     const int k_end = min(p.K, k_begin + p.kchunk);
     const int nst = (k_end - k_begin) / BKS;
 
@@ -297,7 +297,7 @@
     }
 
     const bool direct = p.splits == 1;
-    float* dst = direct ? p.C : p.ws + (size_t)blockIdx.z * p.M * p.N;
+    float* dst = direct ? p.C : p.ws + (size_t)zk * p.M * p.N;
     const int ldd = direct ? p.ldc : p.N;
 #pragma unroll
     for (int i = 0; i < 2; ++i)
@@ -329,6 +329,21 @@
                 *q = v;
             }
         }
+}
+
+template <int TA, int TB, bool SEG, int NS, bool CONV = false, bool TR = false>
+__global__ __launch_bounds__(NTH, 3) void sgemm_x6d_kernel(X6DParams p) {
+    x6d_body<TA, TB, SEG, NS, CONV, TR>(p, blockIdx.z);
+}
+
+struct X6DBatch { m3t_window_problem pr[M3T_WINDOW_BATCH]; };
+template <int TA, int TB, bool SEG, bool TR>
+__global__ __launch_bounds__(NTH, 3) void sgemm_x6d_batch_kernel(X6DParams p, X6DBatch bt) {
+    const int z = blockIdx.z / p.splits, zk = blockIdx.z - z * p.splits;
+    p.A = bt.pr[z].A; p.B = bt.pr[z].B; p.C = bt.pr[z].C; p.bias = bt.pr[z].bias;
+    p.amax_a = bt.pr[z].amax_a; p.amax_b = bt.pr[z].amax_b; p.accumulate = bt.pr[z].accumulate;
+    p.ws += (size_t)z * p.splits * p.M * p.N;
+    x6d_body<TA, TB, SEG, 4, false, TR>(p, zk);
 }
 
 }
@@ -378,6 +393,51 @@
 }
 
 
+int m3t_sgemm_x6d_batch_launch(int n, const m3t_window_problem* pr, int transA, int transB, int M, int N, int K, int lda, int ldb, int ldc,
+                               int act, int seg_len, int seg_stride, int a_off, int b_off, float* ws, int splits, int kchunk, hipStream_t s) {
+    if (n < 1 || n > M3T_WINDOW_BATCH || splits < 1) return M3T_EINVAL;
+    X6DBatch bt = {};
+    for (int i = 0; i < n; ++i) {
+        if (!pr[i].amax_a || !pr[i].amax_b) return M3T_EINVAL;
+        bt.pr[i] = pr[i];
+    }
+    X6DParams p;
+    p.amax_a = p.amax_b = nullptr;
+    p.A = p.B = nullptr; p.C = nullptr; p.bias = nullptr; p.ws = ws;
+    p.M = M; p.N = N; p.K = K; p.lda = lda; p.ldb = ldb; p.ldc = ldc;
+    p.act = act; p.accumulate = 0; p.splits = splits; p.kchunk = kchunk;
+    p.seg_len = seg_len; p.seg_stride = seg_stride; p.a_off = a_off; p.b_off = b_off;
+    p.cv_T = p.cv_C = p.cv_K = p.cv_dil = p.cv_lead = p.cv_anti = 0; p.cv_btap = 0; p.cv_mask = p.cv_res = nullptr; p.cv_pre = nullptr;
+    p.cv_drop = m3t_make_drop(0.f, 0ull);
+    dim3 grid(N / BN, M / BM, n * splits), block(NTH);
+    const size_t lds = 2 * (size_t)STAGEB;
+#define M3T_X6DB_GO(TA_, TB_, SEG_, TR_)                                                                              \
+    do {                                                                                                               \
+        static bool attr_set = false;                                                                                  \
+        if (!attr_set) {                                                                                               \
+            hipError_t ea = hipFuncSetAttribute((const void*)sgemm_x6d_batch_kernel<TA_, TB_, SEG_, TR_>,              \
+                                                hipFuncAttributeMaxDynamicSharedMemorySize, (int)lds);                \
+            if (ea != hipSuccess) return (int)ea;                                                                      \
+            attr_set = true;                                                                                           \
+        }                                                                                                              \
+        sgemm_x6d_batch_kernel<TA_, TB_, SEG_, TR_><<<grid, block, lds, s>>>(p, bt);                                   \
+    } while (0)
+#define M3T_X6DB_DISPATCH(TR_)                                                                                       \
+    do {                                                                                                               \
+        if (seg_len > 0) M3T_X6DB_GO(1, 0, true, TR_);                                                                 \
+        else if (transA == 0 && transB == 1) M3T_X6DB_GO(0, 1, false, false);                                          \
+        else if (transA == 0 && transB == 0) M3T_X6DB_GO(0, 0, false, TR_);                                            \
+        else if (transA == 1 && transB == 0) M3T_X6DB_GO(1, 0, false, TR_);                                            \
+        else M3T_X6DB_GO(1, 1, false, TR_);                                                                            \
+    } while (0)
+    if (m3t_gemm_tr_enabled()) M3T_X6DB_DISPATCH(true);
+    else M3T_X6DB_DISPATCH(false);
+#undef M3T_X6DB_DISPATCH
+#undef M3T_X6DB_GO
+    return (int)hipGetLastError();
+}
+
+
 int m3t_conv_x6d_launch(const float* x, const float* w_t, const float* bias, const float* res, const float* mask, float* y,
                         float* pre, int B, int T, int Ci, int Co, int K, int dil, int lead, int act, int anti, int bf16_operands,
                         M3TDrop drop, hipStream_t s) {
diff --git a/m3f.pytorch_amd/csrc/gemm_x6w.hip b/m3f.pytorch_amd/csrc/gemm_x6w.hip
--- a/m3f.pytorch_amd/csrc/gemm_x6w.hip
+++ b/m3f.pytorch_amd/csrc/gemm_x6w.hip
@@ -115,7 +115,7 @@
 }
 
 template <int TA, int TB, bool SEG, int NS, int BD = 0, bool TR = false>
-__global__ __launch_bounds__(WTH, 2) void sgemm_x6w_kernel(X6WParams p) {
+__device__ __forceinline__ void x6w_body(const X6WParams& p, const int zk) {
     static_assert(!TR || (NS == 4 && !BD), "the transposed-read image is sized for two terms");
     constexpr bool TRA = TR && TA == 1, TRB = TR && TB == 0;
     extern __shared__ __attribute__((aligned(16))) unsigned char ldsb[];
@@ -130,7 +130,7 @@
     const int xq = nt_ >> 3, xr = nt_ & 7, xcd = lin & 7, slot = lin >> 3;
     const int til = xcd * xq + min(xcd, xr) + slot;
     const int bm = (til / tn_) * WM, bn = (til % tn_) * WN;
-    const int k_begin = blockIdx.z * p.kchunk;
+    const int k_begin = zk * p.kchunk;
     const int k_end = min(p.K, k_begin + p.kchunk);
     const int nst = (k_end - k_begin) / WKS;
 
@@ -323,7 +323,7 @@
     }
 
     const bool direct = p.splits == 1;
-    float* dst = direct ? p.C : p.ws + (size_t)blockIdx.z * p.M * p.N;
+    float* dst = direct ? p.C : p.ws + (size_t)zk * p.M * p.N;
     const int ldd = direct ? p.ldc : p.N;
 #pragma unroll
     for (int i = 0; i < 2; ++i)
@@ -345,6 +345,21 @@
                 *q = v;
             }
         }
+}
+
+template <int TA, int TB, bool SEG, int NS, int BD = 0, bool TR = false>
+__global__ __launch_bounds__(WTH, 2) void sgemm_x6w_kernel(X6WParams p) {
+    x6w_body<TA, TB, SEG, NS, BD, TR>(p, blockIdx.z);
+}
+
+struct X6WBatch { m3t_window_problem pr[M3T_WINDOW_BATCH]; };
+template <int TA, int TB, bool SEG, bool TR>
+__global__ __launch_bounds__(WTH, 2) void sgemm_x6w_batch_kernel(X6WParams p, X6WBatch bt) {
+    const int z = blockIdx.z / p.splits, zk = blockIdx.z - z * p.splits;
+    p.A = bt.pr[z].A; p.B = bt.pr[z].B; p.C = bt.pr[z].C; p.bias = bt.pr[z].bias;
+    p.amax_a = bt.pr[z].amax_a; p.amax_b = bt.pr[z].amax_b; p.accumulate = bt.pr[z].accumulate;
+    p.ws += (size_t)z * p.splits * p.M * p.N;
+    x6w_body<TA, TB, SEG, 4, 0, TR>(p, zk);
 }
 
 }
@@ -392,6 +407,50 @@
     return (int)hipGetLastError();
 }
 
+int m3t_sgemm_x6w_batch_launch(int n, const m3t_window_problem* pr, int transA, int transB, int M, int N, int K, int lda, int ldb, int ldc,
+                               int act, int seg_len, int seg_stride, int a_off, int b_off, float* ws, int splits, int kchunk, hipStream_t s) {
+    if (n < 1 || n > M3T_WINDOW_BATCH || splits < 1) return M3T_EINVAL;
+    X6WBatch bt = {};
+    for (int i = 0; i < n; ++i) {
+        if (!pr[i].amax_a || !pr[i].amax_b) return M3T_EINVAL;
+        bt.pr[i] = pr[i];
+    }
+    X6WParams p;
+    p.amax_a = p.amax_b = nullptr;
+    p.A = p.B = nullptr; p.C = nullptr; p.bias = nullptr; p.ws = ws;
+    p.M = M; p.N = N; p.K = K; p.lda = lda; p.ldb = ldb; p.ldc = ldc;
+    p.act = act; p.accumulate = 0; p.splits = splits; p.kchunk = kchunk;
+    p.seg_len = seg_len; p.seg_stride = seg_stride; p.a_off = a_off; p.b_off = b_off;
+    dim3 grid(N / WN, M / WM, n * splits), block(WTH);
+    int dev = 0;
+    if (hipGetDevice(&dev) != hipSuccess || dev < 0 || dev >= 32) return M3T_EINVAL;
+#define M3T_X6WB_GO(TA_, TB_, SEG_, TR_)                                                                              \
+    do {                                                                                                               \
+        const size_t lds = 2 * (size_t)stageb_of(4, TA_, TB_, TR_);                                                    \
+        static std::atomic<unsigned> attr_set{0};                                                                      \
+        if (!(attr_set.load(std::memory_order_relaxed) & (1u << dev))) {                                               \
+            hipError_t ea = hipFuncSetAttribute((const void*)sgemm_x6w_batch_kernel<TA_, TB_, SEG_, TR_>,              \
+                                                hipFuncAttributeMaxDynamicSharedMemorySize, (int)lds);                \
+            if (ea != hipSuccess) return (int)ea;                                                                      \
+            attr_set.fetch_or(1u << dev, std::memory_order_relaxed);                                                   \
+        }                                                                                                              \
+        sgemm_x6w_batch_kernel<TA_, TB_, SEG_, TR_><<<grid, block, lds, s>>>(p, bt);                                   \
+    } while (0)
+#define M3T_X6WB_DISPATCH(TR_)                                                                                       \
+    do {                                                                                                               \
+        if (seg_len > 0) M3T_X6WB_GO(1, 0, true, TR_);                                                                 \
+        else if (transA == 0 && transB == 1) M3T_X6WB_GO(0, 1, false, false);                                          \
+        else if (transA == 0 && transB == 0) M3T_X6WB_GO(0, 0, false, TR_);                                            \
+        else if (transA == 1 && transB == 0) M3T_X6WB_GO(1, 0, false, TR_);                                            \
+        else M3T_X6WB_GO(1, 1, false, TR_);                                                                            \
+    } while (0)
+    if (m3t_gemm_tr_enabled()) M3T_X6WB_DISPATCH(true);
+    else M3T_X6WB_DISPATCH(false);
+#undef M3T_X6WB_DISPATCH
+#undef M3T_X6WB_GO
+    return (int)hipGetLastError();
+}
+
 int m3t_sgemm_x6w_bimg_launch(int M, int N, int K, const float* A, int lda, const float* B_img, float* C, int ldc, const float* bias, int act,
                               int accumulate, float* ws, int splits, int kchunk, const unsigned long long* amax_a,
                               const unsigned long long* amax_b, hipStream_t s) {
diff --git a/m3f.pytorch_amd/m3t/_lib.py b/m3f.pytorch_amd/m3t/_lib.py
--- a/m3f.pytorch_amd/m3t/_lib.py
+++ b/m3f.pytorch_amd/m3t/_lib.py
@@ -57,6 +57,8 @@
     "m3t_sgemm_scaled": [_i, _i, _i, _i, _i, _f, _i, _f, _i, _f, _i, _f, _i, _i, _i, _i, _i, _i, _f, _z, _i, _f, _f, _s],
     "m3t_sgemm_window": [_i, _i, _i, _i, _i, _i, _i, _f, _i, _f, _i, _f, _i, _f, _i, _i, _i, _f, _f, _s],
     "m3t_sgemm_window_batch": [_i, C.POINTER(WindowProblem), _i, _i, _i, _i, _i, _i, _i, _i, _i, _i, _i, _i, _s],
+    "m3t_sgemm_scaled_batch": [_i, C.POINTER(WindowProblem), _i, _i, _i, _i, _i, _i, _i, _i, _i, _i, _i, _i, _i, _f, _z, _i, _s],
+    "m3t_sgemm_batch_plan": [_i, _i, _i, _i, _i, _i, _i, _z, _i, C.POINTER(C.c_int), C.POINTER(C.c_int), C.POINTER(C.c_int)],
     "m3t_absmax": [_i, C.POINTER(C.c_void_p), C.POINTER(C.c_size_t), C.POINTER(C.c_int), C.POINTER(C.c_size_t), C.POINTER(C.c_void_p), _s],
     "m3t_sgemm_plan": [_i, _i, _i, _i, _i, _z, _i, C.POINTER(C.c_int), C.POINTER(C.c_int)],
     "m3t_im2col3d": [_f] + [_i] * 14 + [_f, C.c_longlong, _i, C.c_void_p, _s],
diff --git a/m3f.pytorch_amd/m3t/ops.py b/m3f.pytorch_amd/m3t/ops.py
--- a/m3f.pytorch_amd/m3t/ops.py
+++ b/m3f.pytorch_amd/m3t/ops.py
@@ -288,6 +288,38 @@
                                     _p(bias), act, int(accumulate), seg[0], seg[1], seg[2], seg[3],
                                     _p(ws), (ws.numel() * 4) if ws is not None else 0, flags, amax[0], amax[1], _stream())
     _lib.check(rc, "m3t_sgemm")
+
+
+GEMM_BATCH = [os.environ.get("M3T_GEMM_BATCH", "1") != "0"]
+_GEMM_BATCH_SITES = (set(os.environ["M3T_GEMM_BATCH"].split(",")) if os.environ.get("M3T_GEMM_BATCH", "1") not in ("0", "1", "")
+                     else {"proj", "dx"})
+
+
+def sgemm_batch(transA, transB, M, N, K, lda, ldb, ldc, problems, act=0, seg=(0, 0, 0, 0), use_ws=True, prec=None, exclusive=False):
+    if not problems:
+        return
+    dev = problems[0][4].device
+    ws = workspace(dev) if use_ws else None
+    flags = (_PREC[0] if prec is None else prec) | (_lib.M3T_GEMM_EXCLUSIVE if exclusive else 0)
+    if _FENCED[0]:
+        flags |= _lib.M3T_GEMM_BESIDE_SCAN
+    WP = _lib.WindowProblem
+    with _Timed("sgemm_kernel", len(problems), 2.0 * M * N * K * len(problems)) if PROFILE_GEMM[0] else _NULL:
+        for i in range(0, len(problems), _lib.M3T_WINDOW_BATCH):
+            chunk = problems[i:i + _lib.M3T_WINDOW_BATCH]
+            arr = (WP * len(chunk))(*[WP(_vp(A, ao), _vp(Bm, bo), _vp(Cm, co), _vp(bias), aa, ab, int(acc))
+                                      for A, ao, Bm, bo, Cm, co, bias, acc, aa, ab in chunk])
+            rc = lib().m3t_sgemm_scaled_batch(len(chunk), arr, transA, transB, M, N, K, lda, ldb, ldc, act, seg[0], seg[1], seg[2], seg[3],
+                                              _p(ws), (ws.numel() * 4) if ws is not None else 0, flags, _stream())
+            _lib.check(rc, "m3t_sgemm_scaled_batch")
+
+
+def sgemm_batch_plan(n, transA, transB, M, N, K, seg_len=0, prec=None, ws_bytes=_WS_MIN, beside_scan=False):
+    b, sp, pc = C.c_int(0), C.c_int(0), C.c_int(0)
+    flags = (_PREC[0] if prec is None else prec) | (_lib.M3T_GEMM_BESIDE_SCAN if beside_scan else 0)
+    _lib.check(lib().m3t_sgemm_batch_plan(n, transA, transB, M, N, K, seg_len, ws_bytes, flags, C.byref(b), C.byref(sp), C.byref(pc)),
+               "m3t_sgemm_batch_plan")
+    return b.value, sp.value, pc.value
 
 
 _AMAX_ONE = {}
@@ -989,6 +1021,17 @@
 
         def level_fwd(l, idxs, scan, after=None, wide=False, progress=None):
             descs = []
+            if not scan and GEMM_BATCH[0] and "proj" in _GEMM_BATCH_SITES:
+                shapes = {}
+                for s in idxs:
+                    inp = xs[s] if l == 0 else outs[l - 1][s]
+                    for d in (0, 1):
+                        w_ih, _, b_ih, _ = params[s][(2 * l + d) * 4:(2 * l + d) * 4 + 4]
+                        shapes.setdefault((Hs[s], inp.shape[-1]), []).append(
+                            (inp, 0, w_ih, 0, xprojs[l][s], d * 3 * Hs[s], b_ih, False, fslot_x(l, s), fslot_w(l, s, d)))
+                for (H, I), probs in shapes.items():
+                    sgemm_batch(0, 1, B * T, 3 * H, I, I, I, 6 * H, probs, prec=prec, exclusive=alone)
+                return None
             for s in idxs:
                 H = Hs[s]
                 inp = xs[s] if l == 0 else outs[l - 1][s]
@@ -1366,6 +1409,19 @@
             if pg is not None:
                 dx_pieces(l, idxs, pg[0], pg[1], cur_stream())
                 return
+            todo = [s for s in idxs if need_dx[l][s]]
+            if GEMM_BATCH[0] and "dx" in _GEMM_BATCH_SITES and len(todo) > 1:
+                shapes = {}
+                for s in todo:
+                    shapes.setdefault((Hs[s], layer_io(l, s)[0].shape[-1]), []).append(s)
+                for (H, I), ss in shapes.items():
+                    for d in (0, 1):
+                        sgemm_batch(0, 0, B * T, I, 3 * H, 6 * H, I, I,
+                                    [(dgx[l][s], d * 3 * H, params[s][(2 * l + d) * 4], 0, dinp[l][s], 0, None, d == 1, bslot(l, s, d), fslot_w(l, s, d))
+                                     for s in ss], prec=prec)
+                for s in todo:
+                    cur[s] = dinp[l][s]
+                return
             for s in idxs:
                 H = Hs[s]
                 inp, out, gts = layer_io(l, s)
@@ -1380,6 +1436,27 @@
         rr = [0]
 
         def _level_dw(l, idxs, pool):
+            if GEMM_BATCH[0] and "dw" in _GEMM_BATCH_SITES and T > 1:
+                hh, ih = {}, {}
+                for s in idxs:
+                    H = Hs[s]
+                    inp, out, gts = layer_io(l, s)
+                    I = inp.shape[-1]
+                    for d in (0, 1):
+                        base = s * per + 1 + (2 * l + d) * 4
+                        dw_ih, dw_hh = out_grads[base:base + 2]
+                        hh.setdefault((H, out.stride(1), d), []).append(
+                            (dgh[l][s], d * B * T * 3 * H, out, d * H, dw_hh, 0, None, False, bslot(l, s, d), one if bslots is not None else None))
+                        ih.setdefault((H, I), []).append((dgx[l][s], d * 3 * H, inp, 0, dw_ih, 0, None, False, bslot(l, s, d), fslot_x(l, s)))
+                for (H, ldo, d), probs in hh.items():
+                    with (on_stream(pool[rr[0] % len(pool)]) if pool is not None else _NULL):
+                        sgemm_batch(1, 0, 3 * H, H, B * (T - 1), 3 * H, ldo, H, probs, seg=(T - 1, T, 1 - d, d), prec=prec)
+                rr[0] += 1
+                for (H, I), probs in ih.items():
+                    with (on_stream(pool[rr[0] % len(pool)]) if pool is not None else _NULL):
+                        sgemm_batch(1, 0, 3 * H, I, B * T, 6 * H, I, I, probs, prec=prec)
+                rr[0] += 1
+                return
             for s in idxs:
                 H = Hs[s]
                 inp, out, gts = layer_io(l, s)
```

Result: no change. 2853 (median of 6 runs) (+0.8%).
